# Ray0089/geometric-aware-dense-matching

Measured on AMD Instinct MI355X. Metric: rgbd_crops_per_sec_geomatch_fwd, higher is better.
Workload: dtype bf16x3/f32acc

## Files before the change

geometric_aware_dense_matching_amd/_lib.py:

```python
import ctypes
import os
import subprocess

_PKG = os.path.dirname(os.path.abspath(__file__))
LIB_PATH = os.path.join(_PKG, "libgdm_hip.so")
CSRC = os.path.join(_PKG, "csrc")

_vp = ctypes.c_void_p
_i = ctypes.c_int
_f = ctypes.c_float
_sz = ctypes.c_size_t

GDM_RANSAC_MAX_H = 4096


class KnnJob(ctypes.Structure):
    _fields_ = [("support", _vp), ("query", _vp), ("idx", _vp), ("d2", _vp),
                ("support_bstride", ctypes.c_int64), ("query_bstride", ctypes.c_int64),
                ("S", ctypes.c_int32), ("Q", ctypes.c_int32), ("K", ctypes.c_int32), ("grid_w", ctypes.c_int32)]


class PwSeg(ctypes.Structure):
    _fields_ = [("x", _vp), ("idx", _vp), ("C", ctypes.c_int32), ("n_src", ctypes.c_int32)]


class PwJob(ctypes.Structure):
    _fields_ = [("x", _vp), ("wt", _vp), ("out", _vp), ("n", ctypes.c_int32)]


class CopyJob(ctypes.Structure):
    _fields_ = [("dst", _vp), ("src", _vp), ("sb", ctypes.c_int64), ("s1", ctypes.c_int64), ("s2", ctypes.c_int64),
                ("B", ctypes.c_int32), ("R1", ctypes.c_int32), ("R2", ctypes.c_int32), ("E", ctypes.c_int32)]


SIGNATURES = {
    "gdm_last_error": (ctypes.c_char_p, []),
    "gdm_version": (_i, []),
    "gdm_knn_batch": (None, [_vp, _sz, _sz, _sz, _vp, _sz, _sz, _vp]),
    "gdm_knn_batch_hip": (_i, [_vp, _vp, _i, _i, _i, _i, _vp, _vp, _vp]),
    "gdm_knn_jobs_workspace_bytes": (_sz, [ctypes.POINTER(KnnJob), _i, _i]),
    "gdm_knn_jobs_ws_hip": (_i, [ctypes.POINTER(KnnJob), _i, _i, _vp, _sz, _vp]),
    "gdm_ballquery_hip": (_i, [_i, _i, _i, _f, _i, _vp, _vp, _vp, _vp]),
    "gdm_furthestsampling_hip": (_i, [_i, _i, _i, _vp, _vp, _vp, _vp]),
    "gdm_interpolation_forward_hip": (_i, [_i, _i, _i, _i, _vp, _vp, _vp, _vp, _vp]),
    "gdm_interpolation_backward_hip": (_i, [_i, _i, _i, _i, _vp, _vp, _vp, _vp, _vp]),
    "gdm_labelstat_ballrange_hip": (_i, [_i, _i, _i, _f, _i, _vp, _vp, _vp, _vp, _vp]),
    "gdm_labelstat_idx_hip": (_i, [_i, _i, _i, _i, _i, _vp, _vp, _vp, _vp]),
    "gdm_group_gather_hip": (_i, [_vp, _vp, _i, _i, _i, _i, _i, _vp, _vp]),
    "gdm_group_gather_bwd2_hip": (_i, [_vp, ctypes.c_long, _vp, _i, _i, _i, _i, _i, _vp, _vp]),
    "gdm_gather_max_hip": (_i, [_vp, _vp, _i, _i, _i, _i, _i, _vp, _vp, _vp]),
    "gdm_gather_max_bwd_hip": (_i, [_vp, _vp, _i, _i, _i, _i, _vp, _vp]),
    "gdm_rel_pos_enc_hip": (_i, [_vp, _vp, _i, _i, _i, _vp, _vp]),
    "gdm_att_pool_hip": (_i, [_vp, _vp, _i, _i, _i, _i, _vp, _vp]),
    "gdm_att_pool_bwd_hip": (_i, [_vp, _vp, _vp, _i, _i, _i, _i, _vp, _vp, _vp]),
    "gdm_match_workspace_bytes": (_sz, [_i, _i, _i]),
    "gdm_match_hip": (_i, [_vp, _vp, _i, _i, _i, _i, _i, _vp, _vp, _vp, _vp, _sz, _vp]),
    "gdm_match_rows_bytes": (_sz, [_i]),
    "gdm_match_partial_bytes": (_sz, [_i, _i]),
    "gdm_match_pack_hip": (_i, [_vp, _i, _i, _i, _i, _vp, _vp]),
    "gdm_match_pack2_hip": (_i, [_vp, _i, _i, _vp, _vp, _i, _i, _vp, _i, _i, _vp]),
    "gdm_match_packed_hip": (_i, [_vp, _vp, _i, _i, _i, _vp, _vp, _vp, _vp, _sz, _vp]),
    "gdm_seg_mask_hip": (_i, [_vp, _i, _i, _vp, _vp, _vp]),
    "gdm_spline_aggregate_hip": (_i, [_vp, _vp, _vp, _vp, _vp, _vp, _i, _i, _i, _i, _vp, _vp]),
    "gdm_spline_aggregate_bwd_hip": (_i, [_vp, _vp, _vp, _vp, _i, _i, _i, _vp, _vp]),
    "gdm_spline_direct3_hip": (_i, [_vp, _vp, _vp, _vp, _vp, _vp, _vp, _i, _i, _i, _i, _i, _vp, _vp, _vp, _vp]),
    "gdm_gemm_grouped_hip": (_i, [_vp, _vp, _vp, _vp, _i, _i, _i, _i, _vp, _vp]),
    "gdm_spline_pairs_aggregate3_hip": (_i, [_vp, _vp, _vp, _vp, _vp, _vp, _i, _i, _i, _vp, _vp, _vp, _vp]),
    "gdm_upsample_bilinear_hip": (_i, [_vp, ctypes.c_long, _i, _i, _i, _i, _vp, _vp]),
    "gdm_upsample_bilinear_bwd_hip": (_i, [_vp, ctypes.c_long, _i, _i, _i, _i, _vp, _vp]),
    "gdm_topk_rows_hip": (_i, [_vp, ctypes.c_long, _i, _i, _vp, _vp, _vp]),
    "gdm_topk_negdist_hip": (_i, [_vp, _vp, _i, _i, _i, _vp, _vp]),
    "gdm_edge_feature_hip": (_i, [_vp, _vp, _i, _i, _i, _i, _vp, _vp]),
    "gdm_edge_feature_bwd_hip": (_i, [_vp, _vp, _i, _i, _i, _i, _vp, _vp]),
    "gdm_circle_rows_fwd_hip": (_i, [_vp, _i, _i, _vp, _vp, _vp, _vp, _f, _f, _f, _vp, _vp, _vp, _vp]),
    "gdm_circle_rows_bwd_hip": (_i, [_vp, _i, _i, _vp, _vp, _vp, _vp, _f, _f, _f, _vp, _vp, _vp, _vp, _vp]),
    "gdm_circle_match_rows_bytes": (_sz, [_i]),
    "gdm_circle_match_tp_bytes": (_sz, [_i]),
    "gdm_circle_match_pack_hip": (_i, [_vp, _i, _vp, _vp, _vp, _vp]),
    "gdm_circle_match_nbr_hip": (_i, [_vp, _i, _f, _vp, _vp]),
    "gdm_circle_match_visbits_hip": (_i, [_vp, _i, _i, _vp, _vp]),
    "gdm_circle_match_nbr_items_hip": (_i, [_vp, _i, _vp, _i, _vp, _vp]),
    "gdm_circle_match_fwd2_hip": (_i, [_vp, _vp, _vp, _vp, _vp, _i, _i, _vp, _vp, _vp, _vp, _i, _vp, _i, _f, _f, _vp, _vp, _vp, _vp]),
    "gdm_circle_match_bwd2_hip": (_i, [_vp, _vp, _vp, _vp, _vp, _i, _i, _vp, _vp, _vp, _vp, _i, _vp, _i, _f, _f, _vp, _vp, _vp, _vp, _vp, _vp]),
    "gdm_circle_match_bwd_parts": (_i, [_i, _i]),
    "gdm_lfa_stage_hip": (_i, [_vp] * 13 + [_i, _i, _i, _i, _i, _f, _vp, _vp]),
    "gdm_kabsch_stats_hip": (_i, [_vp, ctypes.c_long, _i, _i, _vp, _vp, _vp, _i, _i, _i, _vp, _vp]),
    "gdm_kabsch_solve_hip": (_i, [_vp, _i, _i, _vp, _vp, _vp]),
    "gdm_ransac_workspace_bytes": (_sz, [_i, _i, _i]),
    "gdm_ransac_pose_hip": (_i, [_vp, ctypes.c_long, _i, _i, _vp, _vp, _vp, _vp, _i, _i, _i, _i, _f, ctypes.c_double, ctypes.c_uint32, _i,
                                 _vp, _sz, _vp, _vp, _vp, _vp, _vp]),
    "gdm_icp_transform_hip": (_i, [_vp, ctypes.c_long, _i, _i, _vp, _i, _i, _vp, _vp]),
    "gdm_icp_update_hip": (_i, [_vp, ctypes.c_long, _i, _i, _vp, _vp, _vp, _vp, _i, _i, _i, _f, ctypes.c_double, _i, _vp, _vp, _vp, _vp,
                                _vp]),
    "gdm_targets_workspace_bytes": (_sz, [_i, _i, _i]),
    "gdm_hpr_visible_hip": (_i, [_vp, ctypes.c_long, _vp, _vp, _i, _i, _vp, _sz, _vp, _vp, _vp]),
    "gdm_pose_targets_hip": (_i, [_vp, ctypes.c_long, _i, _i, _vp, _vp, _vp, ctypes.c_long, _vp, _i, _i, _i, ctypes.c_double, _vp, _sz,
                                  _vp, _vp, _vp, _vp, _vp]),
    "gdm_affine_act_maxk_hip": (_i, [_vp, _vp, _vp, ctypes.c_long, _i, ctypes.c_long, _i, _i, _f, _vp, _vp]),
    "gdm_prelu1_hip": (_i, [_vp, _vp, ctypes.c_long, _vp, _vp]),
    "gdm_prelu1_bwd_hip": (_i, [_vp, _vp, _vp, ctypes.c_long, _vp, _vp, _vp]),
    "gdm_affine_act_hip": (_i, [_vp, _vp, _vp, _vp, _vp, _vp, ctypes.c_long, _i, ctypes.c_long, _i, _f, _vp, _vp]),
    "gdm_upconv3x3_gather_hip": (_i, [_vp, _vp, _vp, _i, _i, _i, _i, _i, _i, _i, _f, _vp, _vp]),
    "gdm_upconv3x3_gather2_hip": (_i, [_vp, _vp, _vp, _i, _i, _i, _i, _i, _i, _i, _f, _vp, _vp, _vp]),
    "gdm_upconv3x3_gather_bwd_hip": (_i, [_vp, _i, _i, _i, _i, _i, _i, _vp, _vp]),
    "gdm_upconv_fused64_weight_bytes": (_sz, []),
    "gdm_upconv_fused64_pack_weight_hip": (_i, [_vp, _vp, _vp]),
    "gdm_upconv_fused64_hip": (_i, [_vp, _vp, _vp, _vp, _i, _i, _i, _i, _i, _i, _i, _f, _vp, _vp]),
    "gdm_psp_combine2_hip": (_i, [_vp, _vp, _i, _vp, _i, _vp, _i, _vp, _i, _vp, _i, _i, _i, _i, _vp, _vp, _vp]),
    "gdm_gather_add_affine_act2_hip": (_i, [_vp, _vp, _vp, _vp, _vp, _i, _i, _i, _i, _i, _f, _vp, _vp, _i, _vp]),
    "gdm_conv1x1_gather_add_act2_hip": (_i, [_vp, _vp, _vp, _vp, _vp, _vp, _i, _i, _i, ctypes.c_long, _i, _f, _i, _vp, _vp]),
    "gdm_conv64_gather_add_act_mfma2_hip": (_i, [_vp, _vp, _vp, _vp, _vp, _vp, _i, _i, ctypes.c_long, _i, _f, _i, _i, _vp, _vp, _i, _vp]),
    "gdm_conv64_gather_add_final_hip": (_i, [_vp, _vp, _vp, _vp, _vp, _vp, _i, _i, ctypes.c_long, _i, _f, _vp, _vp, _vp, _vp]),
    "gdm_conv3x3_act_bytes": (_sz, [_i, _i, _i, _i]),
    "gdm_conv3x3_weight_bytes": (_sz, [_i, _i]),
    "gdm_conv3x3_pack_weight_hip": (_i, [_vp, _i, _i, _vp, _vp]),
    "gdm_conv3x3_pack_act_hip": (_i, [_vp, _i, _i, _i, _i, _vp, _vp]),
    "gdm_conv3x3_packed_hip": (_i, [_vp, _vp, _vp, _vp, _vp, _i, _i, _i, _i, _i, _i, _vp, _vp]),
    "gdm_conv3x3_strided_hip": (_i, [_vp, _vp, _vp, _vp, _vp, _i, _i, _i, _i, _i, _i, _i, _vp, _vp, _vp]),
    "gdm_conv1x1_strided_hip": (_i, [_vp, _vp, _vp, _vp, _i, _i, _i, _i, _i, _i, _i, _vp, _vp]),
    "gdm_affine_relu_maxpool_hip": (_i, [_vp, _vp, _vp, _i, _i, _i, _i, _vp, _vp]),
    "gdm_conv1x1_logsoftmax_hip": (_i, [_vp, _vp, _vp, _i, _i, ctypes.c_long, _vp, _vp]),
    "gdm_pack_rows64_hip": (_i, [_vp, _i, _vp, _vp]),
    "gdm_upconv_final_points_hip": (_i, [_vp, _vp, _vp, _vp, _vp, _i, _f, _vp, _vp, _i, _i, _i, _i, _i, _i, _vp, _vp]),
    "gdm_psp_pools_hip": (_i, [_vp, ctypes.c_long, _i, _i, _vp, _vp, _vp, _vp, _vp]),
    "gdm_psp_pools_bwd_hip": (_i, [_vp, _vp, _vp, _vp, ctypes.c_long, _i, _i, _vp, _vp]),
    "gdm_conv1x1_weight_bytes": (_sz, [_i, _i]),
    "gdm_conv1x1_pack_weight_hip": (_i, [_vp, _i, _i, _vp, _vp]),
    "gdm_conv_pack_weight_dgrad_hip": (_i, [_vp, _i, _i, _i, _vp, _vp]),
    "gdm_conv1x1_packed_hip": (_i, [_vp, _vp, _vp, _vp, _i, _i, _i, _i, _i, _i, _i, _vp, _vp]),
    "gdm_depth_to_xyz_hip": (_i, [_vp, _vp, _vp, _i, _i, _i, _i, _vp, _vp]),
    "gdm_depth_normals_hip": (_i, [_vp, _vp, _i, _i, _i, _i, _i, _i, _vp, _vp]),
    "gdm_warp_crop_hip": (_i, [_vp, _vp, _vp, _vp, _vp, _vp, _vp, _i, _i, _i, _i, _vp, _vp, _vp, _vp, _vp, _vp]),
    "gdm_fill_depth_workspace_bytes": (_sz, [_i, _i, _i, _i]),
    "gdm_fill_depth_hip": (_i, [_vp, _i, _i, _i, _i, _f, _vp, _sz, _vp, _vp, _vp]),
    "gdm_bn_sums_len": (ctypes.c_long, [_i, _i, ctypes.c_long]),
    "gdm_bn_stats_hip": (_i, [_vp, _i, _i, ctypes.c_long, _vp, _vp]),
    "gdm_bn_fwd_apply_hip": (_i, [_vp, _vp, _i, _vp, _vp, _i, _i, ctypes.c_long, _f, _f, _i, _f, _vp, _vp, _vp, _vp, _vp]),
    "gdm_bn_bwd_reduce_hip": (_i, [_vp, _vp, _vp, _i, _i, ctypes.c_long, _i, _f, _vp, _vp]),
    "gdm_bn_bwd_apply_hip": (_i, [_vp, _vp, _vp, _i, _vp, _vp, _i, _i, ctypes.c_long, _i, _f, _vp, _vp, _vp, _vp]),
    "gdm_point_heads2_hip": (_i, [_vp, _vp, _i, _vp, _vp, _i, _i, _i, _i, _vp, _vp, _vp, _vp, _i, _i, _vp, _vp, _i, _vp, _vp, _vp]),
    "gdm_pointwise2_hip": (_i, [ctypes.POINTER(PwSeg), _i, _vp, _i, _vp, _vp, _i, _i, _i, _i, _f, _vp, _i, _i, _i, _vp]),
    "gdm_pointwise_jobs_hip": (_i, [ctypes.POINTER(PwJob), _i, _i, _i, _i, _vp]),
    "gdm_pointwise_chain2_hip": (_i, [_vp, _vp, _vp, _vp, _i, _f, _vp, _vp, _vp, _i, _f, _i, _i, _i, _i, _i, _vp, _vp, _vp]),
    "gdm_stem_weight_bytes": (_sz, []),
    "gdm_stem_pack_weight_hip": (_i, [_vp, _vp, _vp]),
    "gdm_stem_hip": (_i, [_vp, _vp, _vp, _vp, _i, _i, _i, _vp, _vp, _vp]),
    "gdm_wgrad_x_bytes": (_sz, [_i, _i, _i, _i]),
    "gdm_wgrad_go_bytes": (_sz, [_i, _i, _i, _i]),
    "gdm_wgrad_pack_x_hip": (_i, [_vp, _i, _i, _i, _i, _vp, _vp]),
    "gdm_wgrad_pack_go_hip": (_i, [_vp, _i, _i, _i, _i, _vp, _vp]),
    "gdm_wgrad_x1_bytes": (_sz, [_i, _i, _i]),
    "gdm_wgrad_pack_x1_hip": (_i, [_vp, _i, _i, _i, _vp, _vp]),
    "gdm_mfma_probe_hip": (_i, [_i, _i, _i, _vp, _vp]),
    "gdm_mfma_probe_lds_hip": (_i, [_i, _i, _i, _vp, _vp]),
    "gdm_wgrad_direct_hip": (_i, [_vp, ctypes.c_long, _vp, ctypes.c_long, _i, _i, _i, _i, _i, _vp, _vp, _vp]),
    "gdm_conv1x1_packed_wb_hip": (_i, [_vp, _vp, ctypes.c_long, _i, _i, _i, _i, _i, _vp, _vp]),
    "gdm_copy_jobs_hip": (_i, [ctypes.POINTER(CopyJob), _i, _vp]),
}

_lib = None


def _objects_state():
    st = {}
    for f in sorted(os.listdir(CSRC)):
        if f.endswith(".o"):
            st[f] = os.stat(os.path.join(CSRC, f)).st_mtime_ns
    return st


def build(verbose=False):
    import hashlib
    import json
    import time
    before = _objects_state()
    out = None if verbose else subprocess.DEVNULL
    t0 = time.time()
    subprocess.check_call(["make", "-C", CSRC, "-j4"], stdout=out)
    after = _objects_state()
    rebuilt = sorted(f for f, m in after.items() if before.get(f) != m)
    with open(LIB_PATH, "rb") as f:
        digest = hashlib.sha256(f.read()).hexdigest()[:16]
    rec = {"mode": "hipcc --offload-arch=gfx950 via csrc/Makefile (in-tree, ahead of time)", "recompiled": rebuilt,
           "up_to_date": sorted(set(after) - set(rebuilt)), "lib": os.path.basename(LIB_PATH), "lib_bytes": os.path.getsize(LIB_PATH),
           "lib_sha256_16": digest, "seconds": round(time.time() - t0, 1), "when": time.strftime("%Y-%m-%dT%H:%M:%S")}
    try:
        with open(os.path.join(CSRC, "build_record.json"), "w") as f:
            json.dump(rec, f, indent=1)
    except OSError:
        pass
    print("[gdm build] recompiled %d of %d translation units%s; %s %d bytes sha256 %s" %
          (len(rebuilt), len(after), (": " + " ".join(rebuilt)) if rebuilt else "", rec["lib"], rec["lib_bytes"], digest))
    return LIB_PATH


def build_record():
    import hashlib
    import json
    rec = {}
    try:
        with open(os.path.join(CSRC, "build_record.json")) as f:
            rec = json.load(f)
    except (OSError, ValueError):
        rec = {"mode": "prebuilt library (no build record travelled)"}
    try:
        with open(LIB_PATH, "rb") as f:
            rec["loaded_lib_sha256_16"] = hashlib.sha256(f.read()).hexdigest()[:16]
    except OSError:
        rec["loaded_lib_sha256_16"] = None
    rec.pop("up_to_date", None)
    if rec.get("lib_sha256_16") is not None:
        rec["record_matches_loaded_lib"] = rec["lib_sha256_16"] == rec["loaded_lib_sha256_16"]
    return rec


def lib():
    global _lib
    if _lib is None:
        if not os.path.exists(LIB_PATH):
            raise RuntimeError(
                "libgdm_hip.so is not built (%s). Run `python -c 'import __graft_entry__ as g; g.build()'` "
                "or `make -C geometric_aware_dense_matching_amd/csrc`. There is no CPU fallback." % LIB_PATH)
        import torch
        l = ctypes.CDLL(LIB_PATH)
        for name, (res, args) in SIGNATURES.items():
            fn = getattr(l, name)
            fn.restype = res
            fn.argtypes = args
        _lib = l
    return _lib


class GdmError(RuntimeError):
    pass


def check(rc, what):
    if rc != 0:
        msg = lib().gdm_last_error()
        raise GdmError("%s failed (rc=%d): %s" % (what, rc, msg.decode() if msg else "?"))
```

geometric_aware_dense_matching_amd/csrc/gdm_conv.hip:

```cpp
#include "gdm_common.h"
#include <math.h>
#include <stdlib.h>

namespace {

typedef __attribute__((ext_vector_type(16))) float f32x16;
typedef __attribute__((ext_vector_type(8))) __bf16 bf16x8;
typedef __attribute__((ext_vector_type(4))) unsigned u32x4;

constexpr int ROWB = 512;
constexpr int CV_PIX = 256;
constexpr int CV_CO = 128;
constexpr int CV_PANEL = CV_CO * ROWB;
#ifndef GDM_CONV_TAP_INNER
#define GDM_CONV_TAP_INNER 1
#endif
#ifndef GDM_CONV16_PF
#define GDM_CONV16_PF 2
#endif
#ifndef GDM_CONV_GLDS
#define GDM_CONV_GLDS 1
#endif

__device__ __forceinline__ void split8(const float* v, unsigned (&hi)[4], unsigned (&lo)[4])
{
#pragma unroll
    for (int j = 0; j < 4; ++j) gdm_split2(v[2 * j], v[2 * j + 1], hi[j], lo[j]);
}

__global__ __launch_bounds__(256) void conv_pack_act_kernel(const float* __restrict__ x, int C, int H, int W,
                                                            unsigned char* __restrict__ out)
{
    __shared__ float t[128][65];
    const int b = blockIdx.z, chunk = blockIdx.y;
    const int nchunk = (C + 127) / 128;
    const int cvalid = min(128, C - chunk * 128);
    const int hw = H * W;
    const long plane = (long)(H + 2) * (W + 2);
    const int p0 = blockIdx.x * 64;
    const int lane = threadIdx.x & 63, w = threadIdx.x >> 6;
    const int p = min(p0 + lane, hw - 1);
    const float* xb = x + ((long)b * C + chunk * 128) * hw;
    for (int c = w; c < cvalid; c += 4) t[c][lane] = xb[(long)c * hw + p];
    __syncthreads();
    const int pp = p0 + lane;
    if (pp >= hw) return;
    const int y = pp / W, xx = pp - y * W;
    unsigned char* o = out + (((long)(b * nchunk + chunk) * 32) * plane + (long)(y + 1) * (W + 2) + xx + 1) * 16;
    for (int q = w; q * 8 < cvalid; q += 4) {
        float v[8];
#pragma unroll
        for (int j = 0; j < 8; ++j) v[j] = t[q * 8 + j][lane];
        unsigned hi[4], lo[4];
        split8(v, hi, lo);
        *reinterpret_cast<uint4*>(o + (long)q * plane * 16) = make_uint4(hi[0], hi[1], hi[2], hi[3]);
        *reinterpret_cast<uint4*>(o + (long)(16 + q) * plane * 16) = make_uint4(lo[0], lo[1], lo[2], lo[3]);
    }
}

__global__ __launch_bounds__(256) void conv_pack_w_kernel(const float* __restrict__ w, int Cout, int Cin, int taps, unsigned char* __restrict__ out,
                                                          int dgrad = 0)
{
    const int nchunk = (Cin + 127) / 128;
    const int CoutP = (Cout + 127) & ~127;
    const long item = (long)blockIdx.x * 256 + threadIdx.x;
    const long rows = (long)taps * nchunk * CoutP;
    if (item >= rows * 16) return;
    const int ch = (int)(item & 15);
    const long row = item >> 4;
    const int co = (int)(row % CoutP);
    const int tc = (int)(row / CoutP);
    const int chunk = tc % nchunk, tap = tc / nchunk;
    float v[8];
#pragma unroll
    for (int j = 0; j < 8; ++j) {
        const int ci = chunk * 128 + ch * 8 + j;
        const bool in = co < Cout && ci < Cin;
        v[j] = !in ? 0.f : dgrad ? w[((long)ci * Cout + co) * taps + (taps - 1 - tap)] : w[((long)co * Cin + ci) * taps + tap];
    }
    unsigned hi[4], lo[4];
    split8(v, hi, lo);
    unsigned char* r = out + row * ROWB;
    *reinterpret_cast<uint4*>(r + ch * 16) = make_uint4(hi[0], hi[1], hi[2], hi[3]);
    *reinterpret_cast<uint4*>(r + 256 + ch * 16) = make_uint4(lo[0], lo[1], lo[2], lo[3]);
}

__device__ __forceinline__ int swz(int col, int ch) { return col * ROWB + (((ch & 16) | ((ch ^ col) & 15)) << 4); }

typedef __attribute__((ext_vector_type(4))) float f32x4;

#ifndef GDM_CONV_NPH
#define GDM_CONV_NPH 2
#endif
#ifndef GDM_CONV16_LATE
#define GDM_CONV16_LATE 1
#endif
#ifndef GDM_CONV_MFMA_ORDER
#define GDM_CONV_MFMA_ORDER 0
#endif
constexpr int MF_NPH = GDM_CONV_NPH;
constexpr int MF_WPIX = 16 * MF_NPH;
constexpr int MF_WAVES = CV_PIX / MF_WPIX;
constexpr int MF_THREADS = MF_WAVES * 64;
constexpr int MF_TSTRIDE = 132;
constexpr int MF_SMEM = 2 * CV_PANEL > CV_PIX * MF_TSTRIDE * 4 ? 2 * CV_PANEL : CV_PIX * MF_TSTRIDE * 4;

template <int ACT, bool HAS_RES, int TAPS = 9, bool PIXMAJOR = false, int NKS = 8, int NCB = 8, int WV = MF_WAVES>
__global__ __launch_bounds__(MF_THREADS) void conv_mfma16_kernel(const unsigned char* __restrict__ xpk, const unsigned char* __restrict__ wpk,
                                                                 const float* __restrict__ scale, const float* __restrict__ shift,
                                                                 const float* __restrict__ res, int B, int Cin, int Cout, int H, int W,
                                                                 float* __restrict__ out, const int32_t* __restrict__ rowidx = nullptr,
                                                                 const int32_t* __restrict__ tile_co0 = nullptr,
                                                                 unsigned char* __restrict__ outpk = nullptr, int stride = 1,
                                                                 long wbstride = 0)
{
    extern __shared__ __attribute__((aligned(16))) unsigned char smem[];
    constexpr int NS = NKS / 2;
    constexpr int UG = (NCB % 2 == 0) ? 2 : 3;
    constexpr int NPR = NCB / UG;
    constexpr int PANEL = NCB * 16 * ROWB;
    constexpr int TST = NCB * 16 + 4;
    static_assert(NCB == 8 || (NCB == 4 && !PIXMAJOR) || (NCB == 9 && !PIXMAJOR && WV == 8),
                  "64-channel tiles: NCHW / packed output only; 144-channel tiles: NCHW fp32 output only (no packed output: a tile straddles 128-channel chunks)");
    constexpr int NPH = MF_NPH;
    const int tid = threadIdx.x, lane = tid & 63;
    const int wave = __builtin_amdgcn_readfirstlane(tid >> 6);
    const int l16 = lane & 15, kg = lane >> 4;
    const int nchunk = (Cin + 127) / 128;
    const int npanel = TAPS * nchunk;
    const int hw = H * W;
    const long ptot = rowidx ? (long)B : (long)B * hw;
    const unsigned bx = blockIdx.x, by = blockIdx.y;
    const long pix0 = (long)bx * (WV * MF_WPIX) + wave * MF_WPIX;
    const int co0 = tile_co0 ? __builtin_amdgcn_readfirstlane(tile_co0[bx]) : by * (NCB * 16);
    const long pc = min(pix0, ptot - MF_WPIX);
    const int b = (int)(pc / hw);
    const int prem = (int)(pc - (long)b * hw);
    const int Wi = W * stride;
    const long plane = (long)(H * stride + 2) * (Wi + 2);
    const long oplane = (long)(H + 2) * (W + 2);
    const __amdgpu_buffer_rsrc_t xr = __builtin_amdgcn_make_buffer_rsrc(const_cast<unsigned char*>(xpk), (short)0, 0x7ffffff0, 0x00020000);
    int avoff[NPH];
#pragma unroll
    for (int ph = 0; ph < NPH; ++ph) {
        const int pr = prem + 16 * ph;
        const int yy = pr / W, xx = pr - yy * W;
        const long pixbase = rowidx ? (long)max(rowidx[pc + l16 + 16 * ph], 0) : (long)(yy * stride) * (Wi + 2) + (long)(xx + l16) * stride;
        avoff[ph] = (int)(((long)kg * plane + pixbase) * 16);
    }

    u32x4 ahi[NS][NPH], alo[NS][NPH];
    struct Pan { int chunk, ky, kx; };
    auto pan_next = [&](Pan p) -> Pan {
        if (TAPS == 1) { ++p.chunk; return p; }
        if (GDM_CONV_TAP_INNER) {
            if (++p.kx == 3) { p.kx = 0; if (++p.ky == 3) { p.ky = 0; ++p.chunk; } }
        } else {
            if (++p.chunk == nchunk) { p.chunk = 0; if (++p.kx == 3) { p.kx = 0; ++p.ky; } }
        }
        return p;
    };
    const int a_base = (int)(((long)(rowidx ? 0 : b) * nchunk * 32) * plane * 16);
    const int a_chunk = (int)(32 * plane * 16), a_rowb = (Wi + 2) * 16;
    auto pan_a = [&](Pan p) -> int { return a_base + p.chunk * a_chunk + p.ky * a_rowb + p.kx * 16; };
    const int sstride = (int)(4 * plane * 16);
    const int lostride = (int)(16 * plane * 16);
    auto load_a = [&](int r, int S) {
#pragma unroll
        for (int ph = 0; ph < NPH; ++ph) {
            ahi[S][ph] = __builtin_bit_cast(u32x4, __builtin_amdgcn_raw_buffer_load_b128(xr, avoff[ph], r + S * sstride, 0));
            alo[S][ph] = __builtin_bit_cast(u32x4, __builtin_amdgcn_raw_buffer_load_b128(xr, avoff[ph], r + S * sstride + lostride, 0));
        }
    };
    constexpr int THREADS = WV * 64, WGPIX = WV * MF_WPIX;
    constexpr int HS = (NCB * 512 / THREADS) / 2;
    u32x4 stage[HS];
    const __amdgpu_buffer_rsrc_t wr = __builtin_amdgcn_make_buffer_rsrc(const_cast<unsigned char*>(wpk), (short)0, 0x7ffffff0, 0x00020000);
    const int w_base = (wbstride ? (int)(((long)bx * WGPIX / hw) * wbstride) : 0) + co0 * ROWB;
    const int w_panel = ((Cout + 127) & ~127) * ROWB;
    auto pan_w = [&](Pan p) -> int { return w_base + ((TAPS == 1) ? p.chunk : (p.ky * 3 + p.kx) * nchunk + p.chunk) * w_panel; };
    auto stage_load = [&](int src, int half) {
#pragma unroll
        for (int i = 0; i < HS; ++i)
            stage[i] = __builtin_bit_cast(u32x4, __builtin_amdgcn_raw_buffer_load_b128(wr, tid * 16, src + (half * HS + i) * THREADS * 16, 0));
    };
    auto stage_store = [&](int buf, int half) {
        unsigned char* base = smem + buf * PANEL;
#pragma unroll
        for (int i = 0; i < HS; ++i) {
            const int g = (half * HS + i) * THREADS + tid;
            *reinterpret_cast<u32x4*>(base + swz(g >> 5, g & 31)) = stage[i];
        }
    };
    constexpr bool GLDS = GDM_CONV_GLDS && WV == 8;
    constexpr int NPIECE = PANEL / 1024 / 8;
    int glds_voff = 0;
    if (GLDS) {
        const int hrow = lane >> 5, sl = lane & 31;
        const int col15 = (2 * wave + hrow) & 15;
        glds_voff = wave * 1024 + hrow * 512 + (((sl & 16) | ((sl ^ col15) & 15)) << 4);
    }
    typedef __attribute__((address_space(3))) void* lds_void_ptr;
    auto stage_glds = [&](int src, int buf) {
#pragma unroll
        for (int i = 0; i < NPIECE; ++i)
            __builtin_amdgcn_raw_ptr_buffer_load_lds(wr, (lds_void_ptr)(smem + buf * PANEL + (i * 8 + wave) * 1024), 16, glds_voff, src + i * 8192, 0, 0);
    };

    f32x4 acc[NPH][NCB];
#pragma unroll
    for (int ph = 0; ph < NPH; ++ph)
#pragma unroll
        for (int cb = 0; cb < NCB; ++cb)
#pragma unroll
            for (int i = 0; i < 4; ++i) acc[ph][cb][i] = 0.f;

    constexpr int LATE = GDM_CONV16_LATE < NS ? GDM_CONV16_LATE : NS;
    Pan pcur = {0, (TAPS == 1) ? 1 : 0, (TAPS == 1) ? 1 : 0};
    if (GLDS) {
        stage_glds(pan_w(pcur), 0);
    } else {
        stage_load(pan_w(pcur), 0);
        stage_store(0, 0);
        stage_load(pan_w(pcur), 1);
        stage_store(0, 1);
    }
    int rcur = pan_a(pcur);
#pragma unroll
    for (int S = 0; S < NS - LATE; ++S) load_a(rcur, S);
    Pan pnxt = npanel > 1 ? pan_next(pcur) : pcur;
    int rnext = pan_a(pnxt), wnext = pan_w(pnxt);
    for (int it = 0; it < npanel; ++it) {
        __syncthreads();
        const bool more = it + 1 < npanel;
        const unsigned char* base = smem + (it & 1) * PANEL;
        constexpr int PF = GDM_CONV16_PF;
        constexpr int NU = NPR * NS;
        u32x4 fh[PF + 1][UG], fl[PF + 1][UG];
        auto frag_load = [&](int un) {
            const int S = un / NPR, pr = un % NPR, slot = un % (PF + 1);
#pragma unroll
            for (int j = 0; j < UG; ++j) {
                const int col = (UG * pr + j) * 16 + l16;
                fh[slot][j] = *reinterpret_cast<const u32x4*>(base + swz(col, 4 * S + kg));
                fl[slot][j] = *reinterpret_cast<const u32x4*>(base + swz(col, 16 + 4 * S + kg));
            }
        };
#pragma unroll
        for (int un = 0; un < PF; ++un) frag_load(un);
#pragma unroll
        for (int u = 0; u < NU; ++u) {
            const int S = u / NPR, pr = u % NPR, slot = u % (PF + 1);
            if (u + PF < NU) frag_load(u + PF);
#if GDM_CONV_MFMA_ORDER == 0
#pragma unroll
            for (int ph = 0; ph < NPH; ++ph) {
                const bf16x8 ah = __builtin_bit_cast(bf16x8, ahi[S][ph]);
                const bf16x8 al = __builtin_bit_cast(bf16x8, alo[S][ph]);
#pragma unroll
                for (int j = 0; j < UG; ++j) {
                    f32x4 c = acc[ph][UG * pr + j];
                    c = __builtin_amdgcn_mfma_f32_16x16x32_bf16(ah, __builtin_bit_cast(bf16x8, fl[slot][j]), c, 0, 0, 0);
                    c = __builtin_amdgcn_mfma_f32_16x16x32_bf16(al, __builtin_bit_cast(bf16x8, fh[slot][j]), c, 0, 0, 0);
                    c = __builtin_amdgcn_mfma_f32_16x16x32_bf16(ah, __builtin_bit_cast(bf16x8, fh[slot][j]), c, 0, 0, 0);
                    acc[ph][UG * pr + j] = c;
                }
            }
#else
#pragma unroll
            for (int prod = 0; prod < 3; ++prod)
#pragma unroll
                for (int ph = 0; ph < NPH; ++ph)
#pragma unroll
                    for (int j = 0; j < UG; ++j) {
                        const bf16x8 av = __builtin_bit_cast(bf16x8, prod == 1 ? alo[S][ph] : ahi[S][ph]);
                        const bf16x8 bv = __builtin_bit_cast(bf16x8, prod == 0 ? fl[slot][j] : fh[slot][j]);
                        acc[ph][UG * pr + j] = __builtin_amdgcn_mfma_f32_16x16x32_bf16(av, bv, acc[ph][UG * pr + j], 0, 0, 0);
                    }
#endif
            if (pr == NPR - 1 && S < NS - LATE) load_a(rnext, S);
            if (!GLDS && u == NU / 2 && more) {
                stage_store((it + 1) & 1, 0);
                stage_load(wnext, 1);
            }
            if (u == 0) {
                if (more) { if (GLDS) stage_glds(wnext, (it + 1) & 1); else stage_load(wnext, 0); }
#pragma unroll
                for (int S2 = NS - LATE; S2 < NS; ++S2) load_a(rcur, S2);
            }
#pragma unroll
            for (int i = 0; i < 3 * UG * NPH; ++i) {
                __builtin_amdgcn_sched_group_barrier(0x008, 1, 0);
                if (u + PF < NU && (i % NPH) == 0 && i < 2 * UG * NPH) __builtin_amdgcn_sched_group_barrier(0x100, 1, 0);
            }
            __builtin_amdgcn_sched_barrier(0);
        }
        if (!GLDS && more) stage_store((it + 1) & 1, 1);
        rcur = rnext;
        if (it + 2 < npanel) pnxt = pan_next(pnxt);
        rnext = pan_a(pnxt);
        wnext = pan_w(pnxt);
    }

    if (pix0 >= ptot) return;
    if (PIXMAJOR) {
#pragma unroll
        for (int cb = 0; cb < NCB; ++cb) {
            const int co = co0 + cb * 16 + l16;
            if (co >= Cout) continue;
            const float sc = scale ? scale[co] : 1.f, sh = shift ? shift[co] : 0.f;
            const int ocol = tile_co0 ? cb * 16 + l16 : co;
            const int ostride = tile_co0 ? CV_CO : Cout;
#pragma unroll
            for (int ph = 0; ph < NPH; ++ph)
#pragma unroll
                for (int r = 0; r < 4; ++r) {
                    float v = acc[ph][cb][r] * sc + sh;
                    if (ACT == 1) v = fmaxf(v, 0.f);
                    out[(pix0 + 16 * ph + 4 * kg + r) * ostride + ocol] = v;
                }
        }
        return;
    }
    float* tl = reinterpret_cast<float*>(smem) + wave * MF_WPIX * TST;
    if (outpk) __syncthreads();
#pragma unroll
    for (int cb = 0; cb < NCB; ++cb) {
        const int co = co0 + cb * 16 + l16;
        const bool live = co < Cout;
        const float sc = (live && scale) ? scale[co] : 1.f, sh = (live && shift) ? shift[co] : 0.f;
        float* op = out ? out + ((long)b * Cout + (live ? co : 0)) * hw + prem : nullptr;
        const float* rp = (HAS_RES && live) ? res + ((long)b * Cout + co) * hw + prem : nullptr;
#pragma unroll
        for (int ph = 0; ph < NPH; ++ph) {
            const int poff = 16 * ph + 4 * kg;
            float v[4];
#pragma unroll
            for (int j = 0; j < 4; ++j) v[j] = acc[ph][cb][j] * sc + sh;
            if (HAS_RES && live) {
                const float4 r4 = *reinterpret_cast<const float4*>(rp + poff);
                v[0] += r4.x; v[1] += r4.y; v[2] += r4.z; v[3] += r4.w;
            }
            if (ACT == 1) {
#pragma unroll
                for (int j = 0; j < 4; ++j) v[j] = fmaxf(v[j], 0.f);
            }
            if (op && live) *reinterpret_cast<float4*>(op + poff) = make_float4(v[0], v[1], v[2], v[3]);
            if (outpk) {
#pragma unroll
                for (int j = 0; j < 4; ++j) tl[(poff + j) * TST + cb * 16 + l16] = live ? v[j] : 0.f;
            }
        }
    }
    if (outpk) {
        __builtin_amdgcn_fence(__ATOMIC_ACQ_REL, "wavefront");
        const int lr = lane & 31, h = lane >> 5;
        const int ochunks = (Cout + 127) / 128;
        const int ochunk = co0 / 128;
#pragma unroll
        for (int half = 0; half < MF_WPIX / 32; ++half) {
            const int pp = prem + 32 * half + lr;
            const int yy = pp / W, xx = pp - yy * W;
            unsigned char* ob = outpk + (((long)(b * ochunks + ochunk) * 32) * oplane + (long)(yy + 1) * (W + 2) + xx + 1) * 16;
            const float* row = tl + (32 * half + lr) * TST;
#pragma unroll
            for (int it = 0; it < NCB; ++it) {
                const int ql = 2 * it + h;
                if (co0 + ql * 8 >= Cout) continue;
                const int q = (co0 % 128) / 8 + ql;
                const float4 a0 = *reinterpret_cast<const float4*>(row + ql * 8);
                const float4 a1 = *reinterpret_cast<const float4*>(row + ql * 8 + 4);
                const float v[8] = {a0.x, a0.y, a0.z, a0.w, a1.x, a1.y, a1.z, a1.w};
                unsigned hi[4], lo[4];
                split8(v, hi, lo);
                *reinterpret_cast<uint4*>(ob + (long)q * oplane * 16) = make_uint4(hi[0], hi[1], hi[2], hi[3]);
                *reinterpret_cast<uint4*>(ob + (long)(16 + q) * oplane * 16) = make_uint4(lo[0], lo[1], lo[2], lo[3]);
            }
        }
    }
}

#define CONV_KERNEL conv_mfma16_kernel
constexpr int CONV_THREADS = MF_THREADS, CONV_WPIX = MF_WPIX, CONV_SMEM = MF_SMEM;

}

namespace {
template <int CHAIN>
__global__ __launch_bounds__(512) void mfma_probe_kernel(int iters, float* __restrict__ sink)
{
    typedef __attribute__((ext_vector_type(8))) __bf16 pb_bf16x8;
    typedef __attribute__((ext_vector_type(4))) float pb_f32x4;
    const int lane = threadIdx.x & 63;
    pb_f32x4 acc[8];
#pragma unroll
    for (int i = 0; i < 8; ++i) acc[i] = pb_f32x4{0.f, 0.f, 0.f, 0.f};
    const unsigned seed = 0x3f803f80u + (unsigned)lane;
    u32x4 av = {seed, seed ^ 1u, seed ^ 2u, seed ^ 3u}, bv = {seed ^ 4u, seed ^ 5u, seed ^ 6u, seed ^ 7u};
    const pb_bf16x8 a = __builtin_bit_cast(pb_bf16x8, av), b = __builtin_bit_cast(pb_bf16x8, bv);
    for (int it = 0; it < iters; it += CHAIN) {
#pragma unroll
        for (int i = 0; i < 8; ++i)
#pragma unroll
            for (int c = 0; c < CHAIN; ++c) acc[i] = __builtin_amdgcn_mfma_f32_16x16x32_bf16(a, b, acc[i], 0, 0, 0);
    }
    float t = 0.f;
#pragma unroll
    for (int i = 0; i < 8; ++i) t += acc[i][0] + acc[i][1] + acc[i][2] + acc[i][3];
    if (t == 12345.678f) sink[0] = t;
}
template <int RPU>
__global__ __launch_bounds__(512) void mfma_probe_lds_kernel(int iters, float* __restrict__ sink)
{
    typedef __attribute__((ext_vector_type(8))) __bf16 pb_bf16x8;
    typedef __attribute__((ext_vector_type(4))) float pb_f32x4;
    extern __shared__ __attribute__((aligned(16))) unsigned char pl[];
    const int tid = threadIdx.x, lane = tid & 63;
    for (int i = tid; i < 4096; i += 512) reinterpret_cast<u32x4*>(pl)[i] = u32x4{0x3f803f80u, 0x3f803f80u, 0x3f803f80u, 0x3f803f80u + (unsigned)i};
    __syncthreads();
    pb_f32x4 acc[4];
#pragma unroll
    for (int i = 0; i < 4; ++i) acc[i] = pb_f32x4{0.f, 0.f, 0.f, 0.f};
    const unsigned seed = 0x3f803f80u + (unsigned)lane;
    u32x4 a0 = {seed, seed ^ 1u, seed ^ 2u, seed ^ 3u}, a1 = {seed ^ 4u, seed ^ 5u, seed ^ 6u, seed ^ 7u};
    u32x4 f[4] = {a0, a1, a0, a1};
    int off = lane * 16;
    for (int it = 0; it < iters; ++it) {
#pragma unroll
        for (int r = 0; r < RPU; ++r) f[r] = *reinterpret_cast<const u32x4*>(pl + ((off + r * 1024) & 0xffff));
        off += 4096;
#pragma unroll
        for (int prod = 0; prod < 3; ++prod)
#pragma unroll
            for (int i = 0; i < 4; ++i)
                acc[i] = __builtin_amdgcn_mfma_f32_16x16x32_bf16(__builtin_bit_cast(pb_bf16x8, prod == 1 ? a1 : a0),
                                                                 __builtin_bit_cast(pb_bf16x8, f[(i + prod) & 3]), acc[i], 0, 0, 0);
    }
    float t = 0.f;
#pragma unroll
    for (int i = 0; i < 4; ++i) t += acc[i][0] + acc[i][1] + acc[i][2] + acc[i][3];
    if (t == 12345.678f) sink[0] = t;
}
}

extern "C" int gdm_mfma_probe_lds_hip(int blocks, int iters, int rpu, float* sink, void* stream)
{
    GDM_CHECK_ARG(blocks >= 1 && blocks <= 65535 && iters >= 1 && (rpu == 1 || rpu == 2 || rpu == 4) && sink, "gdm_mfma_probe_lds_hip: bad arguments");
    if (rpu == 4) hipLaunchKernelGGL(mfma_probe_lds_kernel<4>, dim3(blocks), dim3(512), 65536, (hipStream_t)stream, iters, sink);
    else if (rpu == 2) hipLaunchKernelGGL(mfma_probe_lds_kernel<2>, dim3(blocks), dim3(512), 65536, (hipStream_t)stream, iters, sink);
    else hipLaunchKernelGGL(mfma_probe_lds_kernel<1>, dim3(blocks), dim3(512), 65536, (hipStream_t)stream, iters, sink);
    return gdm_launch_status("mfma_probe_lds_kernel");
}

extern "C" int gdm_mfma_probe_hip(int blocks, int iters, int chain, float* sink, void* stream)
{
    GDM_CHECK_ARG(blocks >= 1 && blocks <= 65535 && iters >= 3 && iters % 3 == 0 && (chain == 1 || chain == 3) && sink,
                  "gdm_mfma_probe_hip: bad arguments (iters a multiple of 3, chain 1 or 3)");
    if (chain == 3) hipLaunchKernelGGL(mfma_probe_kernel<3>, dim3(blocks), dim3(512), 0, (hipStream_t)stream, iters, sink);
    else hipLaunchKernelGGL(mfma_probe_kernel<1>, dim3(blocks), dim3(512), 0, (hipStream_t)stream, iters, sink);
    return gdm_launch_status("mfma_probe_kernel");
}

static bool cin_ok(int Cin) { return Cin == 64 || (Cin >= 128 && Cin % 128 == 0); }

static bool narrow_tiles(unsigned pixel_tiles, int Cout)
{
    return Cout <= 64 || (long)pixel_tiles * ((Cout + 127) / 128) < 256;
}

extern "C" size_t gdm_conv3x3_act_bytes(int B, int Cin, int H, int W)
{
    if (B < 1 || !cin_ok(Cin) || H < 1 || W < 1) return 0;
    return (size_t)B * (H + 2) * (W + 2) * ((Cin + 127) / 128) * ROWB;
}

extern "C" size_t gdm_conv3x3_weight_bytes(int Cout, int Cin)
{
    if (Cout < 1 || !cin_ok(Cin)) return 0;
    return (size_t)9 * ((Cin + 127) / 128) * ((Cout + 127) & ~127) * ROWB;
}

extern "C" size_t gdm_conv1x1_weight_bytes(int Cout, int Cin)
{
    if (Cout < 1 || !cin_ok(Cin)) return 0;
    return (size_t)((Cin + 127) / 128) * ((Cout + 127) & ~127) * ROWB;
}

static int pack_weight(const float* w, int Cout, int Cin, int taps, void* wpk, void* stream, const char* who, int dgrad = 0)
{
    GDM_CHECK_ARG(w && wpk, "%s: NULL pointer", who);
    GDM_CHECK_ARG(Cout >= 1 && cin_ok(Cin), "%s: Cout=%d Cin=%d (Cin a multiple of 128, or 64)", who, Cout, Cin);
    const long items = (long)taps * ((Cin + 127) / 128) * ((Cout + 127) & ~127) * 16;
    hipLaunchKernelGGL(conv_pack_w_kernel, dim3(gdm_cdiv(items, 256)), dim3(256), 0, (hipStream_t)stream, w, Cout, Cin, taps, (unsigned char*)wpk, dgrad);
    return gdm_launch_status("conv_pack_w_kernel");
}

extern "C" int gdm_conv_pack_weight_dgrad_hip(const float* w, int Cout, int Cin, int taps, void* wpk, void* stream)
{
    GDM_CHECK_ARG(taps == 9 || taps == 1, "gdm_conv_pack_weight_dgrad_hip: taps=%d (9 or 1)", taps);
    return pack_weight(w, Cin, Cout, taps, wpk, stream, "gdm_conv_pack_weight_dgrad_hip", 1);
}

extern "C" int gdm_conv3x3_pack_weight_hip(const float* w, int Cout, int Cin, void* wpk, void* stream)
{
    return pack_weight(w, Cout, Cin, 9, wpk, stream, "gdm_conv3x3_pack_weight_hip");
}

extern "C" int gdm_conv1x1_pack_weight_hip(const float* w, int Cout, int Cin, void* wpk, void* stream)
{
    return pack_weight(w, Cout, Cin, 1, wpk, stream, "gdm_conv1x1_pack_weight_hip");
}

extern "C" int gdm_conv3x3_pack_act_hip(const float* x, int B, int Cin, int H, int W, void* xpk, void* stream)
{
    GDM_CHECK_ARG(x && xpk, "gdm_conv3x3_pack_act_hip: NULL pointer");
    GDM_CHECK_ARG(B >= 1 && B <= 65535 && cin_ok(Cin) && H >= 1 && W >= 1, "gdm_conv3x3_pack_act_hip: bad shape (Cin=%d: a multiple of 128, or 64)", Cin);
    dim3 grid(gdm_cdiv((long)H * W, 64), (Cin + 127) / 128, B);
    hipLaunchKernelGGL(conv_pack_act_kernel, grid, dim3(256), 0, (hipStream_t)stream, x, Cin, H, W, (unsigned char*)xpk);
    return gdm_launch_status("conv_pack_act_kernel");
}

static int conv3x3_launch(const void* xpk, const void* wpk, const float* scale, const float* shift, const float* res,
                          int B, int Cin, int Cout, int H, int W, int stride, int act, float* out, void* outpk, void* stream,
                          const char* who);

extern "C" int gdm_conv3x3_packed_hip(const void* xpk, const void* wpk, const float* scale, const float* shift, const float* res,
                                      int B, int Cin, int Cout, int H, int W, int act, float* out, void* stream)
{
    return conv3x3_launch(xpk, wpk, scale, shift, res, B, Cin, Cout, H, W, 1, act, out, nullptr, stream, "gdm_conv3x3_packed_hip");
}

extern "C" int gdm_conv3x3_strided_hip(const void* xpk, const void* wpk, const float* scale, const float* shift, const float* res,
                                       int B, int Cin, int Cout, int H, int W, int stride, int act, float* out, void* outpk, void* stream)
{
    return conv3x3_launch(xpk, wpk, scale, shift, res, B, Cin, Cout, H, W, stride, act, out, outpk, stream, "gdm_conv3x3_strided_hip");
}

static int conv3x3_launch(const void* xpk, const void* wpk, const float* scale, const float* shift, const float* res,
                          int B, int Cin, int Cout, int H, int W, int stride, int act, float* out, void* outpk, void* stream,
                          const char* who)
{
    GDM_CHECK_ARG(stride == 1 || stride == 2, "%s: stride=%d (1 or 2)", who, stride);
    GDM_CHECK_ARG(xpk && wpk && (out || outpk), "%s: NULL pointer", who);
    GDM_CHECK_ARG(B >= 1 && cin_ok(Cin) && Cout >= 1, "%s: Cin=%d Cout=%d (Cin a multiple of 128, or 64)", who, Cin, Cout);
    GDM_CHECK_ARG(W % 32 == 0 && H >= 1 && (H * W) % CONV_WPIX == 0,
                  "%s: W=%d must be a multiple of 32 and H*W=%d of %d", who, W, H * W, CONV_WPIX);
    GDM_CHECK_ARG(act == 0 || act == 1, "%s: act=%d", who, act);
    GDM_CHECK_ARG(!outpk || (Cout % 8 == 0 && ((long)B * H * W) % CV_PIX == 0),
                  "%s: packed output needs Cout %% 8 == 0 and B*H*W %% 256 == 0 (got Cout=%d, B*H*W=%ld)", who, Cout, (long)B * H * W);
    const long ptot = (long)B * H * W;
    dim3 grid(gdm_cdiv(ptot, CV_PIX), gdm_cdiv(Cout, CV_CO));
    hipStream_t s = (hipStream_t)stream;
    constexpr int SMEM = CONV_SMEM;
    static bool attr = false;
    if (!attr) {
        (void)hipFuncSetAttribute((const void*)CONV_KERNEL<0, false>, hipFuncAttributeMaxDynamicSharedMemorySize, SMEM);
        (void)hipFuncSetAttribute((const void*)CONV_KERNEL<1, false>, hipFuncAttributeMaxDynamicSharedMemorySize, SMEM);
        (void)hipFuncSetAttribute((const void*)CONV_KERNEL<0, true>, hipFuncAttributeMaxDynamicSharedMemorySize, SMEM);
        (void)hipFuncSetAttribute((const void*)CONV_KERNEL<1, true>, hipFuncAttributeMaxDynamicSharedMemorySize, SMEM);
        (void)hipFuncSetAttribute((const void*)CONV_KERNEL<0, false, 9, false, 4>, hipFuncAttributeMaxDynamicSharedMemorySize, SMEM);
        (void)hipFuncSetAttribute((const void*)CONV_KERNEL<1, false, 9, false, 4>, hipFuncAttributeMaxDynamicSharedMemorySize, SMEM);
        (void)hipFuncSetAttribute((const void*)CONV_KERNEL<0, true, 9, false, 4>, hipFuncAttributeMaxDynamicSharedMemorySize, SMEM);
        (void)hipFuncSetAttribute((const void*)CONV_KERNEL<1, true, 9, false, 4>, hipFuncAttributeMaxDynamicSharedMemorySize, SMEM);
        attr = true;
    }
#define CV(A, R, NK) hipLaunchKernelGGL((CONV_KERNEL<A, R, 9, false, NK>), grid, dim3(CONV_THREADS), SMEM, s, (const unsigned char*)xpk, (const unsigned char*)wpk, scale, shift, res, B, Cin, Cout, H, W, out, (const int32_t*)nullptr, (const int32_t*)nullptr, (unsigned char*)outpk, stride)
    if (narrow_tiles(grid.x, Cout)) {
        constexpr int SMEM4 = 2 * 64 * ROWB > CV_PIX * 68 * 4 ? 2 * 64 * ROWB : CV_PIX * 68 * 4;
        const dim3 grid4(grid.x, gdm_cdiv(Cout, 64));
        static bool attr4 = false;
#define CV4(A, R, NK) hipLaunchKernelGGL((CONV_KERNEL<A, R, 9, false, NK, 4>), grid4, dim3(CONV_THREADS), SMEM4, s, (const unsigned char*)xpk, (const unsigned char*)wpk, scale, shift, res, B, Cin, Cout, H, W, out, (const int32_t*)nullptr, (const int32_t*)nullptr, (unsigned char*)outpk, stride)
#define AT4(A, R, NK) (void)hipFuncSetAttribute((const void*)CONV_KERNEL<A, R, 9, false, NK, 4>, hipFuncAttributeMaxDynamicSharedMemorySize, SMEM4)
        if (!attr4) {
            AT4(0, false, 4); AT4(1, false, 4); AT4(0, true, 4); AT4(1, true, 4);
            AT4(0, false, 8); AT4(1, false, 8); AT4(0, true, 8); AT4(1, true, 8);
            attr4 = true;
        }
        if (Cin != 64 && (long)grid4.x * grid4.y < 256 && ptot % (CV_PIX / 2) == 0) {
            const dim3 grid4h(gdm_cdiv(ptot, CV_PIX / 2), grid4.y);
            static bool attr4h = false;
#define CV4H(A, R) hipLaunchKernelGGL((CONV_KERNEL<A, R, 9, false, 8, 4, MF_WAVES / 2>), grid4h, dim3(CONV_THREADS / 2), SMEM4, s, (const unsigned char*)xpk, (const unsigned char*)wpk, scale, shift, res, B, Cin, Cout, H, W, out, (const int32_t*)nullptr, (const int32_t*)nullptr, (unsigned char*)outpk, stride)
#define AT4H(A, R) (void)hipFuncSetAttribute((const void*)CONV_KERNEL<A, R, 9, false, 8, 4, MF_WAVES / 2>, hipFuncAttributeMaxDynamicSharedMemorySize, SMEM4)
            if (!attr4h) {
                AT4H(0, false); AT4H(1, false); AT4H(0, true); AT4H(1, true);
                attr4h = true;
            }
            if (act == 0) { if (res) CV4H(0, true); else CV4H(0, false); }
            else { if (res) CV4H(1, true); else CV4H(1, false); }
#undef CV4H
#undef AT4H
            return gdm_launch_status("conv_mfma16_kernel (3x3, 64-channel tiles, 128 pixels)");
        }
        if (Cin == 64) {
            if (act == 0) { if (res) CV4(0, true, 4); else CV4(0, false, 4); }
            else { if (res) CV4(1, true, 4); else CV4(1, false, 4); }
        } else {
            if (act == 0) { if (res) CV4(0, true, 8); else CV4(0, false, 8); }
            else { if (res) CV4(1, true, 8); else CV4(1, false, 8); }
        }
#undef CV4
#undef AT4
        return gdm_launch_status("conv_mfma16_kernel (3x3, 64-channel tiles)");
    }
    if (Cin == 64) {
        if (act == 0) { if (res) CV(0, true, 4); else CV(0, false, 4); }
        else { if (res) CV(1, true, 4); else CV(1, false, 4); }
    } else {
        if (act == 0) { if (res) CV(0, true, 8); else CV(0, false, 8); }
        else { if (res) CV(1, true, 8); else CV(1, false, 8); }
    }
#undef CV
    return gdm_launch_status("conv_mfma16_kernel (3x3)");
}

extern "C" int gdm_gemm_grouped_hip(const void* xpk, const void* wpk, const int32_t* rowidx, const int32_t* tile_co0, int R, int M,
                                    int Cin, int Cout_total, float* out, void* stream)
{
    GDM_CHECK_ARG(xpk && wpk && rowidx && tile_co0 && out, "gdm_gemm_grouped_hip: NULL pointer");
    GDM_CHECK_ARG(R >= 256 && R % 256 == 0 && M >= 1 && Cin >= 128 && Cin % 128 == 0 && Cout_total >= 128 && Cout_total % 128 == 0,
                  "gdm_gemm_grouped_hip: R=%d (multiple of 256) M=%d Cin=%d Cout_total=%d (multiples of 128)", R, M, Cin, Cout_total);
    static bool attr = false;
    if (!attr) {
        (void)hipFuncSetAttribute((const void*)CONV_KERNEL<0, false, 1, true>, hipFuncAttributeMaxDynamicSharedMemorySize, 2 * CV_PANEL);
        attr = true;
    }
    hipLaunchKernelGGL((CONV_KERNEL<0, false, 1, true>), dim3(R / CV_PIX, 1), dim3(CONV_THREADS), 2 * CV_PANEL, (hipStream_t)stream,
                       (const unsigned char*)xpk, (const unsigned char*)wpk, (const float*)nullptr, (const float*)nullptr, (const float*)nullptr,
                       R, Cin, Cout_total, 1, M, out, rowidx, tile_co0);
    return gdm_launch_status("gemm_grouped_kernel");
}

static int conv1x1_launch(const void* xpk, const void* wpk, const float* scale, const float* shift,
                          int B, int Cin, int Cout, int H, int W, int stride, int act, int pixel_major, float* out, void* stream,
                          const char* who);

extern "C" int gdm_conv1x1_packed_hip(const void* xpk, const void* wpk, const float* scale, const float* shift,
                                      int B, int Cin, int Cout, int H, int W, int act, int pixel_major, float* out, void* stream)
{
    return conv1x1_launch(xpk, wpk, scale, shift, B, Cin, Cout, H, W, 1, act, pixel_major, out, stream, "gdm_conv1x1_packed_hip");
}

extern "C" int gdm_conv1x1_packed_wb_hip(const void* xpk, const void* wpk, long w_bstride, int B, int Cin, int Cout, int H, int W, float* out,
                                         void* stream)
{
    GDM_CHECK_ARG(xpk && wpk && out, "gdm_conv1x1_packed_wb_hip: NULL pointer");
    GDM_CHECK_ARG(B >= 1 && Cin >= 128 && Cin % 128 == 0 && Cout >= 1, "gdm_conv1x1_packed_wb_hip: Cin=%d Cout=%d (Cin a multiple of 128)", Cin, Cout);
    GDM_CHECK_ARG(W % 32 == 0 && H >= 1 && (H * W) % CV_PIX == 0, "gdm_conv1x1_packed_wb_hip: W=%d must be a multiple of 32 and H*W=%d of %d",
                  W, H * W, CV_PIX);
    GDM_CHECK_ARG(w_bstride >= 0 && w_bstride % 16 == 0, "gdm_conv1x1_packed_wb_hip: w_bstride=%ld", w_bstride);
    const long ptot = (long)B * H * W;
    dim3 grid(gdm_cdiv(ptot, CV_PIX), gdm_cdiv(Cout, CV_CO));
    static bool attr = false;
    if (!attr) {
        (void)hipFuncSetAttribute((const void*)CONV_KERNEL<0, false, 1, false>, hipFuncAttributeMaxDynamicSharedMemorySize, 2 * CV_PANEL);
        attr = true;
    }
    hipLaunchKernelGGL((CONV_KERNEL<0, false, 1, false>), grid, dim3(CONV_THREADS), 2 * CV_PANEL, (hipStream_t)stream, (const unsigned char*)xpk,
                       (const unsigned char*)wpk, (const float*)nullptr, (const float*)nullptr, (const float*)nullptr, B, Cin, Cout, H, W, out,
                       (const int32_t*)nullptr, (const int32_t*)nullptr, (unsigned char*)nullptr, 1, w_bstride);
    return gdm_launch_status("conv1x1_bf16x3_kernel (per-image weights)");
}

extern "C" int gdm_conv1x1_strided_hip(const void* xpk, const void* wpk, const float* scale, const float* shift,
                                       int B, int Cin, int Cout, int H, int W, int stride, int act, float* out, void* stream)
{
    return conv1x1_launch(xpk, wpk, scale, shift, B, Cin, Cout, H, W, stride, act, 0, out, stream, "gdm_conv1x1_strided_hip");
}

static int conv1x1_launch(const void* xpk, const void* wpk, const float* scale, const float* shift,
                          int B, int Cin, int Cout, int H, int W, int stride, int act, int pixel_major, float* out, void* stream,
                          const char* who)
{
    GDM_CHECK_ARG(stride == 1 || stride == 2, "%s: stride=%d (1 or 2)", who, stride);
    GDM_CHECK_ARG(xpk && wpk && out, "%s: NULL pointer", who);
    GDM_CHECK_ARG(B >= 1 && cin_ok(Cin) && Cout >= 1, "%s: Cin=%d Cout=%d (Cin a multiple of 128, or 64)", who, Cin, Cout);
    GDM_CHECK_ARG(Cin != 64 || !pixel_major, "%s: Cin=64 is built for the NCHW output only", who);
    GDM_CHECK_ARG(W % 32 == 0 && H >= 1 && (H * W) % CONV_WPIX == 0,
                  "%s: W=%d must be a multiple of 32 and H*W=%d of %d", who, W, H * W, CONV_WPIX);
    GDM_CHECK_ARG(act == 0 || act == 1, "%s: act=%d", who, act);
    const long ptot = (long)B * H * W;
    const unsigned ptiles = gdm_cdiv(ptot, CV_PIX);
    if (Cin != 64 && !pixel_major && stride == 1 && Cout % 144 == 0 && GDM_CONV_GLDS) {
        const long r128 = gdm_cdiv((long)ptiles * gdm_cdiv(Cout, 128), 256) * 128, r144 = gdm_cdiv((long)ptiles * (Cout / 144), 256) * 144;
        if (r144 < r128) {
            constexpr int PANEL9 = 9 * 16 * ROWB, TILE9 = CV_PIX * (9 * 16 + 4) * 4;
            constexpr int SMEM9 = 2 * PANEL9 > TILE9 ? 2 * PANEL9 : TILE9;
            static bool attr9 = false;
            if (!attr9) {
                (void)hipFuncSetAttribute((const void*)CONV_KERNEL<0, false, 1, false, 8, 9>, hipFuncAttributeMaxDynamicSharedMemorySize, SMEM9);
                (void)hipFuncSetAttribute((const void*)CONV_KERNEL<1, false, 1, false, 8, 9>, hipFuncAttributeMaxDynamicSharedMemorySize, SMEM9);
                attr9 = true;
            }
            const dim3 grid9(ptiles, Cout / 144);
#define C19(A) hipLaunchKernelGGL((CONV_KERNEL<A, false, 1, false, 8, 9>), grid9, dim3(CONV_THREADS), SMEM9, (hipStream_t)stream, (const unsigned char*)xpk, (const unsigned char*)wpk, scale, shift, (const float*)nullptr, B, Cin, Cout, H, W, out, (const int32_t*)nullptr, (const int32_t*)nullptr, (unsigned char*)nullptr, stride)
            if (act == 0) C19(0); else C19(1);
#undef C19
            return gdm_launch_status("conv1x1_bf16x3_kernel (144-channel tiles)");
        }
    }
    const bool narrow = Cin != 64 && !pixel_major && narrow_tiles(ptiles, Cout);
    const unsigned ctiles = gdm_cdiv(Cout, narrow ? 64 : CV_CO);
    const dim3 grid(ptiles, ctiles);
    hipStream_t s = (hipStream_t)stream;
    static bool attr = false;
    if (!attr) {
        (void)hipFuncSetAttribute((const void*)CONV_KERNEL<0, false, 1, false>, hipFuncAttributeMaxDynamicSharedMemorySize, 2 * CV_PANEL);
        (void)hipFuncSetAttribute((const void*)CONV_KERNEL<1, false, 1, false>, hipFuncAttributeMaxDynamicSharedMemorySize, 2 * CV_PANEL);
        (void)hipFuncSetAttribute((const void*)CONV_KERNEL<0, false, 1, true>, hipFuncAttributeMaxDynamicSharedMemorySize, 2 * CV_PANEL);
        (void)hipFuncSetAttribute((const void*)CONV_KERNEL<1, false, 1, true>, hipFuncAttributeMaxDynamicSharedMemorySize, 2 * CV_PANEL);
        (void)hipFuncSetAttribute((const void*)CONV_KERNEL<0, false, 1, false, 4>, hipFuncAttributeMaxDynamicSharedMemorySize, 2 * CV_PANEL);
        (void)hipFuncSetAttribute((const void*)CONV_KERNEL<1, false, 1, false, 4>, hipFuncAttributeMaxDynamicSharedMemorySize, 2 * CV_PANEL);
        attr = true;
    }
    if (Cin == 64) {
#define C1TAIL , (const int32_t*)nullptr, (const int32_t*)nullptr, (unsigned char*)nullptr, stride
#define C1H(A) hipLaunchKernelGGL((CONV_KERNEL<A, false, 1, false, 4>), grid, dim3(CONV_THREADS), 2 * CV_PANEL, s, (const unsigned char*)xpk, (const unsigned char*)wpk, scale, shift, (const float*)nullptr, B, Cin, Cout, H, W, out C1TAIL)
        if (act == 0) C1H(0); else C1H(1);
#undef C1H
        return gdm_launch_status("conv1x1_bf16x3_kernel");
    }
    if (narrow) {
        const dim3 grid4 = grid;
        static bool attr4 = false;
        if (!attr4) {
            (void)hipFuncSetAttribute((const void*)CONV_KERNEL<0, false, 1, false, 8, 4>, hipFuncAttributeMaxDynamicSharedMemorySize, 2 * 64 * ROWB);
            (void)hipFuncSetAttribute((const void*)CONV_KERNEL<1, false, 1, false, 8, 4>, hipFuncAttributeMaxDynamicSharedMemorySize, 2 * 64 * ROWB);
            attr4 = true;
        }
#define C14(A) hipLaunchKernelGGL((CONV_KERNEL<A, false, 1, false, 8, 4>), grid4, dim3(CONV_THREADS), 2 * 64 * ROWB, s, (const unsigned char*)xpk, (const unsigned char*)wpk, scale, shift, (const float*)nullptr, B, Cin, Cout, H, W, out C1TAIL)
        if (act == 0) C14(0); else C14(1);
#undef C14
        return gdm_launch_status("conv1x1_bf16x3_kernel (64-channel tiles)");
    }
#define C1(A, P) hipLaunchKernelGGL((CONV_KERNEL<A, false, 1, P>), grid, dim3(CONV_THREADS), 2 * CV_PANEL, s, (const unsigned char*)xpk, (const unsigned char*)wpk, scale, shift, (const float*)nullptr, B, Cin, Cout, H, W, out C1TAIL)
    if (act == 0) { if (pixel_major) C1(0, true); else C1(0, false); }
    else { if (pixel_major) C1(1, true); else C1(1, false); }
#undef C1
    return gdm_launch_status("conv1x1_bf16x3_kernel");
}
```

geometric_aware_dense_matching_amd/ops.py:

```python
import ctypes
import os

import torch

from . import _lib, settings
from ._lib import KnnJob, check

MATCH_BF16X3 = 0
MATCH_F32 = 1


def _stream():
    return torch.cuda.current_stream().cuda_stream


_side_streams = {}


def side_stream(device, which=0):
    key = (device.index if device.index is not None else torch.cuda.current_device(), which)
    st = _side_streams.get(key)
    if st is None:
        st = torch.cuda.Stream(device=device)
        _side_streams[key] = st
    return st


def _stream_lane(device):
    h = torch.cuda.current_stream(device).cuda_stream
    idx = device.index if device.index is not None else torch.cuda.current_device()
    for (d, which), st in _side_streams.items():
        if d == idx and st.cuda_stream == h:
            return ("side", which)
    if _pool is _default_pool:
        return ("main", h)
    return "main"


class fork:

    def __init__(self, device, which=0, after=(), start=None):
        self.side = side_stream(device, which)
        self.cur = torch.cuda.current_stream(device)
        self.after = tuple(after) if isinstance(after, (tuple, list)) else (after,)
        self.start = start
        self._ctx = None

    def __enter__(self):
        if self.start is not None:
            self.side.wait_event(self.start)
        else:
            self.side.wait_stream(self.cur)
        for ev in self.after:
            if ev is not None:
                self.side.wait_event(ev)
        self._ctx = torch.cuda.stream(self.side)
        self._ctx.__enter__()
        return self

    def __exit__(self, *exc):
        self._ctx.__exit__(*exc)
        return False

    def use(self, *tensors):
        for t in tensors:
            if torch.is_tensor(t) and t.is_cuda:
                t.record_stream(self.side)

    def join(self, *tensors):
        self.cur.wait_stream(self.side)
        for t in tensors:
            if torch.is_tensor(t) and t.is_cuda:
                t.record_stream(self.cur)


def _dev(t, dtype, name):
    if not isinstance(t, torch.Tensor) or not t.is_cuda:
        raise RuntimeError("%s must be a CUDA (HIP) tensor: the geoMatch ops have no CPU fallback" % name)
    if t.dtype != dtype:
        raise TypeError("%s must be %s, got %s" % (name, dtype, t.dtype))
    return t if t.is_contiguous() else t.contiguous()


def _idx32(t, name):
    if not isinstance(t, torch.Tensor) or not t.is_cuda:
        raise RuntimeError("%s must be a CUDA (HIP) tensor: the geoMatch ops have no CPU fallback" % name)
    if t.dtype == torch.int64:
        t = t.to(torch.int32)
    elif t.dtype != torch.int32:
        raise TypeError("%s must be int32 or int64, got %s" % (name, t.dtype))
    return t if t.is_contiguous() else t.contiguous()


def knn_batch(support, query, K, return_d2=False):
    support = _dev(support, torch.float32, "support")
    query = _dev(query, torch.float32, "query")
    B, S, _ = support.shape
    Q = query.shape[1]
    assert support.shape[2] == 3 and query.shape[2] == 3 and query.shape[0] == B
    idx = torch.empty((B, Q, K), dtype=torch.int32, device=support.device)
    d2 = torch.empty((B, Q, K), dtype=torch.float32, device=support.device) if return_d2 else None
    check(_lib.lib().gdm_knn_batch_hip(support.data_ptr(), query.data_ptr(), B, S, Q, K, idx.data_ptr(),
                                       d2.data_ptr() if return_d2 else None, _stream()), "gdm_knn_batch_hip")
    return (idx, d2) if return_d2 else idx


def knn_jobs(jobs, B, keep_workspace=None):
    n = len(jobs)
    arr = (KnnJob * n)()
    sizes = []
    for job in jobs:
        sup, qry, K = job[:3]
        for t, nm in ((sup, "support"), (qry, "query")):
            if not t.is_cuda or t.dtype != torch.float32:
                raise RuntimeError("knn_jobs: %s must be a CUDA float32 tensor" % nm)
            if t.dim() != 3 or t.shape[0] != B or t.shape[2] != 3 or t.stride(2) != 1 or t.stride(1) != 3:
                raise ValueError("knn_jobs: %s must be [B,n,3] with unit point stride, got %s strides %s" %
                                 (nm, tuple(t.shape), t.stride()))
        sizes.append(B * qry.shape[1] * K)
    starts = []
    tot = 0
    for sz in sizes:
        starts.append(tot)
        tot += (sz + 63) // 64 * 64
    slab = torch.empty(tot, dtype=torch.int32, device=jobs[0][0].device)
    base = slab.data_ptr()
    outs = []
    for i, job in enumerate(jobs):
        off = starts[i]
        sup, qry, K = job[:3]
        grid_w = int(job[3]) if len(job) > 3 else 0
        S, Q = sup.shape[1], qry.shape[1]
        a = arr[i]
        a.support = sup.data_ptr()
        a.query = qry.data_ptr()
        a.idx = base + 4 * off
        a.d2 = None
        a.support_bstride = sup.stride(0) if B > 1 else S * 3
        a.query_bstride = qry.stride(0) if B > 1 else Q * 3
        a.S, a.Q, a.K = S, Q, K
        a.grid_w = grid_w if (grid_w > 0 and S % grid_w == 0) else 0
        outs.append(slab[off:off + sizes[i]].view(B, Q, K))
    ws = _knn_launch(arr, n, B, jobs[0][0].device)
    if keep_workspace is not None:
        keep_workspace.append(ws)
    return outs


def copy_views(views):
    n = len(views)
    arr = (_lib.CopyJob * n)()
    outs = []
    for i, v in enumerate(views):
        if not v.is_cuda or v.element_size() != 4 or v.dim() not in (3, 4) or v.stride(-1) != 1:
            raise ValueError("copy_views: view %d must be a 3-D / 4-D CUDA tensor of 4-byte elements with a contiguous last dimension" % i)
        out = torch.empty(v.shape, dtype=v.dtype, device=v.device)
        v4 = v if v.dim() == 4 else v.unsqueeze(1)
        arr[i] = _lib.CopyJob(out.data_ptr(), v.data_ptr(), v4.stride(0), v4.stride(1), v4.stride(2),
                              v4.shape[0], v4.shape[1], v4.shape[2], v4.shape[3])
        outs.append(out)
    check(_lib.lib().gdm_copy_jobs_hip(arr, n, _stream()), "gdm_copy_jobs_hip")
    return outs


def _knn_launch(arr, n, B, device):
    L = _lib.lib()
    nbytes = int(L.gdm_knn_jobs_workspace_bytes(arr, n, B))
    ws = torch.empty(max(nbytes, 16), dtype=torch.uint8, device=device)
    check(L.gdm_knn_jobs_ws_hip(arr, n, B, ws.data_ptr(), nbytes, _stream()), "gdm_knn_jobs_ws_hip")
    return ws


def ballquery(radius, nsample, xyz, new_xyz):
    xyz = _dev(xyz, torch.float32, "xyz")
    new_xyz = _dev(new_xyz, torch.float32, "new_xyz")
    B, n, _ = xyz.shape
    m = new_xyz.shape[1]
    idx = torch.zeros((B, m, nsample), dtype=torch.int32, device=xyz.device)
    check(_lib.lib().gdm_ballquery_hip(B, n, m, float(radius), nsample, new_xyz.data_ptr(), xyz.data_ptr(),
                                       idx.data_ptr(), _stream()), "gdm_ballquery_hip")
    return idx


def furthestsampling(xyz, m):
    xyz = _dev(xyz, torch.float32, "xyz")
    B, n, _ = xyz.shape
    idx = torch.empty((B, m), dtype=torch.int32, device=xyz.device)
    temp = torch.empty((B, n), dtype=torch.float32, device=xyz.device)
    check(_lib.lib().gdm_furthestsampling_hip(B, n, m, xyz.data_ptr(), temp.data_ptr(), idx.data_ptr(), _stream()),
          "gdm_furthestsampling_hip")
    return idx


def _feat3(feat):
    if feat.dim() == 4:
        assert feat.shape[3] == 1
        feat = feat.squeeze(3)
    return feat


class _GroupGather(torch.autograd.Function):
    @staticmethod
    def forward(ctx, feat, idx):
        feat = _dev(feat, torch.float32, "feat")
        B, C, n = feat.shape
        m, K = idx.shape[1], idx.shape[2]
        out = torch.empty((B, C, m, K), dtype=torch.float32, device=feat.device)
        check(_lib.lib().gdm_group_gather_hip(feat.data_ptr(), idx.data_ptr(), B, C, n, m, K, out.data_ptr(), _stream()),
              "gdm_group_gather_hip")
        ctx.save_for_backward(idx)
        ctx.n = n
        return out

    @staticmethod
    def backward(ctx, go):
        (idx,) = ctx.saved_tensors
        B, C, m, K = go.shape
        if not (go.dtype == torch.float32 and go.stride(3) == 1 and go.stride(2) == K and go.stride(1) == m * K and go.stride(0) >= C * m * K):
            go = go.contiguous()
        g = torch.zeros((B, C, ctx.n), dtype=torch.float32, device=go.device)
        check(_lib.lib().gdm_group_gather_bwd2_hip(go.data_ptr(), go.stride(0), idx.data_ptr(), B, C, ctx.n, m, K, g.data_ptr(), _stream()),
              "gdm_group_gather_bwd2_hip")
        return g, None


def group_gather(feat, idx):
    idx = _idx32(idx, "idx")
    assert idx.dim() == 3
    return _GroupGather.apply(_feat3(feat), idx)


def gather_nn(feat, idx):
    idx = _idx32(idx, "idx")
    if idx.dim() == 2:
        idx = idx.unsqueeze(2)
    assert idx.shape[2] == 1
    return _GroupGather.apply(_feat3(feat), idx).squeeze(3)


class _GatherMax(torch.autograd.Function):
    @staticmethod
    def forward(ctx, feat, idx):
        feat = _dev(feat, torch.float32, "feat")
        B, C, n = feat.shape
        m, K = idx.shape[1], idx.shape[2]
        out = torch.empty((B, C, m), dtype=torch.float32, device=feat.device)
        need_arg = ctx.needs_input_grad[0]
        arg = torch.empty((B, C, m), dtype=torch.int32, device=feat.device) if need_arg else None
        check(_lib.lib().gdm_gather_max_hip(feat.data_ptr(), idx.data_ptr(), B, C, n, m, K, out.data_ptr(),
                                            arg.data_ptr() if need_arg else None, _stream()), "gdm_gather_max_hip")
        if need_arg:
            ctx.save_for_backward(arg)
        ctx.n = n
        return out

    @staticmethod
    def backward(ctx, go):
        (arg,) = ctx.saved_tensors
        go = go.contiguous()
        B, C, m = go.shape
        g = torch.zeros((B, C, ctx.n), dtype=torch.float32, device=go.device)
        check(_lib.lib().gdm_gather_max_bwd_hip(go.data_ptr(), arg.data_ptr(), B, C, ctx.n, m, g.data_ptr(), _stream()),
              "gdm_gather_max_bwd_hip")
        return g, None


def gather_max(feat, idx):
    idx = _idx32(idx, "idx")
    assert idx.dim() == 3
    return _GatherMax.apply(_feat3(feat), idx)


def rel_pos_enc(xyz, idx):
    xyz = _dev(xyz, torch.float32, "xyz")
    idx = _idx32(idx, "idx")
    B, n, _ = xyz.shape
    K = idx.shape[2]
    assert idx.shape[0] == B and idx.shape[1] == n
    out = torch.empty((B, 10, n, K), dtype=torch.float32, device=xyz.device)
    check(_lib.lib().gdm_rel_pos_enc_hip(xyz.data_ptr(), idx.data_ptr(), B, n, K, out.data_ptr(), _stream()),
          "gdm_rel_pos_enc_hip")
    return out


class _AttPool(torch.autograd.Function):
    @staticmethod
    def forward(ctx, att, feat):
        att = _dev(att, torch.float32, "att")
        feat = _dev(feat, torch.float32, "feat")
        B, C, n, K = att.shape
        assert feat.shape == att.shape
        out = torch.empty((B, C, n), dtype=torch.float32, device=att.device)
        check(_lib.lib().gdm_att_pool_hip(att.data_ptr(), feat.data_ptr(), B, C, n, K, out.data_ptr(), _stream()),
              "gdm_att_pool_hip")
        ctx.save_for_backward(att, feat)
        return out

    @staticmethod
    def backward(ctx, go):
        att, feat = ctx.saved_tensors
        go = go.contiguous()
        B, C, n, K = att.shape
        ga = torch.empty_like(att)
        gf = torch.empty_like(feat)
        check(_lib.lib().gdm_att_pool_bwd_hip(att.data_ptr(), feat.data_ptr(), go.data_ptr(), B, C, n, K,
                                              ga.data_ptr(), gf.data_ptr(), _stream()), "gdm_att_pool_bwd_hip")
        return ga, gf


def att_pool(att, feat):
    return _AttPool.apply(att, feat)


def topk_rows(score, k, return_values=False):
    score = _dev(score, torch.float32, "score")
    n = score.shape[-1]
    rows = score.numel() // n
    idx = torch.empty(score.shape[:-1] + (k,), dtype=torch.int32, device=score.device)
    val = torch.empty(score.shape[:-1] + (k,), dtype=torch.float32, device=score.device) if return_values else None
    check(_lib.lib().gdm_topk_rows_hip(score.data_ptr(), rows, n, k, idx.data_ptr(), val.data_ptr() if return_values else None,
                                       _stream()), "gdm_topk_rows_hip")
    return (idx, val) if return_values else idx


def topk_negdist(gram, xx, k):
    gram = _dev(gram, torch.float32, "gram")
    xx = _dev(xx, torch.float32, "xx")
    B, n, _ = gram.shape
    idx = torch.empty((B, n, k), dtype=torch.int32, device=gram.device)
    check(_lib.lib().gdm_topk_negdist_hip(gram.data_ptr(), xx.data_ptr(), B, n, k, idx.data_ptr(), _stream()), "gdm_topk_negdist_hip")
    return idx


def affine_act_maxk(x, scale, shift, act=0, slope=0.0):
    x = _dev(x, torch.float32, "x")
    B, C, n, K = x.shape
    out = torch.empty((B, C, n), dtype=torch.float32, device=x.device)
    check(_lib.lib().gdm_affine_act_maxk_hip(x.data_ptr(), scale.data_ptr(), shift.data_ptr(), B * C, C, n, K, act, float(slope),
                                             out.data_ptr(), _stream()), "gdm_affine_act_maxk_hip")
    return out


class _EdgeFeature(torch.autograd.Function):
    @staticmethod
    def forward(ctx, x, idx):
        x = _dev(x, torch.float32, "x")
        B, C, n = x.shape
        K = idx.shape[2]
        out = torch.empty((B, 2 * C, n, K), dtype=torch.float32, device=x.device)
        check(_lib.lib().gdm_edge_feature_hip(x.data_ptr(), idx.data_ptr(), B, C, n, K, out.data_ptr(), _stream()),
              "gdm_edge_feature_hip")
        ctx.save_for_backward(idx)
        return out

    @staticmethod
    def backward(ctx, go):
        (idx,) = ctx.saved_tensors
        go = go.contiguous()
        B, C2, n, K = go.shape
        g = torch.zeros((B, C2 // 2, n), dtype=torch.float32, device=go.device)
        check(_lib.lib().gdm_edge_feature_bwd_hip(go.data_ptr(), idx.data_ptr(), B, C2 // 2, n, K, g.data_ptr(), _stream()),
              "gdm_edge_feature_bwd_hip")
        return g, None


def edge_feature(x, idx):
    idx = _idx32(idx, "idx")
    return _EdgeFeature.apply(x, idx)


class _CircleRows(torch.autograd.Function):
    @staticmethod
    def forward(ctx, sim, match, item, xyz, vis, radius, gamma, m):
        sim = _dev(sim, torch.float32, "sim")
        R, Mp = sim.shape
        lse_p = torch.empty(R, dtype=torch.float32, device=sim.device)
        lse_n = torch.empty_like(lse_p)
        loss = torch.empty_like(lse_p)
        check(_lib.lib().gdm_circle_rows_fwd_hip(sim.data_ptr(), R, Mp, match.data_ptr(), item.data_ptr(), xyz.data_ptr(),
                                                 vis.data_ptr(), radius, gamma, m, lse_p.data_ptr(), lse_n.data_ptr(),
                                                 loss.data_ptr(), _stream()), "gdm_circle_rows_fwd_hip")
        ctx.save_for_backward(sim, match, item, xyz, vis, lse_p, lse_n)
        ctx.consts = (radius, gamma, m)
        return loss

    @staticmethod
    def backward(ctx, g):
        sim, match, item, xyz, vis, lse_p, lse_n = ctx.saved_tensors
        radius, gamma, m = ctx.consts
        g = g.contiguous()
        R, Mp = sim.shape
        dsim = torch.empty_like(sim)
        check(_lib.lib().gdm_circle_rows_bwd_hip(sim.data_ptr(), R, Mp, match.data_ptr(), item.data_ptr(), xyz.data_ptr(),
                                                 vis.data_ptr(), radius, gamma, m, lse_p.data_ptr(), lse_n.data_ptr(),
                                                 g.data_ptr(), dsim.data_ptr(), _stream()), "gdm_circle_rows_bwd_hip")
        return dsim, None, None, None, None, None, None, None


def circle_rows(sim, match, item, xyz, vis, radius, gamma=16.0, m=0.2):
    match = _idx32(match, "match")
    item = _idx32(item, "item")
    xyz = _dev(xyz, torch.float32, "xyz")
    if not vis.is_cuda:
        raise RuntimeError("vis must be a CUDA (HIP) tensor: the geoMatch ops have no CPU fallback")
    vis8 = (vis != 0).to(torch.uint8).contiguous()
    return _CircleRows.apply(sim, match, item, xyz, vis8, float(radius), float(gamma), float(m))


def circle_nbr_table(xyz, radius):
    xyz = _dev(xyz, torch.float32, "xyz")
    M = xyz.shape[0]
    nbr = torch.empty((M, (M + 31) // 32), dtype=torch.int32, device=xyz.device)
    check(_lib.lib().gdm_circle_match_nbr_hip(xyz.data_ptr(), M, float(radius), nbr.data_ptr(), _stream()), "gdm_circle_match_nbr_hip")
    return nbr


def circle_nbr_items(xyz, rad):
    xyz = _dev(xyz, torch.float32, "xyz")
    rad = _dev(rad, torch.float32, "rad")
    B, M = rad.shape
    assert xyz.shape == (M, 3)
    nbr = torch.empty((B, M, (M + 31) // 32), dtype=torch.int32, device=xyz.device)
    check(_lib.lib().gdm_circle_match_nbr_items_hip(xyz.data_ptr(), M, rad.data_ptr(), B, nbr.data_ptr(), _stream()),
          "gdm_circle_match_nbr_items_hip")
    return nbr


def circle_visbits(vis):
    if not vis.is_cuda:
        raise RuntimeError("vis must be a CUDA (HIP) tensor: the geoMatch ops have no CPU fallback")
    v8 = (vis != 0).to(torch.uint8).contiguous()
    B, M = v8.shape
    bits = torch.empty((B, (M + 31) // 32), dtype=torch.int32, device=vis.device)
    check(_lib.lib().gdm_circle_match_visbits_hip(v8.data_ptr(), B, M, bits.data_ptr(), _stream()), "gdm_circle_match_visbits_hip")
    return bits


def _cm_pack(x):
    L = _lib.lib()
    n = x.shape[0]
    npad = (n + 127) // 128 * 128
    rows = torch.empty(L.gdm_circle_match_rows_bytes(n), dtype=torch.uint8, device=x.device)
    tp = torch.empty(L.gdm_circle_match_tp_bytes(n), dtype=torch.uint8, device=x.device)
    rsum = torch.empty(npad, dtype=torch.float32, device=x.device)
    check(L.gdm_circle_match_pack_hip(x.data_ptr(), n, rows.data_ptr(), tp.data_ptr(), rsum.data_ptr(), _stream()), "gdm_circle_match_pack_hip")
    return rows, tp, rsum


def _pad_rows(t, npad, fill):
    if t.shape[0] == npad:
        return t.contiguous()
    out = torch.full((npad,) + tuple(t.shape[1:]), fill, dtype=t.dtype, device=t.device)
    out[: t.shape[0]] = t
    return out


class _CircleMatch(torch.autograd.Function):
    @staticmethod
    def forward(ctx, x, y, g, c2, item, nbr, visb, gamma, m, pad_e0=False):
        x = _dev(x, torch.float32, "x")
        y = _dev(y, torch.float32, "y")
        R, M = x.shape[0], y.shape[0]
        assert x.shape[1] == 128 and y.shape[1] == 128, "descriptors must have 128 channels"
        Rp = (R + 127) // 128 * 128
        xr, xt, xs = _cm_pack(x)
        yr, yt, _ = _cm_pack(y)
        per_item = nbr is not None and nbr.dim() == 3
        if pad_e0:
            xs = _pad_rows(x[:, 0].contiguous(), Rp, 0.0)
        gp = _pad_rows(g, Rp, M)
        ip = _pad_rows(item, Rp, 0)
        c2p = _pad_rows(c2, Rp, -1) if c2 is not None else None
        lp = torch.empty(Rp, dtype=torch.float32, device=x.device)
        ln = torch.empty_like(lp)
        loss = torch.empty_like(lp)
        check(_lib.lib().gdm_circle_match_fwd2_hip(xr.data_ptr(), xt.data_ptr(), xs.data_ptr(), yr.data_ptr(), yt.data_ptr(), R, M,
                                                   gp.data_ptr(), c2p.data_ptr() if c2p is not None else None, ip.data_ptr(),
                                                   nbr.data_ptr() if nbr is not None else None, int(per_item),
                                                   visb.data_ptr() if visb is not None else None, int(bool(pad_e0)),
                                                   gamma, m, lp.data_ptr(), ln.data_ptr(), loss.data_ptr(), _stream()), "gdm_circle_match_fwd2_hip")
        ctx.save_for_backward(xr, xt, xs, yr, yt, gp, ip, lp, ln)
        ctx.extra = (c2p, nbr, visb, gamma, m, R, M, per_item, bool(pad_e0))
        return loss[:R]

    @staticmethod
    def backward(ctx, gout):
        xr, xt, xs, yr, yt, gp, ip, lp, ln = ctx.saved_tensors
        c2p, nbr, visb, gamma, m, R, M, per_item, pad_e0 = ctx.extra
        L = _lib.lib()
        Rp, Mp = lp.shape[0], (M + 127) // 128 * 128
        z = lp[:R] + ln[:R]
        sig = torch.where(z > 20.0, torch.ones_like(z), torch.sigmoid(z))
        coef = torch.where(torch.isfinite(lp[:R]), gout.contiguous().float() * sig, torch.zeros_like(z))
        coef = _pad_rows(coef, Rp, 0.0)
        P = int(L.gdm_circle_match_bwd_parts(R, M))
        gx = torch.empty((Rp, 128), dtype=torch.float32, device=lp.device)
        gyp = torch.empty((P, Mp, 128), dtype=torch.float32, device=lp.device)
        check(L.gdm_circle_match_bwd2_hip(xr.data_ptr(), xt.data_ptr(), xs.data_ptr(), yr.data_ptr(), yt.data_ptr(), R, M, gp.data_ptr(),
                                          c2p.data_ptr() if c2p is not None else None, ip.data_ptr(),
                                          nbr.data_ptr() if nbr is not None else None, int(per_item),
                                          visb.data_ptr() if visb is not None else None, int(pad_e0),
                                          gamma, m, lp.data_ptr(), ln.data_ptr(), coef.data_ptr(), gx.data_ptr(), gyp.data_ptr(), _stream()),
              "gdm_circle_match_bwd2_hip")
        return gx[:R], gyp.sum(dim=0)[:M], None, None, None, None, None, None, None, None


def circle_match(x, y, g, item, nbr=None, visb=None, c2=None, gamma=16.0, m=0.2, pad="ones"):
    if pad not in ("ones", "e0"):
        raise ValueError("circle_match: pad=%r" % (pad,))
    g = _idx32(g, "g")
    item = _idx32(item, "item")
    if c2 is not None:
        c2 = _idx32(c2, "c2")
    elif nbr is None or visb is None:
        raise ValueError("circle_match: pass nbr and visb (radius-test positives) or c2 (symmetric objects)")
    return _CircleMatch.apply(x, y, g, c2, item, nbr, visb, float(gamma), float(m), pad == "e0")


ACT_NONE, ACT_RELU, ACT_LEAKY = 0, 1, 2


def affine_act(x, scale, shift, act=ACT_NONE, slope=0.0, res=None, res_scale=None, res_shift=None, inplace=True):
    x = _dev(x, torch.float32, "x")
    B, C = x.shape[0], x.shape[1]
    inner = x.numel() // (B * C)
    if inner % 4 != 0 or B * C > 65535 or x.data_ptr() % 16 != 0:
        y = x * scale.view(1, C, *([1] * (x.dim() - 2))) + shift.view(1, C, *([1] * (x.dim() - 2)))
        if res is not None:
            y = y + (res * res_scale.view_as(scale.view(1, C, *([1] * (x.dim() - 2)))) + res_shift.view(1, C, *([1] * (x.dim() - 2)))
                     if res_scale is not None else res)
        if act == ACT_RELU:
            y = torch.relu(y)
        elif act == ACT_LEAKY:
            y = torch.where(y > 0, y, y * slope)
        return y
    if res is not None:
        res = _dev(res, torch.float32, "res")
        assert res.shape == x.shape
    y = x if inplace else torch.empty_like(x)
    check(_lib.lib().gdm_affine_act_hip(x.data_ptr(), scale.data_ptr(), shift.data_ptr(),
                                        res.data_ptr() if res is not None else None,
                                        res_scale.data_ptr() if res_scale is not None else None,
                                        res_shift.data_ptr() if res_shift is not None else None,
                                        B * C, C, inner, act, float(slope), y.data_ptr(), _stream()), "gdm_affine_act_hip")
    return y


def _pw_seg(spec, B, name):
    x, idx = (spec, None) if torch.is_tensor(spec) else (spec[0], spec[1])
    x = _dev(x, torch.float32, name)
    if x.dim() == 4 and x.shape[3] == 1:
        x = x.reshape(x.shape[0], x.shape[1], x.shape[2])
    if x.dim() != 3 or x.shape[0] != B:
        raise ValueError("pointwise: %s must be [B,C,n(,1)] with B=%d, got %s" % (name, B, tuple(x.shape)))
    n = None
    if idx is not None:
        idx = _idx32(idx, name + " index").reshape(B, -1)
        n = idx.shape[1]
    seg = _lib.PwSeg(x.data_ptr(), idx.data_ptr() if idx is not None else None, x.shape[1], x.shape[2])
    return seg, (x, idx), n


def pointwise(segs, wt, scale=None, shift=None, act=ACT_NONE, slope=0.0, point_major=False, out=None, out_c0=0, w_rowmajor=False):
    if not isinstance(segs, list):
        segs = [segs]
    first = segs[0] if torch.is_tensor(segs[0]) else segs[0][0]
    B = first.shape[0]
    wt = _dev(wt, torch.float32, "wt")
    K, Cout = (wt.shape[1], wt.shape[0]) if w_rowmajor else wt.shape
    if w_rowmajor and K >= 32 and B * first.numel() // max(1, first.shape[0] * first.shape[1]) >= 131072:
        wt, w_rowmajor = wt.t().contiguous(), False
    arr = (_lib.PwSeg * len(segs))()
    keep = []
    n = None
    ksum = 0
    for i, sp in enumerate(segs):
        seg, k, ni = _pw_seg(sp, B, "segment %d" % i)
        arr[i] = seg
        keep.append(k)
        ksum += seg.C
        ni = ni if ni is not None else seg.n_src
        if n is not None and ni != n:
            raise ValueError("pointwise: segments disagree on the number of points (%d vs %d)" % (n, ni))
        n = ni
    if ksum != K:
        raise ValueError("pointwise: weight has %d input rows, the segments %d channels" % (K, ksum))
    if out is None:
        out = torch.empty((B, n, Cout) if point_major else (B, Cout, n), dtype=torch.float32, device=wt.device)
        outC = Cout
    else:
        outC = out.shape[2] if point_major else out.shape[1]
        if not out.is_contiguous() or out.dtype != torch.float32 or out.shape[0] != B or (out.shape[1] if point_major else out.shape[2]) != n:
            raise ValueError("pointwise: out must be a contiguous f32 [B,%s] tensor" % ("n,outC" if point_major else "outC,n"))
    check(_lib.lib().gdm_pointwise2_hip(arr, len(segs), wt.data_ptr(), 1 if w_rowmajor else 0, scale.data_ptr() if scale is not None else None,
                                        shift.data_ptr() if shift is not None else None, B, n, Cout, int(act), float(slope),
                                        out.data_ptr(), outC, int(out_c0), 1 if point_major else 0, _stream()), "gdm_pointwise2_hip")
    return out


def pointwise_chain2(x, p0, p1):
    x = _dev(x, torch.float32, "x")
    B, C0, n = x.shape
    (w0, s0, b0, a0, sl0), (w1, s1, b1, a1, sl1) = p0, p1
    C1, C2 = w0.shape[1], w1.shape[1]
    if w0.shape[0] != C0 or w1.shape[0] != C1:
        raise ValueError("pointwise_chain2: weights %s, %s do not chain from %d channels" % (tuple(w0.shape), tuple(w1.shape), C0))
    y0 = torch.empty((B, C1, n), dtype=torch.float32, device=x.device)
    y1 = torch.empty((B, C2, n), dtype=torch.float32, device=x.device)
    ptr = lambda t: t.data_ptr() if t is not None else None
    check(_lib.lib().gdm_pointwise_chain2_hip(x.data_ptr(), w0.data_ptr(), ptr(s0), ptr(b0), int(a0), float(sl0), w1.data_ptr(), ptr(s1), ptr(b1),
                                              int(a1), float(sl1), B, n, C0, C1, C2, y0.data_ptr(), y1.data_ptr(), _stream()),
          "gdm_pointwise_chain2_hip")
    return y0, y1


def pointwise_jobs(xs, wts):
    if not (1 <= len(xs) <= 4 and len(xs) == len(wts)):
        raise ValueError("pointwise_jobs: one to four (x, wt) pairs")
    B, K = xs[0].shape[0], xs[0].shape[1]
    Cout = wts[0].shape[1]
    arr = (_lib.PwJob * len(xs))()
    keep, outs = [], []
    for j, (x, wt) in enumerate(zip(xs, wts)):
        x = _dev(x.reshape(x.shape[0], x.shape[1], -1), torch.float32, "xs[%d]" % j)
        wt = _dev(wt, torch.float32, "wts[%d]" % j)
        if x.shape[0] != B or x.shape[1] != K or tuple(wt.shape) != (K, Cout):
            raise ValueError("pointwise_jobs: job %d has x %s / wt %s, job 0 has B=%d K=%d Cout=%d" % (j, tuple(x.shape), tuple(wt.shape), B, K, Cout))
        out = torch.empty((B, Cout, x.shape[2]), dtype=torch.float32, device=x.device)
        arr[j] = _lib.PwJob(x.data_ptr(), wt.data_ptr(), out.data_ptr(), x.shape[2])
        keep += [x, wt]
        outs.append(out)
    check(_lib.lib().gdm_pointwise_jobs_hip(arr, len(xs), B, K, Cout, _stream()), "gdm_pointwise_jobs_hip")
    return outs


def _fold_and_all_reduce(sums, C, group):
    import torch.distributed as dist
    compact = torch.cat([sums[:-2].view(-1, 2 * C).sum(0), sums[-2:-1]])
    if dist.get_backend(group) == "nccl":
        dist.all_reduce(compact, group=group)
    else:
        host = compact.cpu()
        dist.all_reduce(host, group=group)
        compact = host.to(sums.device)
    return compact


class _BatchNormAct(torch.autograd.Function):
    @staticmethod
    def forward(ctx, x, weight, bias, running_mean, running_var, eps, momentum, act, slope, group):
        x = _dev(x, torch.float32, "x")
        B, C = x.shape[0], x.shape[1]
        inner = x.numel() // (B * C)
        L = _lib.lib()
        sums = torch.empty(L.gdm_bn_sums_len(B, C, inner), dtype=torch.float64, device=x.device)
        saved = torch.empty(4 * C, dtype=torch.float32, device=x.device)
        y = torch.empty_like(x)
        check(L.gdm_bn_stats_hip(x.data_ptr(), B, C, inner, sums.data_ptr(), _stream()), "gdm_bn_stats_hip")
        groups = 0
        if group is not None:
            sums, groups = _fold_and_all_reduce(sums, C, group), 1
        check(L.gdm_bn_fwd_apply_hip(x.data_ptr(), sums.data_ptr(), groups, weight.data_ptr(), bias.data_ptr(), B, C, inner, float(eps),
                                     float(momentum), act, float(slope), saved.data_ptr(),
                                     running_mean.data_ptr() if running_mean is not None else None,
                                     running_var.data_ptr() if running_var is not None else None, y.data_ptr(), _stream()), "gdm_bn_fwd_apply_hip")
        ctx.save_for_backward(x, weight, saved)
        ctx.act, ctx.slope, ctx.group = act, float(slope), group
        return y

    @staticmethod
    def backward(ctx, go):
        x, weight, saved = ctx.saved_tensors
        go = _dev(go, torch.float32, "grad")
        B, C = x.shape[0], x.shape[1]
        inner = x.numel() // (B * C)
        L = _lib.lib()
        sums = torch.empty(L.gdm_bn_sums_len(B, C, inner), dtype=torch.float64, device=x.device)
        gw = torch.empty(C, dtype=torch.float32, device=x.device)
        gb = torch.empty(C, dtype=torch.float32, device=x.device)
        gx = torch.empty_like(x)
        check(L.gdm_bn_bwd_reduce_hip(x.data_ptr(), go.data_ptr(), saved.data_ptr(), B, C, inner, ctx.act, ctx.slope, sums.data_ptr(), _stream()),
              "gdm_bn_bwd_reduce_hip")
        groups = 0
        local = None
        if ctx.group is not None:
            local = sums[:-2].view(-1, C, 2).sum(0)
            sums, groups = _fold_and_all_reduce(sums, C, ctx.group), 1
        check(L.gdm_bn_bwd_apply_hip(x.data_ptr(), go.data_ptr(), sums.data_ptr(), groups, weight.data_ptr(), saved.data_ptr(), B, C, inner,
                                     ctx.act, ctx.slope, gw.data_ptr(), gb.data_ptr(), gx.data_ptr(), _stream()), "gdm_bn_bwd_apply_hip")
        if local is not None:
            mean, rstd = saved[2 * C:3 * C].double(), saved[3 * C:].double()
            gb = local[:, 0].float()
            gw = (rstd * (local[:, 1] - mean * local[:, 0])).float()
        return gx, gw, gb, None, None, None, None, None, None, None




def _sync_group(bn):
    import torch.distributed as dist
    if not (isinstance(bn, torch.nn.SyncBatchNorm) and dist.is_available() and dist.is_initialized()):
        return None
    group = bn.process_group if bn.process_group is not None else dist.group.WORLD
    return group if dist.get_world_size(group) >= settings.SYNCBN_MIN_WORLD else None


def bn_train_supported(x, bn):
    if not (settings.USE_FUSED_BN_TRAIN and bn.training and x.is_cuda and x.dtype == torch.float32 and x.dim() >= 3 and x.is_contiguous()):
        return False
    if type(bn) not in (torch.nn.BatchNorm1d, torch.nn.BatchNorm2d) and not (settings.USE_FUSED_SYNCBN and type(bn) is torch.nn.SyncBatchNorm):
        return False
    if not bn.affine or bn.momentum is None or not bn.track_running_stats:
        return False
    B, C = x.shape[0], x.shape[1]
    inner = x.numel() // max(B * C, 1)
    return B * C <= 65535 and inner >= 4 and inner % 4 == 0 and x.data_ptr() % 16 == 0 and B * inner > 1


def batch_norm_act_train(x, bn, act=ACT_NONE, slope=0.0):
    y = _BatchNormAct.apply(x, bn.weight, bn.bias, bn.running_mean, bn.running_var, bn.eps, bn.momentum, act, slope, _sync_group(bn))
    if bn.num_batches_tracked is not None:
        if _bn_counters is not None:
            _bn_counters.append(bn.num_batches_tracked)
        else:
            bn.num_batches_tracked.add_(1)
    return y


_bn_counters = None


class batched_bn_counters:

    def __enter__(self):
        global _bn_counters
        self.prev, _bn_counters = _bn_counters, []
        return self

    def __exit__(self, *exc):
        global _bn_counters
        pending, _bn_counters = _bn_counters, self.prev
        if pending:
            torch._foreach_add_(pending, 1)
        return False


def upconv3x3_gather(z, scale, shift, cout, out_size, act=ACT_NONE, slope=0.0, packed=False):
    z = _dev(z, torch.float32, "z")
    B, c9, H, W = z.shape
    assert c9 == 9 * cout
    OH, OW = int(out_size[0]), int(out_size[1])
    out = torch.empty((B, cout, OH, OW), dtype=torch.float32, device=z.device)
    if (packed and (cout == 64 or cout % 128 == 0) and OW % 32 == 0 and (B * OH * OW) % 256 == 0 and B * cout // 8 <= 65535
            and (OH, OW) == (2 * H, 2 * W)):
        opk = PackedAct(_packed_buffer(B, cout, OH, OW, z.device), (B, cout, OH, OW))
        check(_lib.lib().gdm_upconv3x3_gather2_hip(z.data_ptr(), scale.data_ptr(), shift.data_ptr(), B, cout, H, W, OH, OW, act,
                                                   float(slope), out.data_ptr(), opk.buf.data_ptr(), _stream()), "gdm_upconv3x3_gather2_hip")
        out._gdm_packed = opk
        return out
    check(_lib.lib().gdm_upconv3x3_gather_hip(z.data_ptr(), scale.data_ptr(), shift.data_ptr(), B, cout, H, W, OH, OW, act,
                                              float(slope), out.data_ptr(), _stream()), "gdm_upconv3x3_gather_hip")
    return out


def upconv_fused64_pack_weight(weight):
    w = _dev(weight.detach(), torch.float32, "weight")
    if tuple(w.shape) != (64, 64, 3, 3):
        raise ValueError("upconv_fused64_pack_weight: weight must be [64,64,3,3], got %s" % (tuple(w.shape),))
    L = _lib.lib()
    wpk = torch.empty(L.gdm_upconv_fused64_weight_bytes(), dtype=torch.uint8, device=w.device)
    check(L.gdm_upconv_fused64_pack_weight_hip(w.data_ptr(), wpk.data_ptr(), _stream()), "gdm_upconv_fused64_pack_weight_hip")
    return wpk


def upconv_fused64(x, wpk, scale, shift, out_size, act=0, slope=0.0):
    x = _dev(x, torch.float32, "x")
    B, C, H, W = x.shape
    OH, OW = int(out_size[0]), int(out_size[1])
    out = torch.empty((B, C, OH, OW), dtype=torch.float32, device=x.device)
    check(_lib.lib().gdm_upconv_fused64_hip(x.data_ptr(), wpk.data_ptr(), scale.data_ptr(), shift.data_ptr(), B, C, H, W, OH, OW, act,
                                            float(slope), out.data_ptr(), _stream()), "gdm_upconv_fused64_hip")
    return out


class _UpconvGather(torch.autograd.Function):

    @staticmethod
    def forward(ctx, z, bias, cout, OH, OW):
        z = z.contiguous()
        B, c9, H, W = z.shape
        ones = torch.ones(cout, dtype=torch.float32, device=z.device)
        shift = bias.detach().contiguous() if bias is not None else torch.zeros(cout, dtype=torch.float32, device=z.device)
        out = torch.empty((B, cout, OH, OW), dtype=torch.float32, device=z.device)
        check(_lib.lib().gdm_upconv3x3_gather_hip(z.data_ptr(), ones.data_ptr(), shift.data_ptr(), B, cout, H, W, OH, OW, ACT_NONE, 0.0,
                                                  out.data_ptr(), _stream()), "gdm_upconv3x3_gather_hip")
        ctx.shape = (B, cout, H, W, OH, OW)
        ctx.has_bias = bias is not None
        return out

    @staticmethod
    def backward(ctx, go):
        B, cout, H, W, OH, OW = ctx.shape
        go = go.contiguous()
        gz = torch.empty((B, 9 * cout, H, W), dtype=torch.float32, device=go.device)
        check(_lib.lib().gdm_upconv3x3_gather_bwd_hip(go.data_ptr(), B, cout, H, W, OH, OW, gz.data_ptr(), _stream()),
              "gdm_upconv3x3_gather_bwd_hip")
        return gz, (channel_sum(go) if ctx.has_bias else None), None, None, None


def upconv3x3_gather_train(z, bias, cout, out_size):
    z = _dev(z, torch.float32, "z")
    assert z.shape[1] == 9 * cout
    return _UpconvGather.apply(z, bias, cout, int(out_size[0]), int(out_size[1]))


def wx(w2d, x3):
    if torch.is_grad_enabled() and (w2d.requires_grad or x3.requires_grad) and x3.is_cuda and x3.dtype == torch.float32:
        return _WxTrain.apply(x3.contiguous(), w2d.contiguous())
    return torch.bmm(w2d.unsqueeze(0).expand(x3.shape[0], -1, -1), x3)


def _wgrad_parts(nchunk, tiles):
    parts = 1
    for d in range(1, nchunk + 1):
        if nchunk % d == 0 and d * tiles <= 320 and nchunk // d >= 4:
            parts = d
    return parts


def gemm_wgrad_supported(x3, go3):
    B, Cin, P = x3.shape
    return (settings.USE_MFMA_GEMM_TRAIN and x3.is_cuda and x3.dtype == torch.float32 and P % 128 == 0 and Cin % 256 == 0
            and go3.shape[1] >= 64 and 2.0 * B * P * Cin * go3.shape[1] >= 2e9)


def gemm_wgrad(x3, go3):
    x3 = _dev(x3, torch.float32, "x")
    go3 = _dev(go3, torch.float32, "grad_out")
    B, Cin, P = x3.shape
    Cout = go3.shape[1]
    L = _lib.lib()
    nx, ng = L.gdm_wgrad_x1_bytes(B, Cin, P), L.gdm_wgrad_go_bytes(B, Cout, P // 32, 32)
    if nx == 0 or ng == 0 or Cin % 256 != 0:
        raise ValueError("gemm_wgrad: unsupported shape x %s grad_out %s" % (tuple(x3.shape), tuple(go3.shape)))
    xpk = torch.empty(nx, dtype=torch.uint8, device=x3.device)
    gpk = torch.empty(ng, dtype=torch.uint8, device=x3.device)
    check(L.gdm_wgrad_pack_x1_hip(x3.data_ptr(), B, Cin, P, xpk.data_ptr(), _stream()), "gdm_wgrad_pack_x1_hip")
    check(L.gdm_wgrad_pack_go_hip(go3.data_ptr(), B, Cout, P // 32, 32, gpk.data_ptr(), _stream()), "gdm_wgrad_pack_go_hip")
    nchunk = B * P // 128
    parts = _wgrad_parts(nchunk, (Cin // 256) * ((Cout + 127) // 128))
    n = nchunk // parts
    coutp = (Cout + 127) // 128 * 128
    out = torch.empty((parts, Cout, Cin), dtype=torch.float32, device=x3.device)
    check(L.gdm_conv1x1_packed_wb_hip(xpk.data_ptr(), gpk.data_ptr(), n * coutp * 512, parts, 128 * n, Cout, 1, Cin, out.data_ptr(), _stream()),
          "gdm_conv1x1_packed_wb_hip")
    return out[0] if parts == 1 else out.sum(0)


def wgrad_direct_supported(x3, go3, bias=False):
    B, Cin, P = x3.shape
    Cout = go3.shape[1]
    lim = 128 if bias else 64
    return (settings.USE_DIRECT_WGRAD and x3.is_cuda and x3.dtype == torch.float32 and go3.dtype == torch.float32 and P % 32 == 0
            and Cin <= lim and Cout <= lim and B * P >= 16384 and _rows_ok(x3) and _rows_ok(go3))


def _rows_ok(t):
    return t.stride(2) == 1 and t.stride(1) == t.shape[2] and t.stride(0) % 4 == 0 and t.data_ptr() % 16 == 0


def wgrad_direct(x3, go3, bias=False):
    B, Cin, P = x3.shape
    Cout = go3.shape[1]
    nsteps = B * (P // 32)
    bm, bn = (64 if Cout > 32 else 32), (64 if Cin > 32 else 32)
    blocks = -(-Cout // bm) * -(-Cin // bn)
    slices = 4 // ((2 if Cout > 32 else 1) * (2 if Cin > 32 else 1))
    nsplit = max(1, min(nsteps // (8 * slices), 512 // blocks))
    part = torch.empty((nsplit, Cout, Cin), dtype=torch.float32, device=x3.device)
    bpart = torch.empty((nsplit, Cout), dtype=torch.float32, device=x3.device) if bias else None
    check(_lib.lib().gdm_wgrad_direct_hip(go3.data_ptr(), go3.stride(0), x3.data_ptr(), x3.stride(0), B, Cout, Cin, P, nsplit,
                                          part.data_ptr(), bpart.data_ptr() if bias else None, _stream()), "gdm_wgrad_direct_hip")
    return part.sum(0), (bpart.sum(0) if bias else None)


def _gemm_fwd_mfma_ok(cin, cout, n, B):
    return settings.USE_MFMA_GEMM_TRAIN and gemm_supported(cin, cout, n) and 2.0 * B * n * cin * cout >= 2e9


class _WxTrain(torch.autograd.Function):

    @staticmethod
    def forward(ctx, x3, w2):
        ctx.save_for_backward(x3, w2)
        B, Cin, n = x3.shape
        Cout = w2.shape[0]
        if x3.is_cuda and _gemm_fwd_mfma_ok(Cin, Cout, n, B):
            return gemm_bf16x3(x3, gemm_pack_weight(w2), Cout)
        if settings.USE_POINTWISE_TRAIN and x3.is_cuda:
            return pointwise([x3], w2, w_rowmajor=True)
        return torch.bmm(w2.unsqueeze(0).expand(B, -1, -1), x3)

    @staticmethod
    def backward(ctx, go):
        x3, w2 = ctx.saved_tensors
        B, Cin, n = x3.shape
        Cout = w2.shape[0]
        go = go.contiguous()
        gx = gw = None
        if ctx.needs_input_grad[0]:
            if x3.is_cuda and _gemm_fwd_mfma_ok(Cout, Cin, n, B):
                gx = gemm_bf16x3(go, conv_pack_weight_dgrad(w2), Cin)
            elif settings.USE_POINTWISE_TRAIN and x3.is_cuda:
                gx = pointwise([go], w2)
            else:
                gx = torch.bmm(w2.t().unsqueeze(0).expand(B, -1, -1), go)
        if ctx.needs_input_grad[1]:
            if gemm_wgrad_supported(x3, go):
                gw = gemm_wgrad(x3, go)
            elif wgrad_direct_supported(x3, go):
                gw = wgrad_direct(x3, go)[0]
            else:
                gw = torch.bmm(go, x3.transpose(1, 2)).sum(0)
        return gx, gw


class _Conv1x1Train(torch.autograd.Function):

    @staticmethod
    def forward(ctx, x, w2, bias):
        B, Cin = x.shape[0], x.shape[1]
        x3 = x.reshape(B, Cin, -1)
        ctx.save_for_backward(x3, w2)
        ctx.xshape = x.shape
        ctx.has_bias = bias is not None
        y = torch.empty((B, w2.shape[0]) + tuple(x.shape[2:]), dtype=x.dtype, device=x.device)
        y3 = y.view(B, w2.shape[0], -1)
        if settings.USE_POINTWISE_TRAIN and x3.is_cuda and x3.is_contiguous():
            pointwise([x3], w2, None, bias, ACT_NONE, 0.0, out=y3, w_rowmajor=True)
            return y
        torch.bmm(w2.unsqueeze(0).expand(B, -1, -1), x3, out=y3)
        if bias is not None:
            y3 += bias.view(1, -1, 1)
        return y

    @staticmethod
    def backward(ctx, go):
        x3, w2 = ctx.saved_tensors
        B = x3.shape[0]
        go3 = go.reshape(B, w2.shape[0], -1)
        gx = gw = gb = None
        if ctx.needs_input_grad[0]:
            if settings.USE_POINTWISE_TRAIN and go3.is_cuda:
                gx = pointwise([go3.contiguous()], w2).view(ctx.xshape)
            else:
                gx = torch.bmm(w2.t().unsqueeze(0).expand(B, -1, -1), go3).view(ctx.xshape)
        want_gb = ctx.has_bias and ctx.needs_input_grad[2]
        if ctx.needs_input_grad[1] and wgrad_direct_supported(x3, go3, bias=want_gb):
            gw, gb = wgrad_direct(x3, go3, bias=want_gb)
            return gx, gw, gb
        if ctx.needs_input_grad[1]:
            gw = torch.bmm(go3, x3.transpose(1, 2)).sum(0)
        if want_gb:
            gb = go3.sum((0, 2))
        return gx, gw, gb


def conv1x1_train_supported(conv, x):
    return (settings.USE_GEMM_CONV1X1_TRAIN and x.is_cuda and x.dtype == torch.float32 and all(k == 1 for k in conv.kernel_size)
            and all(st == 1 for st in conv.stride) and all(p == 0 for p in conv.padding) and conv.groups == 1 and x.dim() in (3, 4))


def conv1x1_train(conv, x):
    w = conv.weight
    B, Cin = x.shape[0], x.shape[1]
    n = x.numel() // (B * Cin)
    Cout = w.shape[0]
    if x.is_cuda and (_gemm_fwd_mfma_ok(Cin, Cout, n, B) or _gemm_fwd_mfma_ok(Cout, Cin, n, B)):
        y = _WxTrain.apply(x.reshape(B, Cin, n).contiguous(), w.reshape(Cout, Cin).contiguous())
        if conv.bias is not None:
            y = y + conv.bias.view(1, -1, 1)
        return y.view(B, Cout, *x.shape[2:])
    return _Conv1x1Train.apply(x.contiguous(), w.reshape(w.shape[0], w.shape[1]), conv.bias)


def upconv_train_supported(B, cout):
    return B * 9 * cout <= 65535


def psp_combine(g, ys, bias, packed=False):
    g = _dev(g, torch.float32, "g")
    B, C, H, W = g.shape
    ys = [_dev(y, torch.float32, "y") for y in ys]
    assert len(ys) == 4
    opk = None
    if packed and (C == 64 or C % 128 == 0) and W % 32 == 0 and (B * H * W) % 256 == 0 and B * C // 8 <= 65535:
        opk = PackedAct(_packed_buffer(B, C, H, W, g.device), (B, C, H, W))
    check(_lib.lib().gdm_psp_combine2_hip(g.data_ptr(), ys[0].data_ptr(), ys[0].shape[2], ys[1].data_ptr(), ys[1].shape[2],
                                          ys[2].data_ptr(), ys[2].shape[2], ys[3].data_ptr(), ys[3].shape[2],
                                          bias.data_ptr() if bias is not None else None, B, C, H, W, g.data_ptr(),
                                          opk.buf.data_ptr() if opk is not None else None, _stream()), "gdm_psp_combine2_hip")
    if opk is not None:
        g._gdm_packed = opk
    return g


def packed_out_supported(B, C, H, W):
    return (C == 64 or C % 128 == 0) and W % 32 == 0 and (B * H * W) % 256 == 0


def gather_add_affine_act(x, t, idx, scale, shift, act=ACT_NONE, slope=0.0, hw=None, f32_out=True):
    x = _dev(x, torch.float32, "x")
    t = _dev(t, torch.float32, "t")
    idx = _idx32(idx, "idx")
    B, C, m = x.shape
    n = t.shape[2]
    opk = None
    if hw is not None and hw[0] * hw[1] == m and packed_out_supported(B, C, hw[0], hw[1]):
        opk = PackedAct(_packed_buffer(B, C, hw[0], hw[1], x.device), (B, C, hw[0], hw[1]))
    if not f32_out and opk is None:
        raise ValueError("gather_add_affine_act: f32_out=False needs a map the packed operand is built for, got x %s hw %s" % (tuple(x.shape), hw))
    check(_lib.lib().gdm_gather_add_affine_act2_hip(x.data_ptr(), t.data_ptr(), idx.data_ptr(), scale.data_ptr(), shift.data_ptr(),
                                                    B, C, n, m, act, float(slope), x.data_ptr() if f32_out else None,
                                                    opk.buf.data_ptr() if opk is not None else None,
                                                    hw[1] if opk is not None else 0, _stream()),
          "gdm_gather_add_affine_act2_hip")
    if not f32_out:
        return opk
    return (x, opk) if hw is not None else x


def lfa_stage(xyz, idx, feat, w1t, s1, b1, w2t, s2, b2, wft, wmt, sm, bm, slope=0.2):
    xyz = _dev(xyz, torch.float32, "xyz")
    feat = _dev(feat, torch.float32, "feat")
    idx = _idx32(idx, "idx")
    B, n, K = idx.shape
    H = feat.shape[1]
    D, OUT = 2 * H, wmt.shape[1]
    out = torch.empty((B, OUT, n), dtype=torch.float32, device=feat.device)
    z = 0
    check(_lib.lib().gdm_lfa_stage_hip(xyz.data_ptr(), idx.data_ptr(), feat.data_ptr(), w1t.data_ptr(), s1.data_ptr(), b1.data_ptr(),
                                       w2t.data_ptr() if w2t is not None else z, s2.data_ptr() if w2t is not None else z,
                                       b2.data_ptr() if w2t is not None else z, wft.data_ptr(), wmt.data_ptr(), sm.data_ptr(),
                                       bm.data_ptr(), B, n, K, D, OUT, float(slope), out.data_ptr(), _stream()), "gdm_lfa_stage_hip")
    return out


def lfa_supported(d_out, K):
    return K == 16 and d_out in (32, 64, 128, 256)


def conv64_gather_add_act_mfma(x, wpk, t, idx, scale, shift, act=ACT_NONE, slope=0.0, pixel_major=False, t_point_major=False, hw=None):
    x = _dev(x, torch.float32, "x")
    t = _dev(t, torch.float32, "t")
    idx = _idx32(idx, "idx")
    B, C, m = x.shape
    n = t.shape[1] if t_point_major else t.shape[2]
    if C != 64 or t.shape[2 if t_point_major else 1] != 64 or wpk.numel() != 64 * 256:
        raise ValueError("conv64_gather_add_act_mfma: built for 64 -> 64 channels, got x %s t %s" % (tuple(x.shape), tuple(t.shape)))
    y = torch.empty((B, m, C), dtype=torch.float32, device=x.device) if pixel_major else torch.empty_like(x)
    opk = None
    if hw is not None and not pixel_major and hw[0] * hw[1] == m and hw[1] % 32 == 0 and (B * m) % 256 == 0:
        opk = PackedAct(_packed_buffer(B, C, hw[0], hw[1], x.device), (B, C, hw[0], hw[1]))
    check(_lib.lib().gdm_conv64_gather_add_act_mfma2_hip(x.data_ptr(), wpk.data_ptr(), t.data_ptr(), idx.data_ptr(), scale.data_ptr(),
                                                         shift.data_ptr(), B, n, m, act, float(slope), int(bool(pixel_major)),
                                                         int(bool(t_point_major)), y.data_ptr(), opk.buf.data_ptr() if opk is not None else None,
                                                         int(hw[1]) if opk is not None else 0, _stream()), "gdm_conv64_gather_add_act_mfma2_hip")
    if opk is not None:
        y._gdm_packed = opk
    return y


def conv1x1_gather_add_act(x, wt, t, idx, scale, shift, act=ACT_NONE, slope=0.0, pixel_major=False):
    x = _dev(x, torch.float32, "x")
    t = _dev(t, torch.float32, "t")
    wt = _dev(wt, torch.float32, "wt")
    idx = _idx32(idx, "idx")
    B, C, m = x.shape
    if C != 64 or tuple(wt.shape) != (64, 64) or t.shape[1] != 64:
        raise ValueError("conv1x1_gather_add_act: built for 64 -> 64 channels, got x %s wt %s t %s" % (tuple(x.shape), tuple(wt.shape), tuple(t.shape)))
    y = torch.empty((B, m, C), dtype=torch.float32, device=x.device) if pixel_major else torch.empty_like(x)
    check(_lib.lib().gdm_conv1x1_gather_add_act2_hip(x.data_ptr(), wt.data_ptr(), t.data_ptr(), idx.data_ptr(), scale.data_ptr(),
                                                     shift.data_ptr(), B, C, t.shape[2], m, act, float(slope), int(bool(pixel_major)),
                                                     y.data_ptr(), _stream()), "gdm_conv1x1_gather_add_act2_hip")
    return y


def point_heads(a, b, layers, last, feat_layer, res_layer, residual=None):
    import ctypes
    a = _dev(a, torch.float32, "a")
    B, Ca, N = a.shape
    if b is not None:
        b = _dev(b, torch.float32, "b")
        if b.shape[0] != B or b.shape[2] != N or b.shape[1] + Ca != 128:
            raise ValueError("point_heads: a %s + b %s must make 128 channels" % (tuple(a.shape), tuple(b.shape)))
    elif Ca != 128:
        raise ValueError("point_heads: a must have 128 channels when b is None, got %d" % Ca)
    n = len(layers)
    vp, fp = ctypes.c_void_p, ctypes.c_void_p
    w_arr = (vp * n)(*[l[0].data_ptr() for l in layers])
    sc_arr = (fp * n)(*[(l[1].data_ptr() if l[1] is not None else None) for l in layers])
    sh_arr = (fp * n)(*[(l[2].data_ptr() if l[2] is not None else None) for l in layers])
    act_arr = (ctypes.c_int * n)(*[int(l[3]) for l in layers])
    for l in layers:
        if l[3] not in (ACT_NONE, ACT_RELU):
            raise ValueError("point_heads: activations are none / ReLU")
    wl, bl, c_last = last if last is not None else (None, None, 0)
    out_feat = torch.empty((B, 128, N), dtype=torch.float32, device=a.device) if feat_layer >= 0 else None
    out_last = torch.empty((B, int(c_last), N), dtype=torch.float32, device=a.device) if c_last else None
    ra, rb = (None, None)
    if residual is not None:
        ra = _dev(residual[0], torch.float32, "residual")
        rb = _dev(residual[1], torch.float32, "residual") if residual[1] is not None else None
        if ra.shape[0] != B or ra.shape[2] != N or ra.shape[1] + (rb.shape[1] if rb is not None else 0) != 128:
            raise ValueError("point_heads: the residual source must make 128 channels of the same points")
    check(_lib.lib().gdm_point_heads2_hip(a.data_ptr(), b.data_ptr() if b is not None else None, Ca,
                                          ra.data_ptr() if ra is not None else None, rb.data_ptr() if rb is not None else None,
                                          ra.shape[1] if ra is not None else 0, B, N, n, w_arr, sc_arr, sh_arr, act_arr,
                                          int(feat_layer), int(res_layer), wl.data_ptr() if wl is not None else None,
                                          bl.data_ptr() if bl is not None else None, int(c_last),
                                          out_feat.data_ptr() if out_feat is not None else None,
                                          out_last.data_ptr() if out_last is not None else None, _stream()), "gdm_point_heads2_hip")
    return out_feat, out_last


def pack_rows64(w2d):
    w = _dev(w2d.detach(), torch.float32, "w")
    if w.dim() != 2 or w.shape[1] != 64:
        raise ValueError("pack_rows64: expected [R,64], got %s" % (tuple(w.shape),))
    out = torch.empty(w.shape[0] * 256, dtype=torch.uint8, device=w.device)
    check(_lib.lib().gdm_pack_rows64_hip(w.data_ptr(), w.shape[0], out.data_ptr(), _stream()), "gdm_pack_rows64_hip")
    return out


def upconv_final_points(x_pm, hw, choose, wpk, scale, shift, act, slope, wf_pk, fbias, out_size):
    x_pm = _dev(x_pm, torch.float32, "x_pm")
    choose = _idx32(choose, "choose")
    B = x_pm.shape[0]
    H, W = int(hw[0]), int(hw[1])
    if tuple(x_pm.shape) != (B, H * W, 64):
        raise ValueError("upconv_final_points: x_pm must be [B,H*W,64] with (H, W) = %s, got %s" % ((H, W), tuple(x_pm.shape)))
    choose = choose.reshape(B, -1)
    N = choose.shape[1]
    OH, OW = int(out_size[0]), int(out_size[1])
    out = torch.empty((B, 64, N), dtype=torch.float32, device=x_pm.device)
    check(_lib.lib().gdm_upconv_final_points_hip(x_pm.data_ptr(), choose.data_ptr(), wpk.data_ptr(), scale.data_ptr(), shift.data_ptr(),
                                                 act, float(slope), wf_pk.data_ptr(), fbias.data_ptr() if fbias is not None else None,
                                                 B, H, W, OH, OW, N, out.data_ptr(), _stream()), "gdm_upconv_final_points_hip")
    return out




def stem_pack_weight(weight):
    w = _dev(weight.detach(), torch.float32, "weight")
    if tuple(w.shape) != (64, 3, 7, 7):
        raise ValueError("stem_pack_weight: the stem kernel is built for a [64,3,7,7] filter, got %s" % (tuple(w.shape),))
    L = _lib.lib()
    wpk = torch.empty(L.gdm_stem_weight_bytes(), dtype=torch.uint8, device=w.device)
    check(L.gdm_stem_pack_weight_hip(w.data_ptr(), wpk.data_ptr(), _stream()), "gdm_stem_pack_weight_hip")
    return wpk


def stem(x, wpk, scale, shift, packed=True):
    x = _dev(x, torch.float32, "x")
    B, C, H, W = x.shape
    if C != 3:
        raise ValueError("stem: 3 input channels, got %d" % C)
    PH, PW = ((H - 1) // 2) // 2 + 1, ((W - 1) // 2) // 2 + 1
    out = torch.empty((B, 64, PH, PW), dtype=torch.float32, device=x.device)
    opk = None
    if packed and (B * PH * PW) % 256 == 0 and PW % 16 == 0:
        opk = PackedAct(_packed_buffer(B, 64, PH, PW, x.device), (B, 64, PH, PW))
    check(_lib.lib().gdm_stem_hip(x.data_ptr(), wpk.data_ptr(), scale.data_ptr(), shift.data_ptr(), B, H, W, out.data_ptr(),
                                  opk.buf.data_ptr() if opk is not None else None, _stream()), "gdm_stem_hip")
    if opk is not None:
        out._gdm_packed = opk
    return out


def affine_relu_maxpool(x, scale, shift):
    x = _dev(x, torch.float32, "x")
    B, C, H, W = x.shape
    y = torch.empty((B, C, (H - 1) // 2 + 1, (W - 1) // 2 + 1), dtype=torch.float32, device=x.device)
    check(_lib.lib().gdm_affine_relu_maxpool_hip(x.data_ptr(), scale.data_ptr(), shift.data_ptr(), B, C, H, W, y.data_ptr(), _stream()),
          "gdm_affine_relu_maxpool_hip")
    return y


def _final_weight_t(weight):
    key = (weight._version, weight.data_ptr())
    cache = getattr(weight, "_gdm_final_wt", None)
    if cache is None or cache[0] != key:
        C = weight.shape[0]
        cache = (key, weight.detach().reshape(C, C).t().contiguous())
        weight._gdm_final_wt = cache
    return cache[1]


def conv1x1_logsoftmax(x, weight, bias):
    x = _dev(x, torch.float32, "x")
    B, C, H, W = x.shape
    w = _final_weight_t(weight)
    out = torch.empty_like(x)
    check(_lib.lib().gdm_conv1x1_logsoftmax_hip(x.data_ptr(), w.data_ptr(), bias.data_ptr() if bias is not None else None,
                                                B, C, H * W, out.data_ptr(), _stream()), "gdm_conv1x1_logsoftmax_hip")
    return out


def conv64_gather_add_final(x, wpk, t, idx, scale, shift, act, slope, final_weight, final_bias):
    x = _dev(x, torch.float32, "x")
    t = _dev(t, torch.float32, "t")
    idx = _idx32(idx, "idx")
    B, C, m = x.shape
    if C != 64 or t.dim() != 3 or t.shape[2] != 64 or wpk.numel() != 64 * 256 or final_weight.numel() != 64 * 64:
        raise ValueError("conv64_gather_add_final: built for 64 -> 64 -> 64 channels, got x %s t %s final %s"
                         % (tuple(x.shape), tuple(t.shape), tuple(final_weight.shape)))
    wft = _final_weight_t(final_weight)
    out = torch.empty_like(x)
    check(_lib.lib().gdm_conv64_gather_add_final_hip(x.data_ptr(), wpk.data_ptr(), t.data_ptr(), idx.data_ptr(), scale.data_ptr(),
                                                     shift.data_ptr(), B, t.shape[1], m, act, float(slope), wft.data_ptr(),
                                                     final_bias.data_ptr() if final_bias is not None else None, out.data_ptr(),
                                                     _stream()), "gdm_conv64_gather_add_final_hip")
    return out


def channel_sum(t):
    B, C = t.shape[0], t.shape[1]
    inner = t.numel() // max(B * C, 1)
    if not (t.is_cuda and t.dtype == torch.float32 and t.is_contiguous() and B * C <= 65535 and inner >= 4 and inner % 4 == 0
            and t.data_ptr() % 16 == 0):
        return t.sum(dim=[0] + list(range(2, t.dim())))
    L = _lib.lib()
    sums = torch.empty(L.gdm_bn_sums_len(B, C, inner), dtype=torch.float64, device=t.device)
    check(L.gdm_bn_stats_hip(t.data_ptr(), B, C, inner, sums.data_ptr(), _stream()), "gdm_bn_stats_hip")
    return sums[:-2].view(-1, C, 2)[:, :, 0].sum(0).float()


class _PspPools(torch.autograd.Function):
    @staticmethod
    def forward(ctx, x):
        x = _dev(x, torch.float32, "x")
        B, C, H, W = x.shape
        outs = [torch.empty((B, C, s_, s_), dtype=torch.float32, device=x.device) for s_ in (1, 2, 3, 6)]
        check(_lib.lib().gdm_psp_pools_hip(x.data_ptr(), B * C, H, W, outs[0].data_ptr(), outs[1].data_ptr(), outs[2].data_ptr(),
                                           outs[3].data_ptr(), _stream()), "gdm_psp_pools_hip")
        ctx.shape = (B, C, H, W)
        return tuple(outs)

    @staticmethod
    def backward(ctx, g1, g2, g3, g6):
        B, C, H, W = ctx.shape
        gs = [_dev(g, torch.float32, "grad") for g in (g1, g2, g3, g6)]
        gx = torch.empty((B, C, H, W), dtype=torch.float32, device=gs[0].device)
        check(_lib.lib().gdm_psp_pools_bwd_hip(gs[0].data_ptr(), gs[1].data_ptr(), gs[2].data_ptr(), gs[3].data_ptr(), B * C, H, W,
                                               gx.data_ptr(), _stream()), "gdm_psp_pools_bwd_hip")
        return gx


def psp_pools_supported(h, w):
    return 36 <= h * w <= 4096 and h >= 6 and w >= 6


def psp_pools(x):
    return list(_PspPools.apply(x))


class _PspCombine(torch.autograd.Function):

    @staticmethod
    def forward(ctx, g, bias, y1, y2, y3, y4):
        g = _dev(g, torch.float32, "g")
        ys = [_dev(y, torch.float32, "y") for y in (y1, y2, y3, y4)]
        B, C, H, W = g.shape
        out = torch.empty_like(g)
        check(_lib.lib().gdm_psp_combine2_hip(g.data_ptr(), ys[0].data_ptr(), ys[0].shape[2], ys[1].data_ptr(), ys[1].shape[2],
                                              ys[2].data_ptr(), ys[2].shape[2], ys[3].data_ptr(), ys[3].shape[2],
                                              bias.data_ptr() if bias is not None else None, B, C, H, W, out.data_ptr(), None, _stream()),
              "gdm_psp_combine2_hip")
        ctx.save_for_backward(out)
        ctx.sizes = [y.shape[2] for y in ys]
        ctx.has_bias = bias is not None
        return out

    @staticmethod
    def backward(ctx, go):
        (out,) = ctx.saved_tensors
        B, C, H, W = out.shape
        gpre = torch.where(out > 0, go, torch.zeros((), dtype=go.dtype, device=go.device)).contiguous()
        gys = []
        L = _lib.lib()
        for s_ in ctx.sizes:
            gy = torch.empty((B, C, s_, s_), dtype=torch.float32, device=go.device)
            check(L.gdm_upsample_bilinear_bwd_hip(gpre.data_ptr(), B * C, s_, s_, H, W, gy.data_ptr(), _stream()), "gdm_upsample_bilinear_bwd_hip")
            gys.append(gy)
        gb = channel_sum(gpre) if ctx.has_bias else None
        return gpre, gb, gys[0], gys[1], gys[2], gys[3]


def psp_combine_train(g, ys, bias):
    assert len(ys) == 4
    return _PspCombine.apply(g, bias, ys[0], ys[1], ys[2], ys[3])


class BufferPool:

    def __init__(self):
        self.packed = {}
        self.workspace = {}


_default_pool = BufferPool()
_pool = _default_pool
_warned_capture = []


class buffer_pool:
    def __init__(self, pool):
        self.pool, self.prev = pool, None

    def __enter__(self):
        global _pool
        self.prev, _pool = _pool, self.pool
        return self.pool

    def __exit__(self, *exc):
        global _pool
        _pool = self.prev
        return False


def _capturing_unscoped():
    if _pool is _default_pool and torch.cuda.is_current_stream_capturing():
        if not _warned_capture:
            _warned_capture.append(1)
            import warnings
            warnings.warn("geometric_aware_dense_matching_amd.ops: hipGraph capture outside ops.buffer_pool(...): scratch buffers "
                          "are allocated per call inside the graph; give the capture a BufferPool of its own")
        return True
    return False




def conv3x3_wgrad_supported(x, go):
    B, Cin, H, W = x.shape
    return (settings.USE_MFMA_WGRAD and x.is_cuda and x.dtype == torch.float32 and go.shape[0] == B and tuple(go.shape[2:]) == (H, W)
            and W in (32, 64) and (H * W) % 128 == 0 and Cin % 256 == 0 and go.shape[1] % 8 == 0)


def conv3x3_wgrad(x, go, parts=None):
    x = _dev(x, torch.float32, "x")
    go = _dev(go, torch.float32, "grad_out")
    B, Cin, H, W = x.shape
    Cout = go.shape[1]
    L = _lib.lib()
    nx, ng = L.gdm_wgrad_x_bytes(B, Cin, H, W), L.gdm_wgrad_go_bytes(B, Cout, H, W)
    if nx == 0 or ng == 0 or (9 * Cin) % 256 != 0:
        raise ValueError("conv3x3_wgrad: unsupported shape x %s grad_out %s" % (tuple(x.shape), tuple(go.shape)))
    xpk = torch.empty(nx, dtype=torch.uint8, device=x.device)
    gpk = torch.empty(ng, dtype=torch.uint8, device=x.device)
    check(L.gdm_wgrad_pack_x_hip(x.data_ptr(), B, Cin, H, W, xpk.data_ptr(), _stream()), "gdm_wgrad_pack_x_hip")
    check(L.gdm_wgrad_pack_go_hip(go.data_ptr(), B, Cout, H, W, gpk.data_ptr(), _stream()), "gdm_wgrad_pack_go_hip")
    nchunk = B * H * W // 128
    if parts is None:
        tiles = (9 * Cin // 256) * ((Cout + 127) // 128)
        parts = 1
        for d in range(1, nchunk + 1):
            if nchunk % d == 0 and d * tiles <= 320 and nchunk // d >= 4:
                parts = d
    if nchunk % parts != 0:
        raise ValueError("conv3x3_wgrad: %d parts do not divide the %d chunks of the contraction" % (parts, nchunk))
    n = nchunk // parts
    coutp = (Cout + 127) // 128 * 128
    out = torch.empty((parts, Cout, 9, Cin), dtype=torch.float32, device=x.device)
    check(L.gdm_conv1x1_packed_wb_hip(xpk.data_ptr(), gpk.data_ptr(), n * coutp * 512, parts, 128 * n, Cout, 9, Cin, out.data_ptr(), _stream()),
          "gdm_conv1x1_packed_wb_hip")
    dw = out[0] if parts == 1 else out.sum(0)
    return dw.view(Cout, 3, 3, Cin).permute(0, 3, 1, 2).contiguous()


def conv3x3_supported(x, weight, stride=(1, 1), padding=(1, 1), dilation=(1, 1)):
    cin = weight.shape[1]
    st = tuple(stride)
    if st not in ((1, 1), (2, 2)):
        return False
    return (x.is_cuda and x.dtype == torch.float32 and x.dim() == 4 and tuple(weight.shape[2:]) == (3, 3)
            and tuple(padding) == (1, 1) and tuple(dilation) == (1, 1)
            and x.shape[2] % st[0] == 0 and x.shape[3] % st[1] == 0 and (x.shape[3] // st[1]) % 32 == 0
            and (cin == 64 or cin % 128 == 0) and weight.shape[0] % 8 == 0 and x.shape[0] <= 65535)


def conv_pack_weight_dgrad(weight):
    weight = _dev(weight.detach(), torch.float32, "weight")
    Cout, Cin = weight.shape[0], weight.shape[1]
    taps = 9 if weight.dim() == 4 else 1
    L = _lib.lib()
    nbytes = L.gdm_conv3x3_weight_bytes(Cin, Cout) if taps == 9 else L.gdm_conv1x1_weight_bytes(Cin, Cout)
    wpk = torch.empty(nbytes, dtype=torch.uint8, device=weight.device)
    check(L.gdm_conv_pack_weight_dgrad_hip(weight.data_ptr(), Cout, Cin, taps, wpk.data_ptr(), _stream()), "gdm_conv_pack_weight_dgrad_hip")
    return wpk


def conv3x3_pack_weight(weight):
    weight = _dev(weight.detach(), torch.float32, "weight")
    Cout, Cin = weight.shape[0], weight.shape[1]
    L = _lib.lib()
    wpk = torch.empty(L.gdm_conv3x3_weight_bytes(Cout, Cin), dtype=torch.uint8, device=weight.device)
    check(L.gdm_conv3x3_pack_weight_hip(weight.data_ptr(), Cout, Cin, wpk.data_ptr(), _stream()), "gdm_conv3x3_pack_weight_hip")
    return wpk


class PackedAct:
    __slots__ = ("buf", "shape")

    def __init__(self, buf, shape):
        self.buf, self.shape = buf, tuple(shape)


def _packed_buffer(B, C, H, W, device, avoid=None):
    nbytes = _lib.lib().gdm_conv3x3_act_bytes(B, C, H, W)
    if _capturing_unscoped():
        return torch.zeros(nbytes, dtype=torch.uint8, device=device)
    key = (B, C, H, W, device.index, _stream_lane(device))
    pool = _pool.packed.setdefault(key, [])
    for buf in pool:
        if avoid is None or buf.data_ptr() != avoid.data_ptr():
            return buf
    buf = torch.zeros(nbytes, dtype=torch.uint8, device=device)
    pool.append(buf)
    return buf


def conv3x3_pack_act(x):
    x = _dev(x, torch.float32, "x")
    B, C, H, W = x.shape
    buf = _packed_buffer(B, C, H, W, x.device)
    check(_lib.lib().gdm_conv3x3_pack_act_hip(x.data_ptr(), B, C, H, W, buf.data_ptr(), _stream()), "gdm_conv3x3_pack_act_hip")
    return PackedAct(buf, (B, C, H, W))


def conv3x3_bf16x3(x, wpk, cout, scale=None, shift=None, act=ACT_NONE, res=None, out_f32=True, out_packed=False, stride=1):
    xp = x if isinstance(x, PackedAct) else conv3x3_pack_act(x)
    B, Cin, H, W = xp.shape
    if stride != 1:
        if stride != 2 or H % 2 or W % 2:
            raise ValueError("conv3x3_bf16x3: stride %r on a %dx%d map" % (stride, H, W))
        H, W = H // 2, W // 2
    L = _lib.lib()
    dev = xp.buf.device
    out = torch.empty((B, cout, H, W), dtype=torch.float32, device=dev) if out_f32 else None
    opk = None
    if out_packed:
        if (B * H * W) % 256 != 0 or cout % 8 != 0:
            raise ValueError("conv3x3_bf16x3: packed output needs B*H*W %% 256 == 0 and Cout %% 8 == 0")
        opk = PackedAct(_packed_buffer(B, cout, H, W, dev, avoid=xp.buf), (B, cout, H, W))
    if res is not None:
        res = _dev(res, torch.float32, "res")
        assert tuple(res.shape) == (B, cout, H, W)
    check(L.gdm_conv3x3_strided_hip(xp.buf.data_ptr(), wpk.data_ptr(), scale.data_ptr() if scale is not None else None,
                                    shift.data_ptr() if shift is not None else None, res.data_ptr() if res is not None else None,
                                    B, Cin, cout, H, W, int(stride), act, out.data_ptr() if out is not None else None,
                                    opk.buf.data_ptr() if opk is not None else None, _stream()), "gdm_conv3x3_strided_hip")
    return (out, opk) if out_packed else out


def gemm_bf16x3_map(x, wpk, cout):
    B, Cin, H, W = x.shape
    if isinstance(x, PackedAct):
        if W % 32 != 0:
            raise ValueError("gemm_bf16x3_map: a packed-only map needs W %% 32 == 0, got %s" % (x.shape,))
        return conv1x1_packed2d(x, wpk, cout)
    xp = getattr(x, "_gdm_packed", None)
    if isinstance(xp, PackedAct) and xp.shape == (B, Cin, H, W) and W % 32 == 0:
        return conv1x1_packed2d(xp, wpk, cout)
    return gemm_bf16x3(x.reshape(B, Cin, H * W), wpk, cout).view(B, cout, H, W)


def conv1x1_packed2d(xp, wpk, cout, scale=None, shift=None, act=ACT_NONE, stride=1):
    B, Cin, H, W = xp.shape
    if stride not in (1, 2) or H % stride or W % stride:
        raise ValueError("conv1x1_packed2d: stride %r on a %dx%d map" % (stride, H, W))
    H, W = H // stride, W // stride
    out = torch.empty((B, cout, H, W), dtype=torch.float32, device=xp.buf.device)
    check(_lib.lib().gdm_conv1x1_strided_hip(xp.buf.data_ptr(), wpk.data_ptr(), scale.data_ptr() if scale is not None else None,
                                             shift.data_ptr() if shift is not None else None, B, Cin, cout, H, W, int(stride), act,
                                             out.data_ptr(), _stream()), "gdm_conv1x1_strided_hip")
    return out


class _Conv3x3Train(torch.autograd.Function):
    @staticmethod
    def forward(ctx, x, weight):
        ctx.save_for_backward(x, weight)
        return conv3x3_bf16x3(x, conv3x3_pack_weight(weight), weight.shape[0])

    @staticmethod
    def backward(ctx, go):
        x, weight = ctx.saved_tensors
        go = _dev(go, torch.float32, "grad")
        gx = gw = None
        if ctx.needs_input_grad[0]:
            gx = conv3x3_bf16x3(go, conv_pack_weight_dgrad(weight), weight.shape[1])
        if ctx.needs_input_grad[1]:
            if conv3x3_wgrad_supported(x, go):
                gw = conv3x3_wgrad(x, go)
            else:
                gw = torch.ops.aten.convolution_backward(go, x, weight, None, [1, 1], [1, 1], [1, 1], False, [0, 0], 1, [False, True, False])[1]
        return gx, gw


def conv3x3_train(x, weight):
    return _Conv3x3Train.apply(x, weight)


def gemm_supported(cin, cout, npix):
    return (cin % 128 == 0 or cin == 64) and (cout % 128 == 0 or cout >= 192) and npix % 32 == 0


def gemm_pack_weight(weight2d):
    w = _dev(weight2d.detach(), torch.float32, "weight")
    Cout, Cin = w.shape
    L = _lib.lib()
    wpk = torch.empty(L.gdm_conv1x1_weight_bytes(Cout, Cin), dtype=torch.uint8, device=w.device)
    check(L.gdm_conv1x1_pack_weight_hip(w.data_ptr(), Cout, Cin, wpk.data_ptr(), _stream()), "gdm_conv1x1_pack_weight_hip")
    return wpk


def gemm_bf16x3(x, wpk, cout, scale=None, shift=None, act=ACT_NONE, pixel_major=False):
    x = _dev(x, torch.float32, "x")
    B, Cin, n = x.shape
    L = _lib.lib()
    xpk = _packed_buffer(B, Cin, 1, n, x.device)
    check(L.gdm_conv3x3_pack_act_hip(x.data_ptr(), B, Cin, 1, n, xpk.data_ptr(), _stream()), "gdm_conv3x3_pack_act_hip")
    out = torch.empty((B * n, cout) if pixel_major else (B, cout, n), dtype=torch.float32, device=x.device)
    check(L.gdm_conv1x1_packed_hip(xpk.data_ptr(), wpk.data_ptr(), scale.data_ptr() if scale is not None else None,
                                   shift.data_ptr() if shift is not None else None, B, Cin, cout, 1, n, act,
                                   1 if pixel_major else 0, out.data_ptr(), _stream()), "gdm_conv1x1_packed_hip")
    return out


def spline_packed_buffer(C, M, device, avoid=None):
    return _packed_buffer(1, C, 1, M, device, avoid=avoid)


def gemm_grouped(x_cm, wpk, rowidx, tile_co0, cout_total, xpk=None):
    x_cm = _dev(x_cm, torch.float32, "x")
    _, Cin, M = x_cm.shape
    R = rowidx.shape[0]
    L = _lib.lib()
    if xpk is None:
        xpk = _packed_buffer(1, Cin, 1, M, x_cm.device)
        check(L.gdm_conv3x3_pack_act_hip(x_cm.data_ptr(), 1, Cin, 1, M, xpk.data_ptr(), _stream()), "gdm_conv3x3_pack_act_hip")
    Y = torch.empty((R, 128), dtype=torch.float32, device=x_cm.device)
    check(L.gdm_gemm_grouped_hip(xpk.data_ptr(), wpk.data_ptr(), rowidx.data_ptr(), tile_co0.data_ptr(), R, M, Cin, cout_total,
                                 Y.data_ptr(), _stream()), "gdm_gemm_grouped_hip")
    return Y


class _UpsampleBilinear(torch.autograd.Function):
    @staticmethod
    def forward(ctx, x, OH, OW):
        x = _dev(x, torch.float32, "x")
        B, C, H, W = x.shape
        out = torch.empty((B, C, OH, OW), dtype=torch.float32, device=x.device)
        check(_lib.lib().gdm_upsample_bilinear_hip(x.data_ptr(), B * C, H, W, OH, OW, out.data_ptr(), _stream()),
              "gdm_upsample_bilinear_hip")
        ctx.hw = (H, W)
        return out

    @staticmethod
    def backward(ctx, go):
        go = go.contiguous()
        B, C, OH, OW = go.shape
        H, W = ctx.hw
        g = torch.empty((B, C, H, W), dtype=torch.float32, device=go.device)
        check(_lib.lib().gdm_upsample_bilinear_bwd_hip(go.data_ptr(), B * C, H, W, OH, OW, g.data_ptr(), _stream()),
              "gdm_upsample_bilinear_bwd_hip")
        return g, None, None


class _PReLU1(torch.autograd.Function):
    @staticmethod
    def forward(ctx, x, slope):
        x = x.contiguous()
        y = torch.empty_like(x)
        check(_lib.lib().gdm_prelu1_hip(x.data_ptr(), slope.data_ptr(), x.numel(), y.data_ptr(), _stream()), "gdm_prelu1_hip")
        ctx.save_for_backward(x, slope)
        return y

    @staticmethod
    def backward(ctx, go):
        x, slope = ctx.saved_tensors
        go = go.contiguous()
        gx = torch.empty_like(x)
        gs = torch.zeros_like(slope)
        check(_lib.lib().gdm_prelu1_bwd_hip(x.data_ptr(), go.data_ptr(), slope.data_ptr(), x.numel(), gx.data_ptr(), gs.data_ptr(), _stream()),
              "gdm_prelu1_bwd_hip")
        return gx, gs


def prelu1(x, slope):
    x = _dev(x, torch.float32, "x")
    return _PReLU1.apply(x, slope)


def upsample_bilinear(x, size):
    return _UpsampleBilinear.apply(x, int(size[0]), int(size[1]))


def _workspace(nbytes, device):
    if _capturing_unscoped():
        return torch.empty(max(int(nbytes), 16), dtype=torch.uint8, device=device)
    key = (device.index, _stream_lane(device))
    ws = _pool.workspace.get(key)
    if ws is None or ws.numel() < nbytes:
        ws = torch.empty(nbytes, dtype=torch.uint8, device=device)
        _pool.workspace[key] = ws
    return ws


def match(scene, model, precision=MATCH_BF16X3, return_sim=False):
    scene = _dev(scene, torch.float32, "scene")
    model = _dev(model, torch.float32, "model")
    if model.dim() == 3:
        assert model.shape[0] == 1
        model = model[0]
    B, D, N = scene.shape
    M = model.shape[1]
    assert model.shape[0] == D
    L = _lib.lib()
    nbytes = L.gdm_match_workspace_bytes(B, N, M)
    ws = _workspace(nbytes, scene.device)
    best_idx = torch.empty((B, N), dtype=torch.int32, device=scene.device)
    best_sim = torch.empty((B, N), dtype=torch.float32, device=scene.device)
    sim = torch.empty((B, N, M), dtype=torch.float32, device=scene.device) if return_sim else None
    check(L.gdm_match_hip(scene.data_ptr(), model.data_ptr(), B, D, N, M, precision, best_idx.data_ptr(),
                          best_sim.data_ptr(), sim.data_ptr() if return_sim else None, ws.data_ptr(), ws.numel(),
                          _stream()), "gdm_match_hip")
    return (best_idx, best_sim, sim) if return_sim else (best_idx, best_sim)


def match_pack(x, precision=MATCH_BF16X3, out=None):
    x = _dev(x, torch.float32, "x")
    if x.dim() == 2:
        x = x.unsqueeze(0)
    R, D, n = x.shape
    L = _lib.lib()
    if out is None:
        out = torch.empty((L.gdm_match_rows_bytes(R * n),), dtype=torch.uint8, device=x.device)
    check(L.gdm_match_pack_hip(x.data_ptr(), R, D, n, precision, out.data_ptr(), _stream()), "gdm_match_pack_hip")
    return out


def match_pack2(x1, x2, precision=MATCH_BF16X3):
    x1 = _dev(x1, torch.float32, "x1")
    x2 = _dev(x2, torch.float32, "x2")
    x1 = x1.unsqueeze(0) if x1.dim() == 2 else x1
    x2 = x2.unsqueeze(0) if x2.dim() == 2 else x2
    (R1, D, n1), (R2, D2, n2) = x1.shape, x2.shape
    if D != D2:
        raise ValueError("match_pack2: %d vs %d channels" % (D, D2))
    L = _lib.lib()
    o1 = torch.empty((L.gdm_match_rows_bytes(R1 * n1),), dtype=torch.uint8, device=x1.device)
    o2 = torch.empty((L.gdm_match_rows_bytes(R2 * n2),), dtype=torch.uint8, device=x1.device)
    check(L.gdm_match_pack2_hip(x1.data_ptr(), R1, n1, o1.data_ptr(), x2.data_ptr(), R2, n2, o2.data_ptr(), D, precision, _stream()),
          "gdm_match_pack2_hip")
    return o1, o2


def match_packed(scene_rows, model_rows, B, N, M, precision=MATCH_BF16X3, return_sim=False, sim_out=None):
    L = _lib.lib()
    dev = scene_rows.device
    part = _workspace(L.gdm_match_partial_bytes(B, N), dev)
    best_idx = torch.empty((B, N), dtype=torch.int32, device=dev)
    best_sim = torch.empty((B, N), dtype=torch.float32, device=dev)
    sim = None
    if return_sim:
        sim = sim_out if sim_out is not None else torch.empty((B, N, M), dtype=torch.float32, device=dev)
    check(L.gdm_match_packed_hip(scene_rows.data_ptr(), model_rows.data_ptr(), B * N, M, precision, best_idx.data_ptr(),
                                 best_sim.data_ptr(), sim.data_ptr() if return_sim else None, part.data_ptr(), part.numel(),
                                 _stream()), "gdm_match_packed_hip")
    return (best_idx, best_sim, sim) if return_sim else (best_idx, best_sim)


def seg_mask(seg):
    seg = _dev(seg, torch.float32, "seg")
    B, two, N = seg.shape
    assert two == 2
    mask = torch.empty((B, N), dtype=torch.uint8, device=seg.device)
    count = torch.empty((B,), dtype=torch.int32, device=seg.device)
    check(_lib.lib().gdm_seg_mask_hip(seg.data_ptr(), B, N, mask.data_ptr(), count.data_ptr(), _stream()),
          "gdm_seg_mask_hip")
    return mask, count
```

include/gdm.h:

```cpp
#ifndef GDM_H
#define GDM_H

#include <stddef.h>
#include <stdint.h>

#ifdef __cplusplus
extern "C" {
#endif

#define GDM_EINVAL (-1)
#define GDM_ENOMEM (-2)

const char* gdm_last_error(void);
int gdm_version(void);


void gdm_knn_batch(const float* batch_data, size_t batch_size, size_t npts, size_t dim,
                   const float* queries, size_t nqueries, size_t K, long* batch_indices);

int gdm_knn_batch_hip(const float* support, const float* query, int B, int S, int Q, int K,
                      int32_t* idx, float* d2, void* stream);

typedef struct gdm_knn_job {
    const float* support;
    const float* query;
    int32_t* idx;
    float* d2;
    int64_t support_bstride;
    int64_t query_bstride;
    int32_t S, Q, K;
    int32_t grid_w;
} gdm_knn_job;
#define GDM_KNN_MAX_JOBS 32
size_t gdm_knn_jobs_workspace_bytes(const gdm_knn_job* jobs, int njobs, int B);
int gdm_knn_jobs_ws_hip(const gdm_knn_job* jobs, int njobs, int B, void* workspace, size_t workspace_bytes, void* stream);

int gdm_ballquery_hip(int B, int n, int m, float radius, int nsample,
                      const float* new_xyz, const float* xyz, int32_t* idx, void* stream);

int gdm_furthestsampling_hip(int B, int n, int m, const float* xyz, float* temp, int32_t* idx, void* stream);

int gdm_interpolation_forward_hip(int B, int c, int m, int n, const float* feat, const int32_t* idx, const float* weight, float* out, void* stream);
int gdm_interpolation_backward_hip(int B, int c, int n, int m, const float* grad_out, const int32_t* idx, const float* weight,
                                   float* grad_feat, void* stream);

int gdm_labelstat_ballrange_hip(int B, int n, int m, float radius, int nclass, const float* new_xyz, const float* xyz,
                                const int32_t* label_stat, int32_t* new_label_stat, void* stream);
int gdm_labelstat_idx_hip(int B, int n, int m, int nsample, int nclass, const int32_t* label_stat, const int32_t* idx,
                          int32_t* new_label_stat, void* stream);


int gdm_group_gather_hip(const float* feat, const int32_t* idx, int B, int C, int n, int m, int K,
                         float* out, void* stream);
int gdm_group_gather_bwd2_hip(const float* grad_out, long go_bstride, const int32_t* idx, int B, int C, int n, int m, int K,
                              float* grad_feat, void* stream);

int gdm_gather_max_hip(const float* feat, const int32_t* idx, int B, int C, int n, int m, int K,
                       float* out, int32_t* arg, void* stream);
int gdm_gather_max_bwd_hip(const float* grad_out, const int32_t* arg, int B, int C, int n, int m,
                           float* grad_feat, void* stream);

int gdm_rel_pos_enc_hip(const float* xyz, const int32_t* idx, int B, int n, int K, float* out, void* stream);

int gdm_att_pool_hip(const float* att, const float* feat, int B, int C, int n, int K, float* out, void* stream);
int gdm_att_pool_bwd_hip(const float* att, const float* feat, const float* grad_out, int B, int C, int n, int K,
                         float* grad_att, float* grad_feat, void* stream);


#define GDM_MATCH_BF16X3 0
#define GDM_MATCH_F32    1

size_t gdm_match_workspace_bytes(int B, int N, int M);

int gdm_match_hip(const float* scene, const float* model, int B, int D, int N, int M, int precision,
                  int32_t* best_idx, float* best_sim, float* sim,
                  void* workspace, size_t workspace_bytes, void* stream);

size_t gdm_match_rows_bytes(int rows);
size_t gdm_match_partial_bytes(int B, int N);
int gdm_match_pack_hip(const float* x, int R, int D, int n, int precision, void* rows, void* stream);
int gdm_match_pack2_hip(const float* x1, int R1, int n1, void* rows1, const float* x2, int R2, int n2, void* rows2,
                        int D, int precision, void* stream);
int gdm_match_packed_hip(const void* scene_rows, const void* model_rows, int R , int M, int precision,
                         int32_t* best_idx, float* best_sim, float* sim,
                         void* partial, size_t partial_bytes, void* stream);

int gdm_seg_mask_hip(const float* seg, int B, int N, uint8_t* mask, int32_t* count, void* stream);

int gdm_spline_aggregate_hip(const float* xw, const int32_t* rowptr, const int32_t* src, const float* attr,
                             const float* root, const float* bias, int M, int C, int kernel_size, int relu,
                             float* out, void* stream);
int gdm_spline_aggregate_bwd_hip(const float* grad_out, const int32_t* rowptr, const int32_t* src, const float* attr,
                                 int M, int C, int kernel_size, float* grad_xw, void* stream);
int gdm_spline_direct3_hip(const float* x, const float* weight, const int32_t* rowptr, const int32_t* src, const float* attr,
                           const float* root_t, const float* bias, int M, int Cin, int C, int kernel_size, int relu,
                           float* out, float* out_t, void* out_packed, void* stream);
int gdm_gemm_grouped_hip(const void* xpk, const void* wpk, const int32_t* rowidx, const int32_t* tile_co0, int R, int M,
                         int Cin, int Cout_total, float* out, void* stream);
int gdm_spline_pairs_aggregate3_hip(const float* Y, const int32_t* rowptr, const int32_t* pos, const float* basis,
                                    const float* root, const float* bias, int M, int C, int relu, float* out, float* out_t,
                                    void* out_packed, void* stream);

int gdm_upsample_bilinear_hip(const float* in, long planes, int H, int W, int OH, int OW, float* out, void* stream);
int gdm_upsample_bilinear_bwd_hip(const float* grad_out, long planes, int H, int W, int OH, int OW, float* grad_in, void* stream);

int gdm_topk_rows_hip(const float* score, long rows, int n, int K, int32_t* idx, float* val, void* stream);
int gdm_topk_negdist_hip(const float* gram, const float* xx, int B, int n, int K, int32_t* idx, void* stream);
int gdm_edge_feature_hip(const float* x, const int32_t* idx, int B, int C, int n, int K, float* out, void* stream);
int gdm_edge_feature_bwd_hip(const float* grad_out, const int32_t* idx, int B, int C, int n, int K, float* grad_x, void* stream);

int gdm_circle_rows_fwd_hip(const float* sim, int R, int Mp, const int32_t* match, const int32_t* item,
                            const float* xyz, const uint8_t* vis, float radius, float gamma, float m,
                            float* lse_p, float* lse_n, float* loss, void* stream);
int gdm_circle_rows_bwd_hip(const float* sim, int R, int Mp, const int32_t* match, const int32_t* item,
                            const float* xyz, const uint8_t* vis, float radius, float gamma, float m,
                            const float* lse_p, const float* lse_n, const float* grad_rows, float* dsim, void* stream);

size_t gdm_circle_match_rows_bytes(int n);
size_t gdm_circle_match_tp_bytes(int n);
int gdm_circle_match_pack_hip(const float* x, int n, void* rows, void* tp, float* rowsum, void* stream);
int gdm_circle_match_nbr_hip(const float* xyz, int M, float radius, uint32_t* nbr, void* stream);
int gdm_circle_match_visbits_hip(const uint8_t* vis, int B, int M, uint32_t* bits, void* stream);
int gdm_circle_match_nbr_items_hip(const float* xyz, int M, const float* rad , int B, uint32_t* nbr, void* stream);
int gdm_circle_match_fwd2_hip(const void* xrows, const void* xtp, const float* xpad, const void* yrows, const void* ytp,
                              int R, int M, const int32_t* g, const int32_t* c2, const int32_t* item,
                              const uint32_t* nbr, int nbr_per_item, const uint32_t* visb, int pad_e0, float gamma, float m,
                              float* lse_p, float* lse_n, float* loss, void* stream);
int gdm_circle_match_bwd2_hip(const void* xrows, const void* xtp, const float* xpad, const void* yrows, const void* ytp,
                              int R, int M, const int32_t* g, const int32_t* c2, const int32_t* item,
                              const uint32_t* nbr, int nbr_per_item, const uint32_t* visb, int pad_e0, float gamma, float m,
                              const float* lse_p, const float* lse_n, const float* coef, float* gx, float* gy_part, void* stream);
int gdm_circle_match_bwd_parts(int R, int M);

int gdm_lfa_stage_hip(const float* xyz, const int32_t* idx, const float* feat, const float* w1t, const float* s1, const float* b1,
                      const float* w2t, const float* s2, const float* b2, const float* wft, const float* wmt, const float* sm,
                      const float* bm, int B, int n, int K, int D, int OUT, float slope, float* out, void* stream);

int gdm_kabsch_stats_hip(const float* scene_xyz, long scene_bstride, int pt_stride, int ch_stride, const float* model_xyz,
                         const int32_t* best_idx, const uint8_t* mask, int B, int N, int M, double* out, void* stream);

int gdm_kabsch_solve_hip(const double* stats, int B, int min_points, float* RT, uint8_t* valid, void* stream);

#define GDM_RANSAC_MAX_H 4096
size_t gdm_ransac_workspace_bytes(int B, int N, int H);
int gdm_ransac_pose_hip(const float* scene_xyz, long scene_bstride, int pt_stride, int ch_stride, const float* model_xyz,
                        const int32_t* best_idx, const uint8_t* mask, const double* stats, int B, int N, int M, int H,
                        float match_err, double fix_percent, uint32_t seed, int min_points, void* workspace, size_t workspace_bytes,
                        float* RT, uint8_t* valid, int32_t* counts, int32_t* winner, void* stream);

int gdm_icp_transform_hip(const float* scene_xyz, long scene_bstride, int pt_stride, int ch_stride, const float* RT, int B, int N,
                          float* query, void* stream);
int gdm_icp_update_hip(const float* scene_xyz, long scene_bstride, int pt_stride, int ch_stride, const float* model_xyz,
                       const int32_t* nn, const float* d2, const uint8_t* mask, int B, int N, int M, float reject_dist,
                       double tolerance, int min_points, float* RT, uint8_t* active, int32_t* iters, double* err, void* stream);

#define GDM_TARGETS_MIN_M 4
size_t gdm_targets_workspace_bytes(int B, int N, int M);
int gdm_hpr_visible_hip(const float* model_xyz, long model_bstride, const float* RT, const float* cam_center, int B, int M,
                        void* workspace, size_t workspace_bytes, double* flipped, uint8_t* visible, void* stream);
int gdm_pose_targets_hip(const float* cld, long cld_bstride, int pt_stride, int ch_stride, const uint8_t* labels, const float* RT,
                         const float* model_xyz, long model_bstride, const uint8_t* visible, int B, int N, int M, double dist_thresh,
                         void* workspace, size_t workspace_bytes, uint8_t* labels_out, int32_t* match_idx, uint8_t* visible_flag,
                         uint8_t* valid, void* stream);

int gdm_affine_act_maxk_hip(const float* x, const float* scale, const float* shift, long planes, int C, long n, int K, int act,
                            float slope, float* out, void* stream);

int gdm_prelu1_hip(const float* x, const float* slope, long n, float* y, void* stream);
int gdm_prelu1_bwd_hip(const float* x, const float* grad_out, const float* slope, long n, float* grad_x, float* grad_slope, void* stream);

int gdm_affine_act_hip(const float* x, const float* scale, const float* shift, const float* res, const float* res_scale,
                       const float* res_shift, long planes, int C, long inner, int act, float slope, float* y, void* stream);

int gdm_upconv3x3_gather_hip(const float* z, const float* scale, const float* shift, int B, int Cout, int H, int W,
                             int OH, int OW, int act, float slope, float* out, void* stream);
int gdm_upconv3x3_gather2_hip(const float* z, const float* scale, const float* shift, int B, int Cout, int H, int W,
                              int OH, int OW, int act, float slope, float* out, void* outpk, void* stream);
int gdm_upconv3x3_gather_bwd_hip(const float* grad_out, int B, int Cout, int H, int W, int OH, int OW, float* grad_z, void* stream);
size_t gdm_upconv_fused64_weight_bytes(void);
int gdm_upconv_fused64_pack_weight_hip(const float* w, void* wpk, void* stream);
int gdm_upconv_fused64_hip(const float* x, const void* wpk, const float* scale, const float* shift, int B, int C, int H, int W,
                           int OH, int OW, int act, float slope, float* out, void* stream);

int gdm_psp_combine2_hip(const float* g, const float* y1, int s1, const float* y2, int s2, const float* y3, int s3,
                         const float* y4, int s4, const float* bias, int B, int C, int H, int W, float* out, void* outpk, void* stream);
int gdm_gather_add_affine_act2_hip(const float* x, const float* t, const int32_t* idx, const float* scale, const float* shift,
                                   int B, int C, int n, int m, int act, float slope, float* y, void* y_packed, int W, void* stream);
int gdm_conv1x1_gather_add_act2_hip(const float* x, const float* wt, const float* t, const int32_t* idx, const float* scale,
                                    const float* shift, int B, int C, int n, long m, int act, float slope, int pixel_major,
                                    float* y, void* stream);
int gdm_conv64_gather_add_act_mfma2_hip(const float* x, const void* wpk, const float* t, const int32_t* idx, const float* scale,
                                        const float* shift, int B, int n, long m, int act, float slope, int pixel_major,
                                        int t_point_major, float* y, void* ypk, int W, void* stream);
int gdm_conv64_gather_add_final_hip(const float* x, const void* wpk, const float* t, const int32_t* idx, const float* scale,
                                    const float* shift, int B, int n, long m, int act, float slope, const float* wft,
                                    const float* fbias, float* out, void* stream);

size_t gdm_conv3x3_act_bytes(int B, int Cin, int H, int W);
size_t gdm_conv3x3_weight_bytes(int Cout, int Cin);
int gdm_conv3x3_pack_weight_hip(const float* w, int Cout, int Cin, void* wpk, void* stream);
int gdm_conv3x3_pack_act_hip(const float* x, int B, int Cin, int H, int W, void* xpk, void* stream);
int gdm_conv3x3_packed_hip(const void* xpk, const void* wpk, const float* scale, const float* shift, const float* res,
                           int B, int Cin, int Cout, int H, int W, int act, float* out, void* stream);
int gdm_conv3x3_strided_hip(const void* xpk, const void* wpk, const float* scale, const float* shift, const float* res,
                            int B, int Cin, int Cout, int H, int W, int stride, int act, float* out, void* outpk, void* stream);
int gdm_conv1x1_strided_hip(const void* xpk, const void* wpk, const float* scale, const float* shift,
                            int B, int Cin, int Cout, int H, int W, int stride, int act, float* out, void* stream);

int gdm_affine_relu_maxpool_hip(const float* x, const float* scale, const float* shift, int B, int C, int H, int W, float* y, void* stream);
int gdm_conv1x1_logsoftmax_hip(const float* x, const float* w, const float* bias, int B, int C, long hw, float* out, void* stream);
int gdm_pack_rows64_hip(const float* w, int R, void* out, void* stream);
int gdm_upconv_final_points_hip(const float* xpm, const int32_t* choose, const void* wpk, const float* scale, const float* shift,
                                int act, float slope, const void* wfpk, const float* fbias, int B, int H, int W, int OH, int OW,
                                int N, float* out, void* stream);
int gdm_psp_pools_hip(const float* x, long planes, int H, int W, float* o1, float* o2, float* o3, float* o6, void* stream);
int gdm_psp_pools_bwd_hip(const float* g1, const float* g2, const float* g3, const float* g6, long planes, int H, int W,
                          float* grad_x, void* stream);

size_t gdm_conv1x1_weight_bytes(int Cout, int Cin);
int gdm_conv1x1_pack_weight_hip(const float* w, int Cout, int Cin, void* wpk, void* stream);
int gdm_conv_pack_weight_dgrad_hip(const float* w, int Cout, int Cin, int taps, void* wpk, void* stream);
int gdm_conv1x1_packed_hip(const void* xpk, const void* wpk, const float* scale, const float* shift,
                           int B, int Cin, int Cout, int H, int W, int act, int pixel_major, float* out, void* stream);

int gdm_depth_to_xyz_hip(const float* depth, const float* K, const int32_t* origin, int B, int H, int W, int S,
                         float* out, void* stream);

#define GDM_NORMALS_MAX_K 64
int gdm_depth_normals_hip(const float* depth, const float* K, int B, int H, int W, int k_size, int distance_threshold,
                          int difference_threshold, float* normals, void* stream);

int gdm_warp_crop_hip(const uint8_t* rgb, const float* depth, const float* normals, const float* K, const uint8_t* mask,
                      const float* center, const float* scale, int B, int H, int W, int S, float* out_rgb, float* out_normals,
                      float* out_xyz, float* out_depth, uint8_t* out_mask, void* stream);

#define GDM_FILL_MULTISCALE 0
#define GDM_FILL_FAST 1
#define GDM_FILL_STAGES 7
size_t gdm_fill_depth_workspace_bytes(int B, int H, int W, int mode);
int gdm_fill_depth_hip(const float* depth, int B, int H, int W, int mode, float max_depth, void* workspace, size_t workspace_bytes,
                       float* out, float* stages, void* stream);

long gdm_bn_sums_len(int B, int C, long inner);
int gdm_bn_stats_hip(const float* x, int B, int C, long inner, double* sums, void* stream);
int gdm_bn_fwd_apply_hip(const float* x, const double* sums, int groups, const float* weight, const float* bias, int B, int C, long inner, float eps,
                         float momentum, int act, float slope, float* saved, float* running_mean, float* running_var, float* y, void* stream);
int gdm_bn_bwd_reduce_hip(const float* x, const float* grad_out, const float* saved, int B, int C, long inner, int act, float slope,
                          double* sums, void* stream);
int gdm_bn_bwd_apply_hip(const float* x, const float* grad_out, const double* sums, int groups, const float* weight, const float* saved, int B, int C,
                         long inner, int act, float slope, float* grad_weight, float* grad_bias, float* grad_x, void* stream);

int gdm_point_heads2_hip(const float* a, const float* b, int Ca, const float* ra, const float* rb, int rCa, int B, int N, int nlayer,
                         const void* const* w, const float* const* scale, const float* const* shift, const int* act, int feat_layer,
                         int res_layer, const void* w_last, const float* shift_last, int c_last, float* out_feat, float* out_last,
                         void* stream);

typedef struct {
    const float* x;
    const int32_t* idx;
    int32_t C, n_src;
} gdm_pw_seg;
int gdm_pointwise2_hip(const gdm_pw_seg* segs, int nseg, const float* wt, int w_rowmajor, const float* scale, const float* shift,
                       int B, int n, int Cout, int act, float slope, float* out, int out_C, int out_c0, int point_major, void* stream);
typedef struct {
    const float* x;
    const float* wt;
    float* out;
    int32_t n;
} gdm_pw_job;
int gdm_pointwise_jobs_hip(const gdm_pw_job* jobs, int njobs, int B, int K, int Cout, void* stream);
int gdm_pointwise_chain2_hip(const float* x, const float* w0t, const float* s0, const float* b0, int act0, float slope0,
                             const float* w1t, const float* s1, const float* b1, int act1, float slope1,
                             int B, int n, int C0, int C1, int C2, float* y0, float* y1, void* stream);

size_t gdm_stem_weight_bytes(void);
int gdm_stem_pack_weight_hip(const float* w, void* wpk, void* stream);
int gdm_stem_hip(const float* x, const void* wpk, const float* scale, const float* shift, int B, int H, int W, float* out,
                 void* out_packed, void* stream);

size_t gdm_wgrad_x_bytes(int B, int Cin, int H, int W);
size_t gdm_wgrad_go_bytes(int B, int Cout, int H, int W);
int gdm_wgrad_pack_x_hip(const float* x, int B, int Cin, int H, int W, void* out, void* stream);
int gdm_wgrad_pack_go_hip(const float* go, int B, int Cout, int H, int W, void* out, void* stream);
size_t gdm_wgrad_x1_bytes(int B, int Cin, int P);
int gdm_wgrad_pack_x1_hip(const float* x, int B, int Cin, int P, void* out, void* stream);
int gdm_mfma_probe_hip(int blocks, int iters, int chain, float* sink, void* stream);
int gdm_mfma_probe_lds_hip(int blocks, int iters, int rpu, float* sink, void* stream);
int gdm_wgrad_direct_hip(const float* go, long go_bstride, const float* x, long x_bstride, int B, int Cout, int Cin, int P,
                         int nsplit, float* partial, float* bias_partial, void* stream);
int gdm_conv1x1_packed_wb_hip(const void* xpk, const void* wpk, long w_bstride, int B, int Cin, int Cout, int H, int W, float* out,
                              void* stream);

typedef struct gdm_copy_job {
    void* dst;
    const void* src;
    int64_t sb, s1, s2;
    int32_t B, R1, R2, E;
} gdm_copy_job;
#define GDM_COPY_MAX_JOBS 16
int gdm_copy_jobs_hip(const gdm_copy_job* jobs , int njobs, void* stream);

#ifdef __cplusplus
}
#endif
#endif
```

Measured before the change: 5220.

## Unify conv tile selection with shape-driven picker and explicit tile override API

Replaces the ad-hoc macro-based launch paths for 3x3 and 1x1 convs with one templated dispatcher. A shape-driven picker chooses among 144x256, 128x256, 64x256 and 64x128-pixel tile forms, and new entry points let callers force a specific tile. It also enables the global-to-LDS direct load path for four-wave workgroups with a swizzled offset, and declares two workgroups per CU in the launch bounds. Tile selection heuristics shift, for example the 144-channel tile becomes eligible for 3x3... no, only for 1x1; these shifts may change occupancy and register pressure, and the launch-bounds change could cause spills.

```diff
diff --git a/geometric_aware_dense_matching_amd/_lib.py b/geometric_aware_dense_matching_amd/_lib.py
--- a/geometric_aware_dense_matching_amd/_lib.py
+++ b/geometric_aware_dense_matching_amd/_lib.py
@@ -128,6 +128,8 @@
     "gdm_conv1x1_pack_weight_hip": (_i, [_vp, _i, _i, _vp, _vp]),
     "gdm_conv_pack_weight_dgrad_hip": (_i, [_vp, _i, _i, _i, _vp, _vp]),
     "gdm_conv1x1_packed_hip": (_i, [_vp, _vp, _vp, _vp, _i, _i, _i, _i, _i, _i, _i, _vp, _vp]),
+    "gdm_conv3x3_packed_tile_hip": (_i, [_vp, _vp, _vp, _vp, _vp, _i, _i, _i, _i, _i, _i, _i, _vp, _vp, _i, _vp]),
+    "gdm_conv1x1_packed_tile_hip": (_i, [_vp, _vp, _vp, _vp, _i, _i, _i, _i, _i, _i, _i, _i, _vp, _i, _vp]),
     "gdm_depth_to_xyz_hip": (_i, [_vp, _vp, _vp, _i, _i, _i, _i, _vp, _vp]),
     "gdm_depth_normals_hip": (_i, [_vp, _vp, _i, _i, _i, _i, _i, _i, _vp, _vp]),
     "gdm_warp_crop_hip": (_i, [_vp, _vp, _vp, _vp, _vp, _vp, _vp, _i, _i, _i, _i, _vp, _vp, _vp, _vp, _vp, _vp]),
diff --git a/geometric_aware_dense_matching_amd/csrc/gdm_conv.hip b/geometric_aware_dense_matching_amd/csrc/gdm_conv.hip
--- a/geometric_aware_dense_matching_amd/csrc/gdm_conv.hip
+++ b/geometric_aware_dense_matching_amd/csrc/gdm_conv.hip
@@ -102,11 +102,9 @@
 constexpr int MF_WPIX = 16 * MF_NPH;
 constexpr int MF_WAVES = CV_PIX / MF_WPIX;
 constexpr int MF_THREADS = MF_WAVES * 64;
-constexpr int MF_TSTRIDE = 132;
-constexpr int MF_SMEM = 2 * CV_PANEL > CV_PIX * MF_TSTRIDE * 4 ? 2 * CV_PANEL : CV_PIX * MF_TSTRIDE * 4;
 
 template <int ACT, bool HAS_RES, int TAPS = 9, bool PIXMAJOR = false, int NKS = 8, int NCB = 8, int WV = MF_WAVES>
-__global__ __launch_bounds__(MF_THREADS) void conv_mfma16_kernel(const unsigned char* __restrict__ xpk, const unsigned char* __restrict__ wpk,
+__global__ __launch_bounds__(WV * 64, 2) void conv_mfma16_kernel(const unsigned char* __restrict__ xpk, const unsigned char* __restrict__ wpk,
                                                                  const float* __restrict__ scale, const float* __restrict__ shift,
                                                                  const float* __restrict__ res, int B, int Cin, int Cout, int H, int W,
                                                                  float* __restrict__ out, const int32_t* __restrict__ rowidx = nullptr,
@@ -122,6 +120,7 @@
     constexpr int TST = NCB * 16 + 4;
     static_assert(NCB == 8 || (NCB == 4 && !PIXMAJOR) || (NCB == 9 && !PIXMAJOR && WV == 8),
                   "64-channel tiles: NCHW / packed output only; 144-channel tiles: NCHW fp32 output only (no packed output: a tile straddles 128-channel chunks)");
+    static_assert(WV == 8 || (WV == 4 && NCB == 4 && !PIXMAJOR), "four-wave workgroups: 64-channel tiles only");
     constexpr int NPH = MF_NPH;
     const int tid = threadIdx.x, lane = tid & 63;
     const int wave = __builtin_amdgcn_readfirstlane(tid >> 6);
@@ -192,8 +191,8 @@
             *reinterpret_cast<u32x4*>(base + swz(g >> 5, g & 31)) = stage[i];
         }
     };
-    constexpr bool GLDS = GDM_CONV_GLDS && WV == 8;
-    constexpr int NPIECE = PANEL / 1024 / 8;
+    constexpr bool GLDS = GDM_CONV_GLDS;
+    constexpr int NPIECE = PANEL / 1024 / WV;
     int glds_voff = 0;
     if (GLDS) {
         const int hrow = lane >> 5, sl = lane & 31;
@@ -204,7 +203,8 @@
     auto stage_glds = [&](int src, int buf) {
 #pragma unroll
         for (int i = 0; i < NPIECE; ++i)
-            __builtin_amdgcn_raw_ptr_buffer_load_lds(wr, (lds_void_ptr)(smem + buf * PANEL + (i * 8 + wave) * 1024), 16, glds_voff, src + i * 8192, 0, 0);
+            __builtin_amdgcn_raw_ptr_buffer_load_lds(wr, (lds_void_ptr)(smem + buf * PANEL + (i * WV + wave) * 1024), 16,
+                                                     glds_voff ^ (((2 * WV * i) & 15) << 4), src + i * WV * 1024, 0, 0);
     };
 
     f32x4 acc[NPH][NCB];
@@ -381,7 +381,7 @@
 }
 
 #define CONV_KERNEL conv_mfma16_kernel
-constexpr int CONV_THREADS = MF_THREADS, CONV_WPIX = MF_WPIX, CONV_SMEM = MF_SMEM;
+constexpr int CONV_THREADS = MF_THREADS, CONV_WPIX = MF_WPIX;
 
 }
 
@@ -463,9 +463,90 @@
 
 static bool cin_ok(int Cin) { return Cin == 64 || (Cin >= 128 && Cin % 128 == 0); }
 
-static bool narrow_tiles(unsigned pixel_tiles, int Cout)
-{
-    return Cout <= 64 || (long)pixel_tiles * ((Cout + 127) / 128) < 256;
+static const int TILE_FORMS[] = {144256, 128256, 64256, 64128};
+
+struct ConvShape { int taps, B, Cin, Cout, H, W, stride, pixel_major; };
+
+static long conv_ptot(const ConvShape& c) { return (long)c.B * c.H * c.W; }
+
+static bool tile_allowed(const ConvShape& c, int tile)
+{
+    const int ch = tile / 1000, px = tile % 1000;
+    bool known = false;
+    for (int t : TILE_FORMS) known = known || t == tile;
+    if (!known) return false;
+    if (ch == 144) return c.taps == 1 && c.Cin != 64 && !c.pixel_major && c.stride == 1 && c.Cout % 144 == 0 && GDM_CONV_GLDS;
+    if (ch == 64 && c.pixel_major) return false;
+    return px == 256 || conv_ptot(c) % px == 0;
+}
+
+static long tile_grid(const ConvShape& c, int tile) { return gdm_cdiv(conv_ptot(c), tile % 1000) * gdm_cdiv(c.Cout, tile / 1000); }
+
+static int conv_pick_tile(const ConvShape& c)
+{
+    const long ptiles = gdm_cdiv(conv_ptot(c), 256);
+    if (tile_allowed(c, 144256)) {
+        const long r128 = gdm_cdiv(ptiles * gdm_cdiv(c.Cout, 128), 256) * 128, r144 = gdm_cdiv(ptiles * (c.Cout / 144), 256) * 144;
+        if (r144 < r128) return 144256;
+    }
+    if (c.pixel_major || (c.Cout > 64 && tile_grid(c, 128256) >= 256)) return 128256;
+    return (tile_grid(c, 64256) < 256 && tile_allowed(c, 64128)) ? 64128 : 64256;
+}
+
+struct ConvArgs {
+    const unsigned char* xpk; const unsigned char* wpk; const float* scale; const float* shift; const float* res;
+    int B, Cin, Cout, H, W; float* out; unsigned char* outpk; int stride;
+};
+
+template <int ACT, bool RES, int TAPS, bool PM, int NKS, int NCB, int WV>
+static void conv_go(const ConvArgs& a, hipStream_t s)
+{
+    constexpr int PANEL2 = 2 * NCB * 16 * ROWB, TILE = WV * MF_WPIX * (NCB * 16 + 4) * 4;
+    constexpr int SMEM = ((TAPS == 9 || NCB == 9) && TILE > PANEL2) ? TILE : PANEL2;
+    static bool attr = false;
+    if (!attr) {
+        (void)hipFuncSetAttribute((const void*)CONV_KERNEL<ACT, RES, TAPS, PM, NKS, NCB, WV>, hipFuncAttributeMaxDynamicSharedMemorySize, SMEM);
+        attr = true;
+    }
+    const dim3 grid(gdm_cdiv((long)a.B * a.H * a.W, WV * MF_WPIX), gdm_cdiv(a.Cout, NCB * 16));
+    hipLaunchKernelGGL((CONV_KERNEL<ACT, RES, TAPS, PM, NKS, NCB, WV>), grid, dim3(WV * 64), SMEM, s, a.xpk, a.wpk, a.scale, a.shift, a.res,
+                       a.B, a.Cin, a.Cout, a.H, a.W, a.out, (const int32_t*)nullptr, (const int32_t*)nullptr, a.outpk, a.stride);
+}
+
+template <int TAPS, bool PM, int NKS, int NCB, int WV>
+static void conv_epi(const ConvArgs& a, int act, hipStream_t s)
+{
+    if constexpr (TAPS == 9) {
+        if (act == 0) { if (a.res) conv_go<0, true, TAPS, PM, NKS, NCB, WV>(a, s); else conv_go<0, false, TAPS, PM, NKS, NCB, WV>(a, s); }
+        else { if (a.res) conv_go<1, true, TAPS, PM, NKS, NCB, WV>(a, s); else conv_go<1, false, TAPS, PM, NKS, NCB, WV>(a, s); }
+    } else {
+        if (act == 0) conv_go<0, false, TAPS, PM, NKS, NCB, WV>(a, s); else conv_go<1, false, TAPS, PM, NKS, NCB, WV>(a, s);
+    }
+}
+
+template <int TAPS, int NCB, int WV>
+static void conv_tile(const ConvArgs& a, int act, int pixel_major, hipStream_t s)
+{
+    if constexpr (NCB == 9) {
+        conv_epi<TAPS, false, 8, NCB, WV>(a, act, s);
+    } else {
+        if (a.Cin == 64) { conv_epi<TAPS, false, 4, NCB, WV>(a, act, s); return; }
+        if constexpr (TAPS == 1 && NCB == 8) {
+            if (pixel_major) { conv_epi<TAPS, true, 8, NCB, WV>(a, act, s); return; }
+        }
+        conv_epi<TAPS, false, 8, NCB, WV>(a, act, s);
+    }
+}
+
+template <int TAPS>
+static void conv_dispatch(int tile, const ConvArgs& a, int act, int pixel_major, hipStream_t s)
+{
+    switch (tile) {
+    case 144256: if constexpr (TAPS == 1) conv_tile<TAPS, 9, 8>(a, act, pixel_major, s); break;
+    case 128256: conv_tile<TAPS, 8, 8>(a, act, pixel_major, s); break;
+    case 64256: conv_tile<TAPS, 4, 8>(a, act, pixel_major, s); break;
+    default: conv_tile<TAPS, 4, 4>(a, act, pixel_major, s); break;
+    }
 }
 
 extern "C" size_t gdm_conv3x3_act_bytes(int B, int Cin, int H, int W)
@@ -521,23 +602,30 @@
 }
 
 static int conv3x3_launch(const void* xpk, const void* wpk, const float* scale, const float* shift, const float* res,
-                          int B, int Cin, int Cout, int H, int W, int stride, int act, float* out, void* outpk, void* stream,
+                          int B, int Cin, int Cout, int H, int W, int stride, int act, float* out, void* outpk, int tile, void* stream,
                           const char* who);
 
 extern "C" int gdm_conv3x3_packed_hip(const void* xpk, const void* wpk, const float* scale, const float* shift, const float* res,
                                       int B, int Cin, int Cout, int H, int W, int act, float* out, void* stream)
 {
-    return conv3x3_launch(xpk, wpk, scale, shift, res, B, Cin, Cout, H, W, 1, act, out, nullptr, stream, "gdm_conv3x3_packed_hip");
+    return conv3x3_launch(xpk, wpk, scale, shift, res, B, Cin, Cout, H, W, 1, act, out, nullptr, 0, stream, "gdm_conv3x3_packed_hip");
 }
 
 extern "C" int gdm_conv3x3_strided_hip(const void* xpk, const void* wpk, const float* scale, const float* shift, const float* res,
                                        int B, int Cin, int Cout, int H, int W, int stride, int act, float* out, void* outpk, void* stream)
 {
-    return conv3x3_launch(xpk, wpk, scale, shift, res, B, Cin, Cout, H, W, stride, act, out, outpk, stream, "gdm_conv3x3_strided_hip");
+    return conv3x3_launch(xpk, wpk, scale, shift, res, B, Cin, Cout, H, W, stride, act, out, outpk, 0, stream, "gdm_conv3x3_strided_hip");
+}
+
+extern "C" int gdm_conv3x3_packed_tile_hip(const void* xpk, const void* wpk, const float* scale, const float* shift, const float* res,
+                                           int B, int Cin, int Cout, int H, int W, int stride, int act, float* out, void* outpk, int tile,
+                                           void* stream)
+{
+    return conv3x3_launch(xpk, wpk, scale, shift, res, B, Cin, Cout, H, W, stride, act, out, outpk, tile, stream, "gdm_conv3x3_packed_tile_hip");
 }
 
 static int conv3x3_launch(const void* xpk, const void* wpk, const float* scale, const float* shift, const float* res,
-                          int B, int Cin, int Cout, int H, int W, int stride, int act, float* out, void* outpk, void* stream,
+                          int B, int Cin, int Cout, int H, int W, int stride, int act, float* out, void* outpk, int tile, void* stream,
                           const char* who)
 {
     GDM_CHECK_ARG(stride == 1 || stride == 2, "%s: stride=%d (1 or 2)", who, stride);
@@ -548,68 +636,11 @@
     GDM_CHECK_ARG(act == 0 || act == 1, "%s: act=%d", who, act);
     GDM_CHECK_ARG(!outpk || (Cout % 8 == 0 && ((long)B * H * W) % CV_PIX == 0),
                   "%s: packed output needs Cout %% 8 == 0 and B*H*W %% 256 == 0 (got Cout=%d, B*H*W=%ld)", who, Cout, (long)B * H * W);
-    const long ptot = (long)B * H * W;
-    dim3 grid(gdm_cdiv(ptot, CV_PIX), gdm_cdiv(Cout, CV_CO));
-    hipStream_t s = (hipStream_t)stream;
-    constexpr int SMEM = CONV_SMEM;
-    static bool attr = false;
-    if (!attr) {
-        (void)hipFuncSetAttribute((const void*)CONV_KERNEL<0, false>, hipFuncAttributeMaxDynamicSharedMemorySize, SMEM);
-        (void)hipFuncSetAttribute((const void*)CONV_KERNEL<1, false>, hipFuncAttributeMaxDynamicSharedMemorySize, SMEM);
-        (void)hipFuncSetAttribute((const void*)CONV_KERNEL<0, true>, hipFuncAttributeMaxDynamicSharedMemorySize, SMEM);
-        (void)hipFuncSetAttribute((const void*)CONV_KERNEL<1, true>, hipFuncAttributeMaxDynamicSharedMemorySize, SMEM);
-        (void)hipFuncSetAttribute((const void*)CONV_KERNEL<0, false, 9, false, 4>, hipFuncAttributeMaxDynamicSharedMemorySize, SMEM);
-        (void)hipFuncSetAttribute((const void*)CONV_KERNEL<1, false, 9, false, 4>, hipFuncAttributeMaxDynamicSharedMemorySize, SMEM);
-        (void)hipFuncSetAttribute((const void*)CONV_KERNEL<0, true, 9, false, 4>, hipFuncAttributeMaxDynamicSharedMemorySize, SMEM);
-        (void)hipFuncSetAttribute((const void*)CONV_KERNEL<1, true, 9, false, 4>, hipFuncAttributeMaxDynamicSharedMemorySize, SMEM);
-        attr = true;
-    }
-#define CV(A, R, NK) hipLaunchKernelGGL((CONV_KERNEL<A, R, 9, false, NK>), grid, dim3(CONV_THREADS), SMEM, s, (const unsigned char*)xpk, (const unsigned char*)wpk, scale, shift, res, B, Cin, Cout, H, W, out, (const int32_t*)nullptr, (const int32_t*)nullptr, (unsigned char*)outpk, stride)
-    if (narrow_tiles(grid.x, Cout)) {
-        constexpr int SMEM4 = 2 * 64 * ROWB > CV_PIX * 68 * 4 ? 2 * 64 * ROWB : CV_PIX * 68 * 4;
-        const dim3 grid4(grid.x, gdm_cdiv(Cout, 64));
-        static bool attr4 = false;
-#define CV4(A, R, NK) hipLaunchKernelGGL((CONV_KERNEL<A, R, 9, false, NK, 4>), grid4, dim3(CONV_THREADS), SMEM4, s, (const unsigned char*)xpk, (const unsigned char*)wpk, scale, shift, res, B, Cin, Cout, H, W, out, (const int32_t*)nullptr, (const int32_t*)nullptr, (unsigned char*)outpk, stride)
-#define AT4(A, R, NK) (void)hipFuncSetAttribute((const void*)CONV_KERNEL<A, R, 9, false, NK, 4>, hipFuncAttributeMaxDynamicSharedMemorySize, SMEM4)
-        if (!attr4) {
-            AT4(0, false, 4); AT4(1, false, 4); AT4(0, true, 4); AT4(1, true, 4);
-            AT4(0, false, 8); AT4(1, false, 8); AT4(0, true, 8); AT4(1, true, 8);
-            attr4 = true;
-        }
-        if (Cin != 64 && (long)grid4.x * grid4.y < 256 && ptot % (CV_PIX / 2) == 0) {
-            const dim3 grid4h(gdm_cdiv(ptot, CV_PIX / 2), grid4.y);
-            static bool attr4h = false;
-#define CV4H(A, R) hipLaunchKernelGGL((CONV_KERNEL<A, R, 9, false, 8, 4, MF_WAVES / 2>), grid4h, dim3(CONV_THREADS / 2), SMEM4, s, (const unsigned char*)xpk, (const unsigned char*)wpk, scale, shift, res, B, Cin, Cout, H, W, out, (const int32_t*)nullptr, (const int32_t*)nullptr, (unsigned char*)outpk, stride)
-#define AT4H(A, R) (void)hipFuncSetAttribute((const void*)CONV_KERNEL<A, R, 9, false, 8, 4, MF_WAVES / 2>, hipFuncAttributeMaxDynamicSharedMemorySize, SMEM4)
-            if (!attr4h) {
-                AT4H(0, false); AT4H(1, false); AT4H(0, true); AT4H(1, true);
-                attr4h = true;
-            }
-            if (act == 0) { if (res) CV4H(0, true); else CV4H(0, false); }
-            else { if (res) CV4H(1, true); else CV4H(1, false); }
-#undef CV4H
-#undef AT4H
-            return gdm_launch_status("conv_mfma16_kernel (3x3, 64-channel tiles, 128 pixels)");
-        }
-        if (Cin == 64) {
-            if (act == 0) { if (res) CV4(0, true, 4); else CV4(0, false, 4); }
-            else { if (res) CV4(1, true, 4); else CV4(1, false, 4); }
-        } else {
-            if (act == 0) { if (res) CV4(0, true, 8); else CV4(0, false, 8); }
-            else { if (res) CV4(1, true, 8); else CV4(1, false, 8); }
-        }
-#undef CV4
-#undef AT4
-        return gdm_launch_status("conv_mfma16_kernel (3x3, 64-channel tiles)");
-    }
-    if (Cin == 64) {
-        if (act == 0) { if (res) CV(0, true, 4); else CV(0, false, 4); }
-        else { if (res) CV(1, true, 4); else CV(1, false, 4); }
-    } else {
-        if (act == 0) { if (res) CV(0, true, 8); else CV(0, false, 8); }
-        else { if (res) CV(1, true, 8); else CV(1, false, 8); }
-    }
-#undef CV
+    const ConvShape c = {9, B, Cin, Cout, H, W, stride, 0};
+    GDM_CHECK_ARG(tile == 0 || tile_allowed(c, tile), "%s: tile %d is not a form of this shape (Cin=%d Cout=%d, %ld pixels)", who, tile, Cin, Cout,
+                  conv_ptot(c));
+    const ConvArgs a = {(const unsigned char*)xpk, (const unsigned char*)wpk, scale, shift, res, B, Cin, Cout, H, W, out, (unsigned char*)outpk, stride};
+    conv_dispatch<9>(tile ? tile : conv_pick_tile(c), a, act, 0, (hipStream_t)stream);
     return gdm_launch_status("conv_mfma16_kernel (3x3)");
 }
 
@@ -631,13 +662,13 @@
 }
 
 static int conv1x1_launch(const void* xpk, const void* wpk, const float* scale, const float* shift,
-                          int B, int Cin, int Cout, int H, int W, int stride, int act, int pixel_major, float* out, void* stream,
+                          int B, int Cin, int Cout, int H, int W, int stride, int act, int pixel_major, float* out, int tile, void* stream,
                           const char* who);
 
 extern "C" int gdm_conv1x1_packed_hip(const void* xpk, const void* wpk, const float* scale, const float* shift,
                                       int B, int Cin, int Cout, int H, int W, int act, int pixel_major, float* out, void* stream)
 {
-    return conv1x1_launch(xpk, wpk, scale, shift, B, Cin, Cout, H, W, 1, act, pixel_major, out, stream, "gdm_conv1x1_packed_hip");
+    return conv1x1_launch(xpk, wpk, scale, shift, B, Cin, Cout, H, W, 1, act, pixel_major, out, 0, stream, "gdm_conv1x1_packed_hip");
 }
 
 extern "C" int gdm_conv1x1_packed_wb_hip(const void* xpk, const void* wpk, long w_bstride, int B, int Cin, int Cout, int H, int W, float* out,
@@ -664,11 +695,18 @@
 extern "C" int gdm_conv1x1_strided_hip(const void* xpk, const void* wpk, const float* scale, const float* shift,
                                        int B, int Cin, int Cout, int H, int W, int stride, int act, float* out, void* stream)
 {
-    return conv1x1_launch(xpk, wpk, scale, shift, B, Cin, Cout, H, W, stride, act, 0, out, stream, "gdm_conv1x1_strided_hip");
+    return conv1x1_launch(xpk, wpk, scale, shift, B, Cin, Cout, H, W, stride, act, 0, out, 0, stream, "gdm_conv1x1_strided_hip");
+}
+
+extern "C" int gdm_conv1x1_packed_tile_hip(const void* xpk, const void* wpk, const float* scale, const float* shift,
+                                           int B, int Cin, int Cout, int H, int W, int stride, int act, int pixel_major, float* out, int tile,
+                                           void* stream)
+{
+    return conv1x1_launch(xpk, wpk, scale, shift, B, Cin, Cout, H, W, stride, act, pixel_major, out, tile, stream, "gdm_conv1x1_packed_tile_hip");
 }
 
 static int conv1x1_launch(const void* xpk, const void* wpk, const float* scale, const float* shift,
-                          int B, int Cin, int Cout, int H, int W, int stride, int act, int pixel_major, float* out, void* stream,
+                          int B, int Cin, int Cout, int H, int W, int stride, int act, int pixel_major, float* out, int tile, void* stream,
                           const char* who)
 {
     GDM_CHECK_ARG(stride == 1 || stride == 2, "%s: stride=%d (1 or 2)", who, stride);
@@ -678,63 +716,10 @@
     GDM_CHECK_ARG(W % 32 == 0 && H >= 1 && (H * W) % CONV_WPIX == 0,
                   "%s: W=%d must be a multiple of 32 and H*W=%d of %d", who, W, H * W, CONV_WPIX);
     GDM_CHECK_ARG(act == 0 || act == 1, "%s: act=%d", who, act);
-    const long ptot = (long)B * H * W;
-    const unsigned ptiles = gdm_cdiv(ptot, CV_PIX);
-    if (Cin != 64 && !pixel_major && stride == 1 && Cout % 144 == 0 && GDM_CONV_GLDS) {
-        const long r128 = gdm_cdiv((long)ptiles * gdm_cdiv(Cout, 128), 256) * 128, r144 = gdm_cdiv((long)ptiles * (Cout / 144), 256) * 144;
-        if (r144 < r128) {
-            constexpr int PANEL9 = 9 * 16 * ROWB, TILE9 = CV_PIX * (9 * 16 + 4) * 4;
-            constexpr int SMEM9 = 2 * PANEL9 > TILE9 ? 2 * PANEL9 : TILE9;
-            static bool attr9 = false;
-            if (!attr9) {
-                (void)hipFuncSetAttribute((const void*)CONV_KERNEL<0, false, 1, false, 8, 9>, hipFuncAttributeMaxDynamicSharedMemorySize, SMEM9);
-                (void)hipFuncSetAttribute((const void*)CONV_KERNEL<1, false, 1, false, 8, 9>, hipFuncAttributeMaxDynamicSharedMemorySize, SMEM9);
-                attr9 = true;
-            }
-            const dim3 grid9(ptiles, Cout / 144);
-#define C19(A) hipLaunchKernelGGL((CONV_KERNEL<A, false, 1, false, 8, 9>), grid9, dim3(CONV_THREADS), SMEM9, (hipStream_t)stream, (const unsigned char*)xpk, (const unsigned char*)wpk, scale, shift, (const float*)nullptr, B, Cin, Cout, H, W, out, (const int32_t*)nullptr, (const int32_t*)nullptr, (unsigned char*)nullptr, stride)
-            if (act == 0) C19(0); else C19(1);
-#undef C19
-            return gdm_launch_status("conv1x1_bf16x3_kernel (144-channel tiles)");
-        }
-    }
-    const bool narrow = Cin != 64 && !pixel_major && narrow_tiles(ptiles, Cout);
-    const unsigned ctiles = gdm_cdiv(Cout, narrow ? 64 : CV_CO);
-    const dim3 grid(ptiles, ctiles);
-    hipStream_t s = (hipStream_t)stream;
-    static bool attr = false;
-    if (!attr) {
-        (void)hipFuncSetAttribute((const void*)CONV_KERNEL<0, false, 1, false>, hipFuncAttributeMaxDynamicSharedMemorySize, 2 * CV_PANEL);
-        (void)hipFuncSetAttribute((const void*)CONV_KERNEL<1, false, 1, false>, hipFuncAttributeMaxDynamicSharedMemorySize, 2 * CV_PANEL);
-        (void)hipFuncSetAttribute((const void*)CONV_KERNEL<0, false, 1, true>, hipFuncAttributeMaxDynamicSharedMemorySize, 2 * CV_PANEL);
-        (void)hipFuncSetAttribute((const void*)CONV_KERNEL<1, false, 1, true>, hipFuncAttributeMaxDynamicSharedMemorySize, 2 * CV_PANEL);
-        (void)hipFuncSetAttribute((const void*)CONV_KERNEL<0, false, 1, false, 4>, hipFuncAttributeMaxDynamicSharedMemorySize, 2 * CV_PANEL);
-        (void)hipFuncSetAttribute((const void*)CONV_KERNEL<1, false, 1, false, 4>, hipFuncAttributeMaxDynamicSharedMemorySize, 2 * CV_PANEL);
-        attr = true;
-    }
-    if (Cin == 64) {
-#define C1TAIL , (const int32_t*)nullptr, (const int32_t*)nullptr, (unsigned char*)nullptr, stride
-#define C1H(A) hipLaunchKernelGGL((CONV_KERNEL<A, false, 1, false, 4>), grid, dim3(CONV_THREADS), 2 * CV_PANEL, s, (const unsigned char*)xpk, (const unsigned char*)wpk, scale, shift, (const float*)nullptr, B, Cin, Cout, H, W, out C1TAIL)
-        if (act == 0) C1H(0); else C1H(1);
-#undef C1H
-        return gdm_launch_status("conv1x1_bf16x3_kernel");
-    }
-    if (narrow) {
-        const dim3 grid4 = grid;
-        static bool attr4 = false;
-        if (!attr4) {
-            (void)hipFuncSetAttribute((const void*)CONV_KERNEL<0, false, 1, false, 8, 4>, hipFuncAttributeMaxDynamicSharedMemorySize, 2 * 64 * ROWB);
-            (void)hipFuncSetAttribute((const void*)CONV_KERNEL<1, false, 1, false, 8, 4>, hipFuncAttributeMaxDynamicSharedMemorySize, 2 * 64 * ROWB);
-            attr4 = true;
-        }
-#define C14(A) hipLaunchKernelGGL((CONV_KERNEL<A, false, 1, false, 8, 4>), grid4, dim3(CONV_THREADS), 2 * 64 * ROWB, s, (const unsigned char*)xpk, (const unsigned char*)wpk, scale, shift, (const float*)nullptr, B, Cin, Cout, H, W, out C1TAIL)
-        if (act == 0) C14(0); else C14(1);
-#undef C14
-        return gdm_launch_status("conv1x1_bf16x3_kernel (64-channel tiles)");
-    }
-#define C1(A, P) hipLaunchKernelGGL((CONV_KERNEL<A, false, 1, P>), grid, dim3(CONV_THREADS), 2 * CV_PANEL, s, (const unsigned char*)xpk, (const unsigned char*)wpk, scale, shift, (const float*)nullptr, B, Cin, Cout, H, W, out C1TAIL)
-    if (act == 0) { if (pixel_major) C1(0, true); else C1(0, false); }
-    else { if (pixel_major) C1(1, true); else C1(1, false); }
-#undef C1
-    return gdm_launch_status("conv1x1_bf16x3_kernel");
-}
+    const ConvShape c = {1, B, Cin, Cout, H, W, stride, pixel_major ? 1 : 0};
+    GDM_CHECK_ARG(tile == 0 || tile_allowed(c, tile), "%s: tile %d is not a form of this shape (Cin=%d Cout=%d, %ld pixels)", who, tile, Cin, Cout,
+                  conv_ptot(c));
+    const ConvArgs a = {(const unsigned char*)xpk, (const unsigned char*)wpk, scale, shift, nullptr, B, Cin, Cout, H, W, out, nullptr, stride};
+    conv_dispatch<1>(tile ? tile : conv_pick_tile(c), a, act, pixel_major, (hipStream_t)stream);
+    return gdm_launch_status("conv_mfma16_kernel (1x1)");
+}
diff --git a/geometric_aware_dense_matching_amd/ops.py b/geometric_aware_dense_matching_amd/ops.py
--- a/geometric_aware_dense_matching_amd/ops.py
+++ b/geometric_aware_dense_matching_amd/ops.py
@@ -1440,7 +1440,7 @@
     return PackedAct(buf, (B, C, H, W))
 
 
-def conv3x3_bf16x3(x, wpk, cout, scale=None, shift=None, act=ACT_NONE, res=None, out_f32=True, out_packed=False, stride=1):
+def conv3x3_bf16x3(x, wpk, cout, scale=None, shift=None, act=ACT_NONE, res=None, out_f32=True, out_packed=False, stride=1, tile=0):
     xp = x if isinstance(x, PackedAct) else conv3x3_pack_act(x)
     B, Cin, H, W = xp.shape
     if stride != 1:
@@ -1458,6 +1458,13 @@
     if res is not None:
         res = _dev(res, torch.float32, "res")
         assert tuple(res.shape) == (B, cout, H, W)
+    if tile:
+        check(L.gdm_conv3x3_packed_tile_hip(xp.buf.data_ptr(), wpk.data_ptr(), scale.data_ptr() if scale is not None else None,
+                                            shift.data_ptr() if shift is not None else None, res.data_ptr() if res is not None else None,
+                                            B, Cin, cout, H, W, int(stride), act, out.data_ptr() if out is not None else None,
+                                            opk.buf.data_ptr() if opk is not None else None, int(tile), _stream()),
+              "gdm_conv3x3_packed_tile_hip")
+        return (out, opk) if out_packed else out
     check(L.gdm_conv3x3_strided_hip(xp.buf.data_ptr(), wpk.data_ptr(), scale.data_ptr() if scale is not None else None,
                                     shift.data_ptr() if shift is not None else None, res.data_ptr() if res is not None else None,
                                     B, Cin, cout, H, W, int(stride), act, out.data_ptr() if out is not None else None,
@@ -1477,12 +1484,17 @@
     return gemm_bf16x3(x.reshape(B, Cin, H * W), wpk, cout).view(B, cout, H, W)
 
 
-def conv1x1_packed2d(xp, wpk, cout, scale=None, shift=None, act=ACT_NONE, stride=1):
+def conv1x1_packed2d(xp, wpk, cout, scale=None, shift=None, act=ACT_NONE, stride=1, tile=0):
     B, Cin, H, W = xp.shape
     if stride not in (1, 2) or H % stride or W % stride:
         raise ValueError("conv1x1_packed2d: stride %r on a %dx%d map" % (stride, H, W))
     H, W = H // stride, W // stride
     out = torch.empty((B, cout, H, W), dtype=torch.float32, device=xp.buf.device)
+    if tile:
+        check(_lib.lib().gdm_conv1x1_packed_tile_hip(xp.buf.data_ptr(), wpk.data_ptr(), scale.data_ptr() if scale is not None else None,
+                                                     shift.data_ptr() if shift is not None else None, B, Cin, cout, H, W, int(stride), act,
+                                                     0, out.data_ptr(), int(tile), _stream()), "gdm_conv1x1_packed_tile_hip")
+        return out
     check(_lib.lib().gdm_conv1x1_strided_hip(xp.buf.data_ptr(), wpk.data_ptr(), scale.data_ptr() if scale is not None else None,
                                              shift.data_ptr() if shift is not None else None, B, Cin, cout, H, W, int(stride), act,
                                              out.data_ptr(), _stream()), "gdm_conv1x1_strided_hip")
@@ -1527,13 +1539,18 @@
     return wpk
 
 
-def gemm_bf16x3(x, wpk, cout, scale=None, shift=None, act=ACT_NONE, pixel_major=False):
+def gemm_bf16x3(x, wpk, cout, scale=None, shift=None, act=ACT_NONE, pixel_major=False, tile=0):
     x = _dev(x, torch.float32, "x")
     B, Cin, n = x.shape
     L = _lib.lib()
     xpk = _packed_buffer(B, Cin, 1, n, x.device)
     check(L.gdm_conv3x3_pack_act_hip(x.data_ptr(), B, Cin, 1, n, xpk.data_ptr(), _stream()), "gdm_conv3x3_pack_act_hip")
     out = torch.empty((B * n, cout) if pixel_major else (B, cout, n), dtype=torch.float32, device=x.device)
+    if tile:
+        check(L.gdm_conv1x1_packed_tile_hip(xpk.data_ptr(), wpk.data_ptr(), scale.data_ptr() if scale is not None else None,
+                                            shift.data_ptr() if shift is not None else None, B, Cin, cout, 1, n, 1, act,
+                                            1 if pixel_major else 0, out.data_ptr(), int(tile), _stream()), "gdm_conv1x1_packed_tile_hip")
+        return out
     check(L.gdm_conv1x1_packed_hip(xpk.data_ptr(), wpk.data_ptr(), scale.data_ptr() if scale is not None else None,
                                    shift.data_ptr() if shift is not None else None, B, Cin, cout, 1, n, act,
                                    1 if pixel_major else 0, out.data_ptr(), _stream()), "gdm_conv1x1_packed_hip")
diff --git a/include/gdm.h b/include/gdm.h
--- a/include/gdm.h
+++ b/include/gdm.h
@@ -222,6 +222,11 @@
 int gdm_conv_pack_weight_dgrad_hip(const float* w, int Cout, int Cin, int taps, void* wpk, void* stream);
 int gdm_conv1x1_packed_hip(const void* xpk, const void* wpk, const float* scale, const float* shift,
                            int B, int Cin, int Cout, int H, int W, int act, int pixel_major, float* out, void* stream);
+int gdm_conv3x3_packed_tile_hip(const void* xpk, const void* wpk, const float* scale, const float* shift, const float* res,
+                                int B, int Cin, int Cout, int H, int W, int stride, int act, float* out, void* outpk, int tile, void* stream);
+int gdm_conv1x1_packed_tile_hip(const void* xpk, const void* wpk, const float* scale, const float* shift,
+                                int B, int Cin, int Cout, int H, int W, int stride, int act, int pixel_major, float* out, int tile,
+                                void* stream);
 
 int gdm_depth_to_xyz_hip(const float* depth, const float* K, const int32_t* origin, int B, int H, int W, int S,
                          float* out, void* stream);
```

Result: no change. 5203 (-0.3%).
